# pnotp/ArcFlow

Hardware: AMD Instinct MI355X
Metric: 1024x1024 images/sec @ 2 NFE (FLUX-12B architecture, denoiser + ArcFlow integrator) (higher is better)
Workload: dtype bf16; 1 GPU; ArcFlow-FLUX-12B 2-NFE inference, 1024x1024, bs=1 per GPU; nfe=2, parallelism=1 independent replica(s), no collective, lora=merged into base weights

## Files before the change

arcflow_amd/_lib.py:

```python
from __future__ import annotations

import ctypes as C
import os
from typing import Optional

from .build import lib_path

AFX_DT_BF16 = 1
AFX_DT_F32 = 2
AFX_DT_FP8 = 3

EXPORTS = [
    'afx_last_error', 'afx_version', 'afx_create', 'afx_destroy', 'afx_bind_weight', 'afx_finalize',
    'afx_workspace_bytes', 'afx_head_width', 'afx_set_workspace', 'afx_mmdit_forward', 'afx_profile_enable', 'afx_profile_read', 'afx_set_checkpoint_buffer', 'afx_arcflow_step',
    'afx_arcflow_velocity', 'afx_linear_bf16', 'afx_attention_ws_bytes', 'afx_attention_bf16', 'afx_attention_to_mx8',
    'afx_norm_modulate_bf16', 'afx_qk_norm_rope_bf16', 'afx_gemv_bf16',
    'afx_attention_fwd_lse_bf16', 'afx_attention_bwd_ws_bytes', 'afx_attention_bwd_bf16',
    'afx_ln_modulate_backward', 'afx_qk_norm_rope_oop_bf16', 'afx_gelu_bf16', 'afx_add_scale_bf16',
    'afx_conv3x3_bf16', 'afx_conv3x3_bf16_stats', 'afx_groupnorm_nhwc_from_stats', 'afx_conv_stats_available', 'afx_upconv3x3_bf16', 'afx_groupnorm_nhwc', 'afx_groupnorm_ws_bytes', 'afx_upsample2x_nhwc', 'afx_interior_nhwc', 'afx_softmax_rows_f32',
    'afx_latent_to_nhwc', 'afx_nhwc_to_image', 'afx_latent_to_nhwc_affine', 'afx_rmsnorm_nhwc',
    'afx_conv3x3s2_bf16', 'afx_image_to_cols27', 'afx_posterior_latents',
    'afx_embed_rows_bf16', 'afx_norm_rows_bf16', 'afx_act_mul_bf16', 'afx_rope_half_bf16', 'afx_attention_ext_ws_bytes',
    'afx_attention_ext_bf16', 'afx_linear_bf16_splitk', 'afx_finish_f32_bf16', 'afx_linear_splitk_chunks', 'afx_quant_rows_fp8', 'afx_linear_fp8', 'afx_quant_rows_mx8', 'afx_linear_fp8_mx', 'afx_linear_fp8_to_mx8',
    'afx_linear_bf16_pre', 'afx_gemm_set_mode', 'afx_gemm_set_fp8_tile', 'afx_gemm_dropres_available', 'afx_attn_set_impl', 'afx_attn_bwd_set_impl', 'afx_mmdit_prepare_steps', 'afx_mmdit_use_prepared_step', 'afx_lora_dropout_bf16', 'afx_mmdit_forward_stage', 'afx_mmdit_import_tokens',
    'afx_coldot_bf16', 'afx_gate_residual_bf16', 'afx_gemv_t_bf16', 'afx_set_temb_override', 'afx_set_fp8_linear',
    'afx_arcflow_step_dropout', 'afx_arcflow_backward', 'afx_mse_loss', 'afx_euler_roll', 'afx_axpby_rows', 'afx_cfg_combine',
    'afx_head_grad', 'afx_linear_bf16_f32out', 'afx_linear_tn_f32out', 'afx_linear_tn_f32out_ws', 'afx_linear_tn_ws_bytes', 'afx_linear_bf16_dropres', 'afx_transpose_bf16', 'afx_colsum_bf16', 'afx_normout_backward', 'afx_normout_backward_split',
    'afx_outer_accum', 'afx_mmdit_export', 'afx_sumsq', 'afx_adamw_step', 'afx_adamw8bit_step', 'afx_ema_lerp', 'afx_cast_f32_bf16',
    'afx_qkv_operands', 'afx_norm_modulate_joint_bf16', 'afx_norm_modulate_mx8',
]

AFX_BLOCK_DOUBLE, AFX_BLOCK_SINGLE = 0, 1
AFX_QKV_PATHS = {'auto': 0, 'vt_proj': 1, 'qk_epi': 2, 'kv_prep': 3}


class ModelDesc(C.Structure):
    _fields_ = [(n, C.c_int32) for n in (
        'family', 'num_double', 'num_single', 'heads', 'head_dim', 'in_channels', 'joint_dim',
        'pooled_dim', 'guidance_embeds', 'num_gaussians', 'logweights_channels', 'head_mode')]


class ArcflowHipError(RuntimeError):
    pass


_lib: Optional[C.CDLL] = None


def load() -> C.CDLL:
    global _lib
    if _lib is not None:
        return _lib
    path = os.environ.get('ARCFLOW_HIP_LIB', lib_path())
    if not os.path.exists(path):
        raise ArcflowHipError(
            f'{path} not found: the HIP engine is not built. Run `python -m arcflow_amd.build` '
            '(needs hipcc, cross-compiles for gfx950 without a GPU). There is no CPU fallback.')
    lib = C.CDLL(path)
    vp, i32, i64, f32 = C.c_void_p, C.c_int32, C.c_int64, C.c_float
    lib.afx_last_error.restype = C.c_char_p
    lib.afx_version.restype = C.c_char_p
    lib.afx_create.argtypes = [C.POINTER(ModelDesc), C.POINTER(vp)]
    lib.afx_destroy.argtypes = [vp]
    lib.afx_bind_weight.argtypes = [vp, C.c_char_p, vp, i32, i32, C.POINTER(i64)]
    lib.afx_finalize.argtypes = [vp]
    lib.afx_workspace_bytes.argtypes = [vp, i32, i32, i32]
    lib.afx_workspace_bytes.restype = i64
    lib.afx_head_width.argtypes = [vp]
    lib.afx_head_width.restype = i32
    lib.afx_set_workspace.argtypes = [vp, vp, i64]
    lib.afx_mmdit_forward.argtypes = [vp, vp, vp, vp, vp, vp, vp, vp, i32, i32, i32, vp, vp, vp, vp]
    lib.afx_set_checkpoint_buffer.argtypes = [vp, vp]
    lib.afx_profile_enable.argtypes = [vp, i32]
    lib.afx_profile_read.argtypes = [vp, i32, C.POINTER(C.c_double), C.POINTER(i64), C.POINTER(C.c_double)]
    lib.afx_arcflow_step.argtypes = [vp, vp, vp, vp, i32, f32, f32, f32, vp, f32, vp, i32, i32, i32, i32, i32, vp]
    lib.afx_arcflow_velocity.argtypes = [vp, vp, vp, i32, f32, f32, vp, vp, i32, i32, i32, i32, i32, vp]
    lib.afx_linear_bf16.argtypes = [vp, i64, vp, i64, vp, vp, i64, i32, i32, i32, i32, i32, vp, i64, i32, vp, i64, vp]
    lib.afx_attention_ws_bytes.argtypes = [i32, i32, i32]
    lib.afx_attention_ws_bytes.restype = i64
    lib.afx_attention_bf16.argtypes = [vp, i64, vp, i64, vp, i64, vp, i64, vp, i32, i32, i32, vp]
    lib.afx_attention_to_mx8.argtypes = [vp, i64, vp, i64, vp, i64, vp, i64, vp, i64, vp, i32, i32, i32, vp]
    lib.afx_norm_modulate_bf16.argtypes = [vp, i64, vp, i64, i32, i32, vp, vp, i64, i32, i32, vp]
    lib.afx_qk_norm_rope_bf16.argtypes = [vp, i64, vp, vp, vp, vp, i32, i32, i32, i32, vp]
    lib.afx_gemv_bf16.argtypes = [vp, vp, vp, vp, i32, i32, i32, i32, i32, vp]
    lib.afx_attention_fwd_lse_bf16.argtypes = [vp, i64, vp, i64, vp, i64, vp, i64, vp, vp, i32, i32, i32, vp]
    lib.afx_attention_bwd_ws_bytes.argtypes = [i32, i32, i32]
    lib.afx_attention_bwd_ws_bytes.restype = i64
    lib.afx_attention_bwd_bf16.argtypes = [vp, i64, vp, i64, vp, i64, vp, i64, vp, i64, vp, vp, i64, vp, i64, vp, i64, vp, i32, i32, i32, vp]
    lib.afx_ln_modulate_backward.argtypes = [vp, i64, vp, i64, vp, i64, i32, vp, i64, vp, i64, i32, i32, vp]
    lib.afx_qk_norm_rope_oop_bf16.argtypes = [vp, i64, vp, i64, vp, i64, vp, vp, vp, vp, i32, i32, i32, i32, i32, vp]
    lib.afx_gelu_bf16.argtypes = [vp, i64, vp, i64, vp, i64, i64, i32, vp]
    lib.afx_add_scale_bf16.argtypes = [vp, i64, vp, i64, vp, i64, i32, vp, i64, i64, i32, vp]
    lib.afx_conv3x3_bf16.argtypes = [vp, vp, vp, vp, i32, i32, i32, i32, vp, vp]
    lib.afx_groupnorm_nhwc.argtypes = [vp, vp, vp, i32, i32, i32, i32, vp, vp, f32, i32, vp]
    lib.afx_groupnorm_ws_bytes.argtypes = [i32, i32]
    lib.afx_groupnorm_ws_bytes.restype = i64
    lib.afx_conv3x3_bf16_stats.argtypes = [vp, vp, vp, vp, i32, i32, i32, i32, vp, vp, i32, vp]
    lib.afx_groupnorm_nhwc_from_stats.argtypes = [vp, vp, vp, vp, i32, i32, i32, i32, vp, vp, f32, i32, vp]
    lib.afx_conv_stats_available.argtypes = []
    lib.afx_upconv3x3_bf16.argtypes = [vp, vp, vp, vp, i32, i32, i32, i32, vp]
    lib.afx_upsample2x_nhwc.argtypes = [vp, vp, i32, i32, i32, vp]
    lib.afx_interior_nhwc.argtypes = [vp, vp, vp, i32, i32, i32, i32, vp]
    lib.afx_softmax_rows_f32.argtypes = [vp, i64, vp, i64, i32, i32, f32, vp]
    lib.afx_latent_to_nhwc.argtypes = [vp, vp, i32, i32, i32, f32, f32, vp]
    lib.afx_nhwc_to_image.argtypes = [vp, vp, i32, i32, i32, vp]
    lib.afx_latent_to_nhwc_affine.argtypes = [vp, vp, i32, i32, i32, vp, vp, vp]
    lib.afx_rmsnorm_nhwc.argtypes = [vp, vp, i64, i32, i32, vp, i32, vp]
    lib.afx_conv3x3s2_bf16.argtypes = [vp, vp, vp, vp, vp, i32, i32, i32, i32, vp, i32, vp]
    lib.afx_image_to_cols27.argtypes = [vp, i32, vp, i32, i32, i32, vp]
    lib.afx_posterior_latents.argtypes = [vp, i32, i32, i32, vp, vp, vp, vp, vp, i32, vp, i32, vp, vp]
    lib.afx_embed_rows_bf16.argtypes = [vp, vp, vp, vp, i32, i32, vp]
    lib.afx_norm_rows_bf16.argtypes = [vp, i64, vp, i64, i32, i32, vp, vp, f32, i32, vp]
    lib.afx_act_mul_bf16.argtypes = [vp, i64, vp, i64, i64, i32, i32, i32, vp]
    lib.afx_rope_half_bf16.argtypes = [vp, i64, vp, vp, i32, i32, i32, vp]
    lib.afx_linear_bf16_splitk.argtypes = [vp, i64, vp, i64, vp, vp, i32, i32, i32, i32, vp]
    lib.afx_finish_f32_bf16.argtypes = [vp, i32, vp, i64, vp, i64, i64, i32, vp]
    lib.afx_quant_rows_fp8.argtypes = [vp, i64, vp, i64, vp, i32, i32, vp]
    lib.afx_linear_fp8.argtypes = [vp, i64, vp, vp, i64, vp, vp, vp, i64, i32, i32, i32, i32, i32, vp, i64, i32, vp, i64, vp]
    lib.afx_quant_rows_mx8.argtypes = [vp, i64, vp, i64, vp, i64, i32, i32, vp]
    lib.afx_linear_fp8_to_mx8.argtypes = [vp, i64, vp, i64, vp, vp, i64, vp, vp, vp, i64, vp, i64, vp, i64, i32, i32, i32, i32, i32, vp]
    lib.afx_linear_fp8_mx.argtypes = [vp, i64, vp, i64, vp, vp, i64, vp, vp, vp, i64, i32, i32, i32, i32, i32, vp, i64, i32, vp, i64, vp]
    lib.afx_linear_splitk_chunks.argtypes = [i32, i32, i32, i32]
    lib.afx_linear_bf16_pre.argtypes = [vp, i64, vp, i64, vp, vp, i64, i32, i32, i32, i32, i32, vp, i64, i32, vp, i64, vp, i64, vp]
    lib.afx_mmdit_prepare_steps.argtypes = [vp, vp, vp, vp, i32, i32, vp]
    lib.afx_mmdit_use_prepared_step.argtypes = [vp, i32]
    lib.afx_gemm_set_mode.argtypes = [i32, i32]
    lib.afx_gemm_set_mode.restype = i32
    lib.afx_gemm_set_fp8_tile.argtypes = [i32]
    lib.afx_gemm_set_fp8_tile.restype = i32
    lib.afx_gemm_dropres_available.argtypes = []
    lib.afx_gemm_dropres_available.restype = i32
    lib.afx_attn_set_impl.argtypes = [i32]
    lib.afx_attn_set_impl.restype = i32
    lib.afx_attn_bwd_set_impl.argtypes = [i32]
    lib.afx_attn_bwd_set_impl.restype = i32
    lib.afx_lora_dropout_bf16.argtypes = [vp, i64, vp, i64, i64, i32, i64, f32, C.c_uint32, i32, vp]
    lib.afx_mmdit_forward_stage.argtypes = [vp, vp, vp, vp, vp, vp, vp, vp, i32, i32, i32, vp, vp, vp, i32, vp]
    lib.afx_mmdit_import_tokens.argtypes = [vp, vp, i32, i32, i32, vp]
    lib.afx_coldot_bf16.argtypes = [vp, i64, vp, i64, vp, i32, i32, vp]
    lib.afx_gate_residual_bf16.argtypes = [vp, i64, vp, vp, i64, vp, i64, i64, i32, vp]
    lib.afx_gemv_t_bf16.argtypes = [vp, i64, vp, i64, vp, i32, i64, i32, vp]
    lib.afx_set_temb_override.argtypes = [vp, vp]
    lib.afx_set_fp8_linear.argtypes = [vp, i32]
    lib.afx_linear_splitk_chunks.restype = i32
    lib.afx_attention_ext_ws_bytes.argtypes = [i32, i32, i32, i32]
    lib.afx_attention_ext_ws_bytes.restype = i64
    lib.afx_attention_ext_bf16.argtypes = [vp, i64, vp, i64, vp, i64, vp, i64, vp, i32, i32, i32, i32, i32, f32, i32, vp, vp]
    lib.afx_arcflow_step_dropout.argtypes = [vp, vp, vp, vp, i32, vp, vp, f32, vp, i32, i32, i32, i32, i32, vp]
    lib.afx_arcflow_backward.argtypes = [vp, vp, vp, vp, i32, f32, f32, f32, vp, vp, f32, f32, vp, vp, vp, i32, i32, i32,
                                         i32, i32, i32, i32, vp]
    lib.afx_mse_loss.argtypes = [vp, vp, f32, vp, vp, i64, vp]
    lib.afx_euler_roll.argtypes = [vp, vp, vp, vp, vp, i32, i64, vp]
    lib.afx_axpby_rows.argtypes = [vp, vp, vp, vp, vp, i32, i64, vp]
    lib.afx_cfg_combine.argtypes = [vp, vp, f32, vp, i64, vp]
    lib.afx_head_grad.argtypes = [vp, vp, vp, vp, vp, i64, i64, i32, i32, i32, vp]
    lib.afx_linear_bf16_f32out.argtypes = [vp, i64, vp, i64, vp, i64, i32, i32, i32, i32, vp]
    lib.afx_linear_tn_f32out.argtypes = [vp, i64, vp, i64, vp, i64, i32, i32, i32, i32, vp]
    lib.afx_linear_tn_f32out_ws.argtypes = [vp, i64, vp, i64, vp, i64, i32, i32, i32, i32, vp, vp]
    lib.afx_linear_tn_ws_bytes.argtypes = [i32, i32, i32]
    lib.afx_linear_tn_ws_bytes.restype = i64
    lib.afx_linear_bf16_dropres.argtypes = [vp, i64, vp, i64, vp, i64, i32, i32, i32, vp, i64, f32, C.c_uint32, i64, vp]
    lib.afx_transpose_bf16.argtypes = [vp, i64, vp, i64, i32, i32, vp]
    lib.afx_colsum_bf16.argtypes = [vp, i64, vp, i32, i32, vp]
    lib.afx_normout_backward.argtypes = [vp, i64, vp, i64, vp, i32, i32, i32, vp]
    lib.afx_normout_backward_split.argtypes = [vp, i64, vp, i64, vp, vp, i32, i32, vp]
    lib.afx_outer_accum.argtypes = [vp, vp, vp, i32, i32, i32, vp]
    lib.afx_mmdit_export.argtypes = [vp, C.c_char_p, vp, i32, i32, i32, vp]
    lib.afx_sumsq.argtypes = [vp, vp, i64, vp]
    lib.afx_adamw_step.argtypes = [vp, vp, vp, vp, f32, f32, f32, f32, f32, i32, f32, i64, vp]
    lib.afx_adamw8bit_step.argtypes = [vp, vp, vp, vp, vp, vp, vp, vp, f32, f32, f32, f32, f32, i32, f32, i64, vp]
    lib.afx_ema_lerp.argtypes = [vp, vp, f32, i64, vp]
    lib.afx_cast_f32_bf16.argtypes = [vp, vp, i64, vp]
    lib.afx_qkv_operands.argtypes = [i32, vp, i64, vp, vp, vp, vp, vp, vp, vp, i32, i32, i32, i32, i32, vp, i64, vp, vp]
    lib.afx_norm_modulate_joint_bf16.argtypes = [vp, i64, vp, i64, i32, i32, vp, vp, vp, vp, i64, i32, i32, vp]
    lib.afx_norm_modulate_mx8.argtypes = [vp, i64, vp, i64, vp, i64, vp, i32, i32, vp, vp, vp, vp, i64, i32, i32, C.POINTER(i32), vp]
    for name in EXPORTS:
        fn = getattr(lib, name)
        if fn.restype is C.c_int:
            fn.restype = C.c_int32
    _lib = lib
    return lib


def check(rc: int) -> None:
    if rc != 0:
        raise ArcflowHipError(f'libarcflow_hip error {rc}: {load().afx_last_error().decode()}')
```

arcflow_amd/csrc/afx_elementwise.hip:

```cpp
#include <cstdlib>

#include "afx_common.h"
#include "afx_kernels.h"

namespace afx {

constexpr int NM_MAX_CHUNKS = 8;

__global__ __launch_bounds__(256) void norm_modulate_kernel(
    const bf16_t* __restrict__ x, int64_t ldx, bf16_t* __restrict__ out, int64_t ldo, int rows, int D,
    const float* __restrict__ scale, const float* __restrict__ shift, int64_t ldmod, int rows_per_batch,
    int rms, const float* __restrict__ scale_txt, const float* __restrict__ shift_txt, int n_txt) {
  const int lane = threadIdx.x & 63;
  const int row = blockIdx.x * 4 + (threadIdx.x >> 6);
  if (row >= rows) return;
  const int nchunk = D >> 3;
  const bf16_t* xr = x + (int64_t)row * ldx;
  float v[NM_MAX_CHUNKS][8];
  float s = 0.f;
#pragma unroll
  for (int i = 0; i < NM_MAX_CHUNKS; ++i) {
    const int c = lane + i * 64;
    if (c < nchunk) {
      const u32x4_t w = *reinterpret_cast<const u32x4_t*>(xr + c * 8);
      unpack8(w, v[i]);
#pragma unroll
      for (int e = 0; e < 8; ++e) s += rms ? v[i][e] * v[i][e] : v[i][e];
    }
  }
  s = wave_sum(s);
  float mean = 0.f, rstd;
  if (rms) {
    rstd = rsqrtf(s / (float)D + 1e-6f);
  } else {
    mean = s / (float)D;
    float q = 0.f;
#pragma unroll
    for (int i = 0; i < NM_MAX_CHUNKS; ++i) {
      const int c = lane + i * 64;
      if (c < nchunk) {
#pragma unroll
        for (int e = 0; e < 8; ++e) {
          const float d = v[i][e] - mean;
          q += d * d;
        }
      }
    }
    q = wave_sum(q);
    rstd = rsqrtf(q / (float)D + 1e-6f);
  }
  const int64_t moff = rms ? 0 : (int64_t)(row / rows_per_batch) * ldmod;
  if (scale_txt != nullptr && row % rows_per_batch < n_txt) {
    scale = scale_txt;
    shift = shift_txt;
  }
  bf16_t* orow = out + (int64_t)row * ldo;
#pragma unroll
  for (int i = 0; i < NM_MAX_CHUNKS; ++i) {
    const int c = lane + i * 64;
    if (c < nchunk) {
      const f32x4_t s0 = *reinterpret_cast<const f32x4_t*>(scale + moff + c * 8);
      const f32x4_t s1 = *reinterpret_cast<const f32x4_t*>(scale + moff + c * 8 + 4);
      const float sc[8] = {s0[0], s0[1], s0[2], s0[3], s1[0], s1[1], s1[2], s1[3]};
      float r[8];
      if (rms) {
#pragma unroll
        for (int e = 0; e < 8; ++e) r[e] = v[i][e] * rstd * sc[e];
      } else {
        const f32x4_t h0 = *reinterpret_cast<const f32x4_t*>(shift + moff + c * 8);
        const f32x4_t h1 = *reinterpret_cast<const f32x4_t*>(shift + moff + c * 8 + 4);
        const float sh[8] = {h0[0], h0[1], h0[2], h0[3], h1[0], h1[1], h1[2], h1[3]};
#pragma unroll
        for (int e = 0; e < 8; ++e) r[e] = (v[i][e] - mean) * rstd * (1.0f + sc[e]) + sh[e];
      }
      *reinterpret_cast<u32x4_t*>(orow + c * 8) = pack8(r);
    }
  }
}

template <int NCH, int R, int QOUT = 0>
__global__ __launch_bounds__(256) void norm_modulate_rows_kernel(
    const bf16_t* __restrict__ x, int64_t ldx, bf16_t* __restrict__ out, int64_t ldo, int rows,
    const float* __restrict__ scale, const float* __restrict__ shift, int64_t ldmod, int rows_per_batch,
    const float* __restrict__ scale_txt, const float* __restrict__ shift_txt, int n_txt, uint8_t* __restrict__ q8 = nullptr, int64_t ldq = 0,
    uint8_t* __restrict__ mx = nullptr, int64_t ld_mx = 0, float* __restrict__ rowscale = nullptr) {
  constexpr bool MX8 = QOUT == 1;
  constexpr int D = 512 * NCH;
  const int lane = threadIdx.x & 63;
  const int row0 = (blockIdx.x * 4 + (threadIdx.x >> 6)) * R;
  if (row0 >= rows) return;
  const int nrows = min(R, rows - row0);
  float sc[NCH][8], sh[NCH][8];
  int key = -1;
  u32x4_t cur[NCH], nxt[NCH];
  {
    const bf16_t* xr = x + (int64_t)row0 * ldx;
#pragma unroll
    for (int i = 0; i < NCH; ++i) cur[i] = *reinterpret_cast<const u32x4_t*>(xr + (lane + i * 64) * 8);
  }
#pragma unroll 1
  for (int rr = 0; rr < nrows; ++rr) {
    const int row = row0 + rr;
    if (rr + 1 < nrows) {
      const bf16_t* xn = x + (int64_t)(row + 1) * ldx;
#pragma unroll
      for (int i = 0; i < NCH; ++i) nxt[i] = *reinterpret_cast<const u32x4_t*>(xn + (lane + i * 64) * 8);
    }
    const int b = row / rows_per_batch;
    const bool txt = scale_txt != nullptr && row - b * rows_per_batch < n_txt;
    const int k = 2 * b + (txt ? 1 : 0);
    if (k != key) {
      key = k;
      const float* sp = (txt ? scale_txt : scale) + (int64_t)b * ldmod;
      const float* hp = (txt ? shift_txt : shift) + (int64_t)b * ldmod;
#pragma unroll
      for (int i = 0; i < NCH; ++i) {
        const int c = (lane + i * 64) * 8;
        const f32x4_t s0 = *reinterpret_cast<const f32x4_t*>(sp + c), s1 = *reinterpret_cast<const f32x4_t*>(sp + c + 4);
        const f32x4_t h0 = *reinterpret_cast<const f32x4_t*>(hp + c), h1 = *reinterpret_cast<const f32x4_t*>(hp + c + 4);
#pragma unroll
        for (int e = 0; e < 4; ++e) {
          sc[i][e] = 1.0f + s0[e]; sc[i][4 + e] = 1.0f + s1[e];
          sh[i][e] = h0[e];        sh[i][4 + e] = h1[e];
        }
      }
    }
    float v[NCH][8];
    float s = 0.f;
#pragma unroll
    for (int i = 0; i < NCH; ++i) {
      unpack8(cur[i], v[i]);
#pragma unroll
      for (int e = 0; e < 8; ++e) s += v[i][e];
    }
    s = wave_sum(s);
    const float mean = s / (float)D;
    float q = 0.f;
#pragma unroll
    for (int i = 0; i < NCH; ++i)
#pragma unroll
      for (int e = 0; e < 8; ++e) {
        const float d = v[i][e] - mean;
        q += d * d;
      }
    q = wave_sum(q);
    const float rstd = rsqrtf(q / (float)D + 1e-6f);
    bf16_t* orow = out + (int64_t)row * ldo;
    if constexpr (QOUT == 2) {
      float amax = 0.f;
#pragma unroll
      for (int i = 0; i < NCH; ++i)
#pragma unroll
        for (int e = 0; e < 8; ++e) {
          v[i][e] = (v[i][e] - mean) * rstd * sc[i][e] + sh[i][e];
          amax = fmaxf(amax, fabsf(v[i][e]));
        }
#pragma unroll
      for (int o = 32; o > 0; o >>= 1) amax = fmaxf(amax, __shfl_xor(amax, o, 64));
      const float s_ = fmaxf(amax, 1e-12f) / 448.0f;
      const float inv = 1.0f / s_;
      if (lane == 0) rowscale[row] = s_;
#pragma unroll
      for (int i = 0; i < NCH; ++i) {
        uint32_t w0, w1;
        mx_pack8(v[i], inv, w0, w1);
        *reinterpret_cast<u32x2_t*>(q8 + (int64_t)row * ldq + (lane + i * 64) * 8) = (u32x2_t){w0, w1};
      }
    } else
#pragma unroll
    for (int i = 0; i < NCH; ++i) {
      float r[8];
#pragma unroll
      for (int e = 0; e < 8; ++e) r[e] = (v[i][e] - mean) * rstd * sc[i][e] + sh[i][e];
      if constexpr (MX8) {
        float amax = 0.f;
#pragma unroll
        for (int e = 0; e < 8; ++e) amax = fmaxf(amax, fabsf(r[e]));
#pragma unroll
        for (int o = 8; o > 0; o >>= 1) amax = fmaxf(amax, __shfl_xor(amax, o, 64));
        const int eb = mx_exp(amax);
        uint32_t w0, w1;
        mx_pack8(r, mx_inv(eb), w0, w1);
        *reinterpret_cast<u32x2_t*>(q8 + (int64_t)row * ldq + (lane + i * 64) * 8) = (u32x2_t){w0, w1};
        if ((lane & 15) == 0) mx[(int64_t)row * ld_mx + 4 * i + (lane >> 4)] = (uint8_t)eb;
      } else
      *reinterpret_cast<u32x4_t*>(orow + (lane + i * 64) * 8) = pack8(r);
    }
#pragma unroll
    for (int i = 0; i < NCH; ++i) cur[i] = nxt[i];
  }
}

static int nm_rows_per_wave() {
  static int r = -1;
  if (r < 0) {
    const char* e = getenv("AFX_NM_ROWS");
    r = e ? atoi(e) : 2;
  }
  return r;
}

static bool launch_norm_modulate_rows(const uint16_t* x, int64_t ldx, uint16_t* out, int64_t ldo, int rows, int D, const float* scale,
                                      const float* shift, int64_t ldmod, int rows_per_batch, const float* scale_txt, const float* shift_txt,
                                      int n_txt, hipStream_t stream, uint8_t* q8 = nullptr, int64_t ldq = 0, uint8_t* mx = nullptr, int64_t ld_mx = 0,
                                      float* rowscale = nullptr) {
  const int R = nm_rows_per_wave();
  if (D != 3072 || rows < 1024 || (R != 2 && R != 4)) return false;
  const dim3 grid((rows + 4 * R - 1) / (4 * R));
  if (q8 != nullptr) {
    if (R != 2) return false;
    if (rowscale != nullptr)
      hipLaunchKernelGGL((norm_modulate_rows_kernel<6, 2, 2>), grid, dim3(256), 0, stream, x, ldx, out, ldo, rows, scale, shift, ldmod, rows_per_batch,
                         scale_txt, shift_txt, n_txt, q8, ldq, (uint8_t*)nullptr, (int64_t)0, rowscale);
    else
      hipLaunchKernelGGL((norm_modulate_rows_kernel<6, 2, 1>), grid, dim3(256), 0, stream, x, ldx, out, ldo, rows, scale, shift, ldmod, rows_per_batch,
                         scale_txt, shift_txt, n_txt, q8, ldq, mx, ld_mx, (float*)nullptr);
    return true;
  }
  if (R == 2)
    hipLaunchKernelGGL((norm_modulate_rows_kernel<6, 2, 0>), grid, dim3(256), 0, stream, x, ldx, out, ldo, rows, scale, shift, ldmod, rows_per_batch,
                       scale_txt, shift_txt, n_txt);
  else
    hipLaunchKernelGGL((norm_modulate_rows_kernel<6, 4, 0>), grid, dim3(256), 0, stream, x, ldx, out, ldo, rows, scale, shift, ldmod, rows_per_batch,
                       scale_txt, shift_txt, n_txt);
  return true;
}

hipError_t launch_norm_modulate(const uint16_t* x, int64_t ldx, uint16_t* out, int64_t ldo, int rows,
                                int D, const float* scale, const float* shift, int64_t ldmod,
                                int rows_per_batch, int rms, hipStream_t stream) {
  if (rows <= 0) return hipSuccess;
  if (D > NM_MAX_CHUNKS * 512 || (D & 7)) return hipErrorInvalidValue;
  if (!rms && launch_norm_modulate_rows(x, ldx, out, ldo, rows, D, scale, shift, ldmod, rows_per_batch > 0 ? rows_per_batch : rows, nullptr, nullptr, 0,
                                        stream))
    return hipGetLastError();
  hipLaunchKernelGGL(norm_modulate_kernel, dim3((rows + 3) / 4), dim3(256), 0, stream, x, ldx, out, ldo, rows,
                     D, scale, shift, ldmod, rows_per_batch > 0 ? rows_per_batch : rows, rms, (const float*)nullptr,
                     (const float*)nullptr, 0);
  return hipGetLastError();
}

hipError_t launch_norm_modulate_mx8(const uint16_t* x, int64_t ldx, uint8_t* q8, int64_t ldq, uint8_t* mx, int64_t ld_mx, int rows, int D,
                                    const float* scale, const float* shift, const float* scale_txt, const float* shift_txt, int64_t ldmod, int S,
                                    int n_txt, hipStream_t stream, bool* fused, float* rowscale) {
  *fused = rows > 0 && launch_norm_modulate_rows(x, ldx, nullptr, 0, rows, D, scale, shift, ldmod, S, scale_txt, shift_txt, n_txt, stream, q8, ldq, mx, ld_mx,
                                                 rowscale);
  return hipGetLastError();
}

hipError_t launch_norm_modulate_joint(const uint16_t* x, int64_t ldx, uint16_t* out, int64_t ldo, int rows, int D, const float* scale,
                                      const float* shift, const float* scale_txt, const float* shift_txt, int64_t ldmod, int S,
                                      int n_txt, hipStream_t stream) {
  if (rows <= 0) return hipSuccess;
  if (D > NM_MAX_CHUNKS * 512 || (D & 7) || S <= 0) return hipErrorInvalidValue;
  if (launch_norm_modulate_rows(x, ldx, out, ldo, rows, D, scale, shift, ldmod, S, scale_txt, shift_txt, n_txt, stream)) return hipGetLastError();
  hipLaunchKernelGGL(norm_modulate_kernel, dim3((rows + 3) / 4), dim3(256), 0, stream, x, ldx, out, ldo, rows, D, scale, shift, ldmod,
                     S, 0, scale_txt, shift_txt, n_txt);
  return hipGetLastError();
}

struct QkRopeArgs { bf16_t* x[2]; const float* w_txt[2]; const float* w_img[2]; };

__global__ __launch_bounds__(256) void qk_norm_rope_kernel(
    const QkRopeArgs a, int64_t ldx, const float* __restrict__ cos_t, const float* __restrict__ sin_t, int S, int n_txt, int H,
    int64_t total) {
  bf16_t* __restrict__ x = a.x[blockIdx.y];
  const float* __restrict__ w_txt = a.w_txt[blockIdx.y];
  const float* __restrict__ w_img = a.w_img[blockIdx.y];
  const int64_t g = (int64_t)blockIdx.x * 256 + threadIdx.x;
  if (g >= total) return;
  const int c = (int)(g & 15);
  const int64_t th = g >> 4;
  const int h = (int)(th % H);
  const int64_t row = th / H;
  const int s = (int)(row % S);
  bf16_t* p = x + row * ldx + h * 128 + c * 8;
  float v[8];
  unpack8(*reinterpret_cast<const u32x4_t*>(p), v);
  float ss = 0.f;
#pragma unroll
  for (int e = 0; e < 8; ++e) ss += v[e] * v[e];
#pragma unroll
  for (int o = 8; o > 0; o >>= 1) ss += __shfl_xor(ss, o, 64);
  const float rstd = rsqrtf(ss * (1.0f / 128.0f) + 1e-6f);
  const float* w = (s < n_txt ? w_txt : w_img) + c * 8;
  const f32x4_t w0 = *reinterpret_cast<const f32x4_t*>(w);
  const f32x4_t w1 = *reinterpret_cast<const f32x4_t*>(w + 4);
  const float wv[8] = {w0[0], w0[1], w0[2], w0[3], w1[0], w1[1], w1[2], w1[3]};
  const f32x4_t cs = *reinterpret_cast<const f32x4_t*>(cos_t + (int64_t)s * 64 + c * 4);
  const f32x4_t sn = *reinterpret_cast<const f32x4_t*>(sin_t + (int64_t)s * 64 + c * 4);
  float r[8];
#pragma unroll
  for (int i = 0; i < 4; ++i) {
    const float a = v[2 * i] * rstd * wv[2 * i];
    const float b = v[2 * i + 1] * rstd * wv[2 * i + 1];
    r[2 * i] = a * cs[i] - b * sn[i];
    r[2 * i + 1] = a * sn[i] + b * cs[i];
  }
  *reinterpret_cast<u32x4_t*>(p) = pack8(r);
}

hipError_t launch_qk_norm_rope(uint16_t* x, int64_t ldx, const float* w_txt, const float* w_img,
                               const float* cos_t, const float* sin_t, int B, int S, int n_txt, int H,
                               hipStream_t stream) {
  const int64_t total = (int64_t)B * S * H * 16;
  if (total == 0) return hipSuccess;
  QkRopeArgs a{};
  a.x[0] = x; a.w_txt[0] = w_txt; a.w_img[0] = w_img;
  hipLaunchKernelGGL(qk_norm_rope_kernel, dim3((unsigned)((total + 255) / 256), 1), dim3(256), 0, stream, a, ldx, cos_t, sin_t, S,
                     n_txt, H, total);
  return hipGetLastError();
}

hipError_t launch_qk_norm_rope2(uint16_t* xk, uint16_t* xq, int64_t ldx, const float* wk_txt, const float* wk_img, const float* wq_txt,
                                const float* wq_img, const float* cos_t, const float* sin_t, int B, int S, int n_txt, int H,
                                hipStream_t stream) {
  const int64_t total = (int64_t)B * S * H * 16;
  if (total == 0) return hipSuccess;
  QkRopeArgs a{};
  a.x[0] = xk; a.w_txt[0] = wk_txt; a.w_img[0] = wk_img;
  a.x[1] = xq; a.w_txt[1] = wq_txt; a.w_img[1] = wq_img;
  hipLaunchKernelGGL(qk_norm_rope_kernel, dim3((unsigned)((total + 255) / 256), 2), dim3(256), 0, stream, a, ldx, cos_t, sin_t, S,
                     n_txt, H, total);
  return hipGetLastError();
}

constexpr int GEMV_MAXB = 8;

__global__ __launch_bounds__(256) void gemv_kernel(const float* __restrict__ x, const bf16_t* __restrict__ W,
                                                   const bf16_t* __restrict__ bias, float* __restrict__ y,
                                                   int B, int N, int K, int act, int accumulate, int64_t ldy) {
  const int lane = threadIdx.x & 63;
  const int n = blockIdx.x * 4 + (threadIdx.x >> 6);
  if (n >= N) return;
  const bf16_t* wr = W + (int64_t)n * K;
  float acc[GEMV_MAXB];
#pragma unroll
  for (int b = 0; b < GEMV_MAXB; ++b) acc[b] = 0.f;
  for (int c = lane; c < (K >> 3); c += 64) {
    float w[8];
    unpack8(*reinterpret_cast<const u32x4_t*>(wr + c * 8), w);
#pragma unroll
    for (int b = 0; b < GEMV_MAXB; ++b) {
      if (b < B) {
        const f32x4_t x0 = *reinterpret_cast<const f32x4_t*>(x + (int64_t)b * K + c * 8);
        const f32x4_t x1 = *reinterpret_cast<const f32x4_t*>(x + (int64_t)b * K + c * 8 + 4);
        acc[b] += w[0] * x0[0] + w[1] * x0[1] + w[2] * x0[2] + w[3] * x0[3] + w[4] * x1[0] + w[5] * x1[1] +
                  w[6] * x1[2] + w[7] * x1[3];
      }
    }
  }
  const float bv = bias ? bf16_to_f32(bias[n]) : 0.f;
#pragma unroll
  for (int b = 0; b < GEMV_MAXB; ++b) {
    if (b < B) {
      float r = wave_sum(acc[b]) + bv;
      if (act == 1) r = silu(r);
      if (lane == 0) {
        float* yp = y + (int64_t)b * ldy + n;
        *yp = accumulate ? (*yp + r) : r;
      }
    }
  }
}

hipError_t launch_gemv(const float* x, const uint16_t* W, const uint16_t* bias, float* y, int B, int N,
                       int K, int act, int accumulate, hipStream_t stream, int64_t ldy) {
  if (ldy <= 0) ldy = N;
  if (B > GEMV_MAXB || (K & 7)) return hipErrorInvalidValue;
  if (N == 0 || B == 0) return hipSuccess;
  hipLaunchKernelGGL(gemv_kernel, dim3((N + 3) / 4), dim3(256), 0, stream, x, W, bias, y, B, N, K, act, accumulate, ldy);
  return hipGetLastError();
}

__global__ void sincos_kernel(const float* __restrict__ t, float scale, float* __restrict__ out, int B, int cast_mode) {
  const int i = threadIdx.x;
  const int b = blockIdx.x;
  if (b >= B) return;
  const float f = expf(-9.210340371976184f * (float)i / 128.0f);
  float tb = t[b];
  if (cast_mode != 0) tb = bf16_to_f32(f32_to_bf16(tb));
  float a;
  if (cast_mode == 1) a = bf16_to_f32(f32_to_bf16(tb * scale)) * f;
  else a = scale * (tb * f);
  out[b * 256 + i] = cosf(a);
  out[b * 256 + 128 + i] = sinf(a);
}
hipError_t launch_sincos(const float* t, float scale, float* out, int B, int cast_mode, hipStream_t stream) {
  hipLaunchKernelGGL(sincos_kernel, dim3(B), dim3(128), 0, stream, t, scale, out, B, cast_mode);
  return hipGetLastError();
}

__global__ void silu_kernel(const float* __restrict__ x, float* __restrict__ y, int64_t n) {
  const int64_t i = (int64_t)blockIdx.x * 256 + threadIdx.x;
  if (i < n) y[i] = silu(x[i]);
}
hipError_t launch_silu(const float* x, float* y, int64_t n, hipStream_t stream) {
  hipLaunchKernelGGL(silu_kernel, dim3((unsigned)((n + 255) / 256)), dim3(256), 0, stream, x, y, n);
  return hipGetLastError();
}

__global__ void bf16_to_f32_kernel(const bf16_t* __restrict__ x, float* __restrict__ y, int64_t n) {
  const int64_t i = (int64_t)blockIdx.x * 256 + threadIdx.x;
  if (i < n) y[i] = bf16_to_f32(x[i]);
}
hipError_t launch_bf16_to_f32(const uint16_t* x, float* y, int64_t n, hipStream_t stream) {
  hipLaunchKernelGGL(bf16_to_f32_kernel, dim3((unsigned)((n + 255) / 256)), dim3(256), 0, stream, x, y, n);
  return hipGetLastError();
}

__global__ void copy_rows_kernel(const bf16_t* __restrict__ src, int64_t lds_, bf16_t* __restrict__ dst,
                                 int64_t ldd, int64_t rows, int cols) {
  const int cpr = cols >> 3;
  const int64_t g = (int64_t)blockIdx.x * 256 + threadIdx.x;
  if (g >= rows * cpr) return;
  const int64_t r = g / cpr;
  const int c = (int)(g % cpr);
  *reinterpret_cast<u32x4_t*>(dst + r * ldd + c * 8) = *reinterpret_cast<const u32x4_t*>(src + r * lds_ + c * 8);
}
hipError_t launch_copy_rows(const uint16_t* src, int64_t lds_, uint16_t* dst, int64_t ldd, int64_t rows,
                            int cols, hipStream_t stream) {
  const int64_t total = rows * (cols >> 3);
  if (total == 0) return hipSuccess;
  hipLaunchKernelGGL(copy_rows_kernel, dim3((unsigned)((total + 255) / 256)), dim3(256), 0, stream, src, lds_,
                     dst, ldd, rows, cols);
  return hipGetLastError();
}

__global__ __launch_bounds__(256) void head_split_kernel(const bf16_t* __restrict__ head, int64_t ldh,
                                                         bf16_t* __restrict__ means, bf16_t* __restrict__ logw,
                                                         bf16_t* __restrict__ logg, int64_t rows, int K, int ch,
                                                         int lw) {
  const int64_t row = blockIdx.x;
  const bf16_t* hr = head + row * ldh;
  const int nm = K * ch, nw = K * lw, ng = (K - 1) * lw;
  for (int i = threadIdx.x; i < nm; i += 256) means[row * nm + i] = hr[i];
  for (int i = threadIdx.x; i < ng; i += 256) logg[row * ng + i] = hr[nm + nw + i];
  if (threadIdx.x < lw) {
    const int p = threadIdx.x;
    float mx = -INFINITY;
    for (int k = 0; k < K; ++k) mx = fmaxf(mx, bf16_to_f32(hr[nm + k * lw + p]));
    float se = 0.f;
    for (int k = 0; k < K; ++k) se += expf(bf16_to_f32(hr[nm + k * lw + p]) - mx);
    const float lse = mx + logf(se);
    for (int k = 0; k < K; ++k) logw[row * nw + k * lw + p] = f32_to_bf16(bf16_to_f32(hr[nm + k * lw + p]) - lse);
  }
}
hipError_t launch_head_split(const uint16_t* head, int64_t ldh, uint16_t* means, uint16_t* logw,
                             uint16_t* logg, int64_t rows, int K, int ch, int lw, hipStream_t stream) {
  if (rows == 0) return hipSuccess;
  hipLaunchKernelGGL(head_split_kernel, dim3((unsigned)rows), dim3(256), 0, stream, head, ldh, means, logw, logg,
                     rows, K, ch, lw);
  return hipGetLastError();
}

template <typename MixT> AFX_DEV float mix_load(const MixT* p, int64_t i);
template <> AFX_DEV float mix_load<float>(const float* p, int64_t i) { return p[i]; }
template <> AFX_DEV float mix_load<bf16_t>(const bf16_t* p, int64_t i) { return bf16_to_f32(p[i]); }

constexpr int ARC_MAXK = 32;

template <typename MixT>
__global__ __launch_bounds__(256) void arcflow_step_kernel(
    const float* __restrict__ x_in, const MixT* __restrict__ means, const MixT* __restrict__ logw,
    const MixT* __restrict__ logg, float s_src, float s_start, float s_end,
    const float* __restrict__ sigma_vec, float eps, float* __restrict__ x_out, int64_t tokens, int n_tok, int K,
    int ch, int pp, int velocity_only, const uint8_t* __restrict__ drop) {
  const int lane = threadIdx.x & 63;
  const int64_t tok = (int64_t)blockIdx.x * 4 + (threadIdx.x >> 6);
  if (tok >= tokens) return;
  const int64_t bidx = tok / n_tok;
  if (sigma_vec != nullptr) {
    s_src = sigma_vec[3 * bidx];
    s_start = sigma_vec[3 * bidx + 1];
    s_end = sigma_vec[3 * bidx + 2];
  }
  const float d_past = s_src - s_start;
  const float d_step = s_start - s_end;
  const uint8_t* dr = drop ? drop + bidx * K : nullptr;
  const MixT* mt = means + tok * (int64_t)K * ch;
  const MixT* wt = logw + tok * (int64_t)K * pp;
  const MixT* gt = logg + tok * (int64_t)(K - 1) * pp;
  for (int c = lane; c < ch; c += 64) {
    const int q = c % pp;
    float lw[ARC_MAXK];
    float mx = -INFINITY;
#pragma unroll
    for (int k = 0; k < ARC_MAXK; ++k)
      if (k < K) {
        lw[k] = (dr && dr[k]) ? -INFINITY : mix_load<MixT>(wt, k * pp + q);
        mx = fmaxf(mx, lw[k]);
      }
    float den = 0.f;
#pragma unroll
    for (int k = 0; k < ARC_MAXK; ++k)
      if (k < K) {
        lw[k] = expf(lw[k] - mx);
        den += lw[k];
      }
    const float inv = 1.0f / den;
    float acc = (lw[0] * inv) * mix_load<MixT>(mt, c) * (velocity_only ? 1.0f : d_step);
#pragma unroll
    for (int k = 1; k < ARC_MAXK; ++k)
      if (k < K) {
        const float g = mix_load<MixT>(gt, (k - 1) * pp + q);
        const float m = mix_load<MixT>(mt, (int64_t)k * ch + c);
        const float decay = expf(g * d_past);
        float term;
        if (velocity_only) {
          term = m * decay;
        } else {
          const float z = g * d_step;
          const float zs = (z < 0.f ? -1.0f : 1.0f) * fmaxf(fabsf(z), eps);
          const float phi = expm1f(zs) / zs;
          term = m * decay * d_step * phi;
        }
        acc += (lw[k] * inv) * term;
      }
    const int64_t xi = tok * ch + c;
    x_out[xi] = velocity_only ? acc : (x_in[xi] - acc);
  }
}


template <typename MixT> struct Mix8;
template <> struct Mix8<bf16_t> {
  AFX_DEV static void load(const bf16_t* p, float (&f)[8]) { unpack8(*reinterpret_cast<const u32x4_t*>(p), f); }
};
template <> struct Mix8<float> {
  AFX_DEV static void load(const float* p, float (&f)[8]) {
    const f32x4_t a = *reinterpret_cast<const f32x4_t*>(p), b = *reinterpret_cast<const f32x4_t*>(p + 4);
    f[0] = a[0]; f[1] = a[1]; f[2] = a[2]; f[3] = a[3]; f[4] = b[0]; f[5] = b[1]; f[6] = b[2]; f[7] = b[3];
  }
};

template <typename MixT, int TPW>
__global__ __launch_bounds__(256) void arcflow_step_k16_kernel(
    const float* __restrict__ x_in, const MixT* __restrict__ means, const MixT* __restrict__ logw,
    const MixT* __restrict__ logg, float s_src0, float s_start0, float s_end0, const float* __restrict__ sigma_vec, float eps,
    float* __restrict__ x_out, int64_t tokens, int n_tok, int velocity_only, const uint8_t* __restrict__ drop) {
  constexpr int K = 16, CH = 64, PP = 4;
  const int lane = threadIdx.x & 63;
  const int64_t tok0 = ((int64_t)blockIdx.x * 4 + (threadIdx.x >> 6)) * TPW;
  if (tok0 >= tokens) return;
  const int k = lane >> 2;
  float mA[TPW][8], mB[TPW][8], lw[TPW], lg[TPW], xv[TPW];
#pragma unroll
  for (int t = 0; t < TPW; ++t) {
    const int64_t tok = tok0 + t < tokens ? tok0 + t : tokens - 1;
    const MixT* mt = means + tok * (int64_t)(K * CH);
    Mix8<MixT>::load(mt + lane * 8, mA[t]);
    Mix8<MixT>::load(mt + (64 + lane) * 8, mB[t]);
    lw[t] = mix_load<MixT>(logw + tok * (K * PP), lane);
    lg[t] = k > 0 ? mix_load<MixT>(logg + tok * ((K - 1) * PP), lane - PP) : 0.f;
  }
  const int e3 = ((lane >> 5) & 1) * 4 + ((lane >> 4) & 1) * 2 + ((lane >> 3) & 1);
  const int cfin = (lane & 7) * 8 + e3;
  if (!velocity_only) {
#pragma unroll
    for (int t = 0; t < TPW; ++t) xv[t] = x_in[(tok0 + t < tokens ? tok0 + t : tokens - 1) * CH + cfin];
  }
#pragma unroll
  for (int t = 0; t < TPW; ++t) {
    const int64_t tok = tok0 + t;
    if (tok >= tokens) break;
    const int64_t bidx = tok / n_tok;
    float s_src = s_src0, s_start = s_start0, s_end = s_end0;
    if (sigma_vec != nullptr) {
      s_src = sigma_vec[3 * bidx];
      s_start = sigma_vec[3 * bidx + 1];
      s_end = sigma_vec[3 * bidx + 2];
    }
    const float d_past = s_src - s_start, d_step = s_start - s_end;
    float l = lw[t];
    if (drop != nullptr && drop[bidx * K + k]) l = -INFINITY;
    float mx = l;
#pragma unroll
    for (int o = 4; o < 64; o <<= 1) mx = fmaxf(mx, __shfl_xor(mx, o, 64));
    const float ex = expf(l - mx);
    float den = ex;
#pragma unroll
    for (int o = 4; o < 64; o <<= 1) den += __shfl_xor(den, o, 64);
    float coef = ex / den;
    if (k > 0) {
      const float g = lg[t];
      coef *= expf(g * d_past);
      if (!velocity_only) {
        const float z = g * d_step;
        const float zs = (z < 0.f ? -1.0f : 1.0f) * fmaxf(fabsf(z), eps);
        coef *= d_step * (expm1f(zs) / zs);
      }
    } else if (!velocity_only) {
      coef *= d_step;
    }
    float cA[4], cB[4];
#pragma unroll
    for (int q = 0; q < 4; ++q) {
      cA[q] = __shfl(coef, (lane >> 3) * 4 + q, 64);
      cB[q] = __shfl(coef, (8 + (lane >> 3)) * 4 + q, 64);
    }
    float v[8];
#pragma unroll
    for (int e = 0; e < 8; ++e) v[e] = cA[e & 3] * mA[t][e] + cB[e & 3] * mB[t][e];
    const bool h5 = (lane & 32) != 0, h4 = (lane & 16) != 0, h3 = (lane & 8) != 0;
    float w4[4], w2[2];
#pragma unroll
    for (int i = 0; i < 4; ++i) {
      const float keep = h5 ? v[4 + i] : v[i], send = h5 ? v[i] : v[4 + i];
      w4[i] = keep + __shfl_xor(send, 32, 64);
    }
#pragma unroll
    for (int i = 0; i < 2; ++i) {
      const float keep = h4 ? w4[2 + i] : w4[i], send = h4 ? w4[i] : w4[2 + i];
      w2[i] = keep + __shfl_xor(send, 16, 64);
    }
    const float keep = h3 ? w2[1] : w2[0], send = h3 ? w2[0] : w2[1];
    const float acc = keep + __shfl_xor(send, 8, 64);
    x_out[tok * CH + cfin] = velocity_only ? acc : (xv[t] - acc);
  }
}

hipError_t launch_arcflow_step(const float* x_in, const void* means, const void* logw, const void* logg,
                               int mix_bf16, float s_src, float s_start, float s_end,
                               const float* sigma_vec, float eps, float* x_out, int B, int n_tok, int K,
                               int ch, int pp, int velocity_only, const uint8_t* drop, hipStream_t stream) {
  if (K < 1 || K > ARC_MAXK || pp < 1 || ch < 1) return hipErrorInvalidValue;
  const int64_t tokens = (int64_t)B * n_tok;
  if (tokens == 0) return hipSuccess;
  if (K == 16 && ch == 64 && pp == 4) {
    static int tpw = -1;
    if (tpw < 0) {
      const char* e = getenv("AFX_STEP_TPW");
      tpw = e ? atoi(e) : 1;
      if (tpw != 1 && tpw != 2 && tpw != 4) tpw = 1;
    }
#define AFX_STEP_LAUNCH(T, TPW)                                                                                                     \
    hipLaunchKernelGGL((arcflow_step_k16_kernel<T, TPW>), dim3((unsigned)((tokens + 4 * TPW - 1) / (4 * TPW))), dim3(256), 0, stream, \
                       x_in, (const T*)means, (const T*)logw, (const T*)logg, s_src, s_start, s_end, sigma_vec, eps, x_out, tokens,  \
                       n_tok, velocity_only, drop)
    if (mix_bf16) {
      if (tpw == 1) AFX_STEP_LAUNCH(bf16_t, 1); else if (tpw == 4) AFX_STEP_LAUNCH(bf16_t, 4); else AFX_STEP_LAUNCH(bf16_t, 2);
    } else {
      if (tpw == 1) AFX_STEP_LAUNCH(float, 1); else if (tpw == 4) AFX_STEP_LAUNCH(float, 4); else AFX_STEP_LAUNCH(float, 2);
    }
#undef AFX_STEP_LAUNCH
    return hipGetLastError();
  }
  dim3 grid((unsigned)((tokens + 3) / 4)), block(256);
  if (mix_bf16)
    hipLaunchKernelGGL(arcflow_step_kernel<bf16_t>, grid, block, 0, stream, x_in, (const bf16_t*)means,
                       (const bf16_t*)logw, (const bf16_t*)logg, s_src, s_start, s_end, sigma_vec, eps, x_out,
                       tokens, n_tok, K, ch, pp, velocity_only, drop);
  else
    hipLaunchKernelGGL(arcflow_step_kernel<float>, grid, block, 0, stream, x_in, (const float*)means,
                       (const float*)logw, (const float*)logg, s_src, s_start, s_end, sigma_vec, eps, x_out,
                       tokens, n_tok, K, ch, pp, velocity_only, drop);
  return hipGetLastError();
}

}
```

arcflow_amd/csrc/afx_engine.hip:

```cpp
#include <hip/hip_runtime.h>

#include <cstdarg>
#include <cstdio>
#include <cstring>
#include <string>
#include <unordered_map>
#include <vector>

#include "../../include/arcflow_hip.h"
#include "afx_kernels.h"

using namespace afx;

#include "afx_api_util.h"

thread_local char afx_g_err[512] = "";

int afx_fail(int code, const char* fmt, ...) {
  va_list ap;
  va_start(ap, fmt);
  vsnprintf(afx_g_err, sizeof(afx_g_err), fmt, ap);
  va_end(ap);
  return code;
}

namespace {

struct Weight {
  const void* ptr = nullptr;
  int dtype = 0;
  std::vector<int64_t> shape;
};

inline int64_t align256(int64_t x) { return (x + 255) / 256 * 256; }

}

struct LinW {
  const uint16_t* w = nullptr;
  const uint16_t* b = nullptr;
  const void* wq = nullptr;
  const float* wscale = nullptr;
};
struct DoubleW { LinW qkv[2], out[2], mlp1[2], mlp2[2]; const float* qkn = nullptr; };
struct SingleW { LinW fused, out; const float* qkn = nullptr; };

struct afx_ctx {
  afx_model_desc d;
  std::unordered_map<std::string, Weight> w;
  bool finalized = false;
  std::vector<DoubleW> dbl;
  std::vector<SingleW> sgl;
  char* ws = nullptr;
  int64_t ws_bytes = 0;
  int D = 0;
  int64_t n_mod = 0;
  int head_n = 0;
  uint16_t* ckpt = nullptr;
  bool fp8 = false;
  int fp8_mx = -1;
  const float* temb_override = nullptr;
  int prep_steps = 0, prep_B = 0, prep_use = -1;
  bool prof_on = false;
  int prof_stride = 1;
  uint64_t prof_count = 0;
  struct ProfRec { hipEvent_t a, b; int klass; double flops; };
  std::vector<ProfRec> prof_pool;
  size_t prof_used = 0;
};

namespace {

const uint16_t* W16(const afx_ctx* c, const std::string& n) {
  auto it = c->w.find(n);
  return it == c->w.end() ? nullptr : (const uint16_t*)it->second.ptr;
}
const float* W32(const afx_ctx* c, const std::string& n) {
  auto it = c->w.find(n);
  return it == c->w.end() ? nullptr : (const float*)it->second.ptr;
}

const void* WQ(const afx_ctx* c, const std::string& n) {
  auto it = c->w.find(n);
  return it == c->w.end() ? nullptr : it->second.ptr;
}

int need(const afx_ctx* c, const std::string& n, int dtype, std::vector<int64_t> shape) {
  auto it = c->w.find(n);
  if (it == c->w.end()) return fail(AFX_E_MISSING, "weight '%s' is not bound", n.c_str());
  if (it->second.dtype != dtype) return fail(AFX_E_INVALID, "weight '%s': wrong dtype", n.c_str());
  if (it->second.shape != shape) {
    std::string got, want;
    for (auto v : it->second.shape) got += std::to_string(v) + ",";
    for (auto v : shape) want += std::to_string(v) + ",";
    return fail(AFX_E_INVALID, "weight '%s': shape [%s] expected [%s]", n.c_str(), got.c_str(), want.c_str());
  }
  return AFX_OK;
}

int need_linear(const afx_ctx* c, const std::string& n, int64_t out_f, int64_t in_f) {
  int r = need(c, n + ".weight", AFX_DT_BF16, {out_f, in_f});
  if (r) return r;
  return need(c, n + ".bias", AFX_DT_BF16, {out_f});
}

struct ModLayout {
  int64_t D;
  int nd, ns;
  int64_t dbl(int i, int stream , int chunk ) const {
    return ((int64_t)i * 12 + stream * 6 + chunk) * D;
  }
  int64_t sgl(int i, int chunk ) const { return (int64_t)nd * 12 * D + ((int64_t)i * 3 + chunk) * D; }
  int64_t fin(int chunk ) const { return (int64_t)nd * 12 * D + (int64_t)ns * 3 * D + chunk * D; }
  int64_t total() const { return (int64_t)nd * 12 * D + (int64_t)ns * 3 * D + 2 * D; }
};

constexpr int AFX_PREP_ROWS = 8;

struct Workspace {
  uint16_t *X, *Xn, *F, *Vt, *head;
  float *sincos, *tmp, *temb, *semb, *mod, *pooled;
  float *prep_temb, *prep_semb, *prep_mod;
  uint8_t* q8;
  uint8_t* q8n;
  uint8_t* mxn;
  uint8_t* mxw;
  float* ones;
  int64_t ld_mxn, ld_mxw;
  float* qs;
  int64_t total;
};

Workspace carve(const afx_ctx* c, char* base, int B, int N, int T) {
  const int64_t D = c->D, S = (int64_t)N + T, R = (int64_t)B * S;
  Workspace w;
  int64_t off = 0;
  auto take = [&](int64_t bytes) {
    char* p = base ? base + off : nullptr;
    off += align256(bytes);
    return p;
  };
  w.prep_temb = (float*)take((int64_t)AFX_PREP_ROWS * D * 4);
  w.prep_semb = (float*)take((int64_t)AFX_PREP_ROWS * D * 4);
  w.prep_mod = (float*)take((int64_t)AFX_PREP_ROWS * c->n_mod * 4);
  w.X = (uint16_t*)take(R * D * 2);
  w.Xn = (uint16_t*)take(R * D * 2);
  w.F = (uint16_t*)take(R * 7 * D * 2);
  w.Vt = (uint16_t*)take((int64_t)B * c->d.heads * 128 * attn_spad((int)S) * 2);
  w.head = (uint16_t*)take((int64_t)B * N * c->head_n * 2);
  w.sincos = (float*)take((int64_t)B * 256 * 4);
  w.tmp = (float*)take((int64_t)B * D * 4);
  w.temb = (float*)take((int64_t)B * D * 4);
  w.semb = (float*)take((int64_t)B * D * 4);
  w.pooled = (float*)take((int64_t)B * (c->d.pooled_dim > 0 ? c->d.pooled_dim : 8) * 4);
  w.mod = (float*)take((int64_t)B * c->n_mod * 4);
  w.q8 = nullptr;
  w.qs = nullptr;
  w.q8n = w.mxn = w.mxw = nullptr;
  w.ones = nullptr;
  w.ld_mxn = (D / 128 + 3) / 4 * 4;
  w.ld_mxw = (5 * D / 128 + 3) / 4 * 4;
  if (c->fp8) {
    w.q8 = (uint8_t*)take(R * 5 * D);
    w.qs = (float*)take(R * 4);
    w.q8n = (uint8_t*)take(R * D);
    w.mxn = (uint8_t*)take(R * w.ld_mxn);
    w.mxw = (uint8_t*)take(R * w.ld_mxw);
    w.ones = (float*)take(R * 4);
  }
  w.total = off;
  return w;
}

struct ProfScope {
  afx_ctx* c; hipStream_t st; afx_ctx::ProfRec* r = nullptr;
  ProfScope(afx_ctx* c_, hipStream_t st_, int klass, double flops) : c(c_), st(st_) {
    if (!c->prof_on) return;
    if ((c->prof_count++ % (uint64_t)c->prof_stride) != 0) return;
    if (c->prof_used == c->prof_pool.size()) {
      afx_ctx::ProfRec n{};
      if (hipEventCreate(&n.a) != hipSuccess || hipEventCreate(&n.b) != hipSuccess) return;
      c->prof_pool.push_back(n);
    }
    r = &c->prof_pool[c->prof_used++];
    r->klass = klass; r->flops = flops;
    launch_timer().start = r->a;
    launch_timer().stop = r->b;
  }
  ~ProfScope() { launch_timer() = LaunchTimer{}; }
};

double gemm_flops(const GemmBatch& gb) {
  double f = 0;
  for (int i = 0; i < gb.nprob; ++i) f += 2.0 * gb.p[i].M * (double)gb.p[i].N * gb.p[i].K;
  return f;
}

struct BlockShape {
  int64_t D;
  int H, B, N, T, S, S_pad;
  const float* rope_cos;
  const float* rope_sin;
  uint16_t* Vt;
};

BlockShape block_shape(int H, int B, int N, int T, const float* rope_cos, const float* rope_sin, uint16_t* Vt) {
  BlockShape q;
  q.D = (int64_t)H * 128; q.H = H; q.B = B; q.N = N; q.T = T; q.S = N + T; q.S_pad = (int)attn_spad(N + T);
  q.rope_cos = rope_cos; q.rope_sin = rope_sin; q.Vt = Vt;
  return q;
}

bool vt_proj_shape_ok(const BlockShape& q, bool single) {
  return q.T % 16 == 0 && q.S % 64 == 0 && (!single || q.B + 3 <= GEMM_MAX_PROBLEMS);
}

int qkv_path(const BlockShape& q, bool single, bool fp8, bool qk_fuse_fp8) {
  const bool qk_fuse = gemm_qk_fusion_available() && (!fp8 || qk_fuse_fp8);
  const bool vt_fuse = qk_fuse && !fp8 && getenv("AFX_VT_FUSE_OFF") == nullptr && vt_proj_shape_ok(q, single);
  return vt_fuse ? AFX_QKV_VT_PROJ : qk_fuse ? AFX_QKV_QK_EPI : AFX_QKV_KV_PREP;
}

void set_qk_epilogue(GemmProblem& p, const BlockShape& q, const float* wq, const float* wk, int row0, int period) {
  p.qk_D = (int)q.D; p.qk_wq = wq; p.qk_wk = wk;
  p.rope_cos = q.rope_cos; p.rope_sin = q.rope_sin; p.rope_row0 = row0; p.rope_period = period; p.rope_rows = q.S;
}

void stream_qk_epilogue(GemmProblem& p, const BlockShape& q, const float* qkn, int s) {
  set_qk_epilogue(p, q, qkn + (s == 0 ? 0 : 2) * 128, qkn + (s == 0 ? 1 : 3) * 128, s == 0 ? q.T : 0, 1 << 30);
}

void stream_problem(GemmProblem& p, const BlockShape& q, const uint16_t* A, int64_t lda, int K, const LinW& lw, uint16_t* C, int64_t ldc,
                    int Nout, int b, int s) {
  p = GemmProblem{};
  const int64_t row0 = (int64_t)b * q.S + (s == 0 ? q.T : 0);
  p.A = A + row0 * lda; p.lda = lda;
  p.W = lw.w; p.ldw = K; p.bias = lw.b;
  p.C = C + row0 * ldc; p.ldc = ldc;
  p.M = (s == 0 ? q.N : q.T); p.N = Nout; p.K = K;
}

void kqv_problems(GemmBatch& gb, const BlockShape& q, const uint16_t* A, int64_t lda, const LinW& lw, uint16_t* C, int64_t ldc, int64_t row0g,
                  int rows, int b, int pos0, int period, const float* wq, const float* wk, bool with_v) {
  const int64_t D = q.D;
  for (int part = 0; part < (with_v ? 3 : 2); ++part) {
    GemmProblem& p = gb.p[gb.nprob++];
    p = GemmProblem{};
    p.K = (int)D; p.epi = EPI_NONE;
    if (part < 2) {
      const int64_t wrow = part == 0 ? 0 : 2 * D;
      p.A = A + row0g * lda; p.lda = lda;
      p.W = lw.w + wrow * D; p.ldw = D; p.bias = lw.b ? lw.b + wrow : nullptr;
      p.C = C + row0g * ldc + wrow; p.ldc = ldc; p.M = rows; p.N = (int)D;
      set_qk_epilogue(p, q, part == 0 ? wk : wq, part == 0 ? wk : wq, pos0, period);
    } else {
      p.A = lw.w + D * D; p.lda = D; p.bias = lw.b ? lw.b + D : nullptr; p.bias_rows = 1;
      p.W = A + row0g * lda; p.ldw = lda; p.w_perm16 = 1;
      p.C = q.Vt + (int64_t)b * q.H * 128 * q.S_pad + pos0; p.ldc = q.S_pad; p.M = (int)D; p.N = rows;
    }
  }
}

void double_vt_batch(GemmBatch& gb, const BlockShape& q, const uint16_t* A, int64_t lda, const LinW (&lw)[2], uint16_t* QKV, int64_t ldq,
                     const float* qkn, int b) {
  for (int s = 0; s < 2; ++s)
    kqv_problems(gb, q, A, lda, lw[s], QKV, ldq, (int64_t)b * q.S + (s == 0 ? q.T : 0), s == 0 ? q.N : q.T, b, s == 0 ? q.T : 0, 1 << 30,
                 qkn + (s == 0 ? 0 : 2) * 128, qkn + (s == 0 ? 1 : 3) * 128, true);
}

void single_qkv_batch(GemmBatch& gb, int path, const BlockShape& q, const uint16_t* A, int64_t lda, const LinW& lw, uint16_t* F, int64_t ldf,
                      const float* qkn) {
  const int64_t D = q.D;
  const int R = q.B * q.S;
  gb.nprob = 1;
  GemmProblem& f = gb.p[0];
  f = GemmProblem{};
  f.A = A; f.lda = lda; f.W = lw.w; f.ldw = D; f.bias = lw.b;
  f.C = F; f.ldc = ldf; f.M = R; f.N = (int)(7 * D); f.K = (int)D; f.epi = EPI_GELU; f.gelu_col0 = (int)(3 * D);
  if (path == AFX_QKV_VT_PROJ) {
    gb.nprob = 0;
    kqv_problems(gb, q, A, lda, lw, F, ldf, 0, R, 0, 0, q.S, qkn, qkn + 128, false);
    GemmProblem& m = gb.p[gb.nprob++];
    m = GemmProblem{};
    m.A = A; m.lda = lda; m.W = lw.w + 3 * D * D; m.ldw = D; m.bias = lw.b ? lw.b + 3 * D : nullptr;
    m.C = F + 3 * D; m.ldc = ldf; m.M = R; m.N = (int)(4 * D); m.K = (int)D; m.epi = EPI_GELU; m.gelu_col0 = 0;
    for (int b = 0; b < q.B; ++b) {
      GemmProblem& v = gb.p[gb.nprob++];
      v = GemmProblem{};
      v.A = lw.w + D * D; v.lda = D; v.bias = lw.b ? lw.b + D : nullptr; v.bias_rows = 1;
      v.W = A + (int64_t)b * q.S * lda; v.ldw = lda; v.w_perm16 = 1;
      v.C = q.Vt + (int64_t)b * q.H * 128 * q.S_pad; v.ldc = q.S_pad; v.M = (int)D; v.N = q.S; v.K = (int)D; v.epi = EPI_NONE;
    }
  } else if (path == AFX_QKV_QK_EPI) {
    set_qk_epilogue(f, q, qkn, qkn + 128, 0, q.S);
  }
}

hipError_t qkv_finish(int path, const BlockShape& q, uint16_t* F, int64_t ldf, const float* wk_txt, const float* wk_img, const float* wq_txt,
                      const float* wq_img, hipStream_t st) {
  if (path == AFX_QKV_QK_EPI) return launch_v_transpose(F + q.D, ldf, q.Vt, q.B, q.H, q.S, st);
  if (path == AFX_QKV_KV_PREP)
    return launch_kv_prep(F, F + 2 * q.D, ldf, wk_txt, wk_img, wq_txt, wq_img, q.rope_cos, q.rope_sin, q.T, F + q.D, ldf, q.Vt, q.B, q.H, q.S, st);
  return hipSuccess;
}

}

extern "C" {

const char* afx_last_error(void) { return afx_g_err; }
const char* afx_version(void) { return "arcflow_hip 0.1 (gfx950)"; }

int afx_create(const afx_model_desc* desc, afx_ctx** out) {
  if (!desc || !out) return fail(AFX_E_INVALID, "null argument");
  if (desc->head_dim != 128) return fail(AFX_E_UNSUPPORTED, "head_dim must be 128");
  if (desc->heads <= 0 || desc->num_double < 0 || desc->num_single < 0 || desc->num_gaussians < 1 ||
      desc->num_gaussians > 32)
    return fail(AFX_E_INVALID, "bad model description");
  if (desc->in_channels % 64 != 0 || desc->joint_dim % 64 != 0)
    return fail(AFX_E_UNSUPPORTED, "in_channels and joint_dim must be multiples of 64");
  afx_ctx* c = new afx_ctx();
  c->d = *desc;
  c->D = desc->heads * desc->head_dim;
  ModLayout ml{c->D, desc->num_double, desc->num_single};
  c->n_mod = ml.total();
  const int K = desc->num_gaussians, ch = desc->in_channels, lw = desc->logweights_channels;
  const int raw = desc->head_mode == 0 ? K * ch + K * lw + (K - 1) * lw : ch;
  c->head_n = (raw + 7) / 8 * 8;
  *out = c;
  return AFX_OK;
}

int afx_destroy(afx_ctx* ctx) {
  if (ctx) {
    for (auto& r : ctx->prof_pool) { (void)hipEventDestroy(r.a); (void)hipEventDestroy(r.b); }
  }
  delete ctx;
  return AFX_OK;
}

int afx_bind_weight(afx_ctx* ctx, const char* name, const void* dptr, int32_t dtype, int32_t ndim,
                    const int64_t* shape) {
  if (!ctx || !name || !dptr || ndim < 1 || ndim > 4 || !shape) return fail(AFX_E_INVALID, "bad bind_weight argument");
  if (dtype != AFX_DT_BF16 && dtype != AFX_DT_F32 && dtype != AFX_DT_FP8) return fail(AFX_E_INVALID, "bad dtype for '%s'", name);
  Weight w;
  w.ptr = dptr;
  w.dtype = dtype;
  w.shape.assign(shape, shape + ndim);
  ctx->w[name] = w;
  ctx->finalized = false;
  return AFX_OK;
}

int afx_finalize(afx_ctx* c) {
  if (!c) return fail(AFX_E_INVALID, "null ctx");
  const int64_t D = c->D;
  const afx_model_desc& d = c->d;
  int r;
#define NEED(x) \
  if ((r = (x)) != AFX_OK) return r
  NEED(need_linear(c, "x_in", D, d.in_channels));
  NEED(need_linear(c, "ctx_in", D, d.joint_dim));
  if (d.family == 1) NEED(need(c, "txt_norm.weight", AFX_DT_F32, {d.joint_dim}));
  NEED(need_linear(c, "temb.t.l1", D, 256));
  NEED(need_linear(c, "temb.t.l2", D, D));
  if (d.guidance_embeds) {
    NEED(need_linear(c, "temb.g.l1", D, 256));
    NEED(need_linear(c, "temb.g.l2", D, D));
  }
  if (d.pooled_dim > 0) {
    NEED(need_linear(c, "temb.p.l1", D, d.pooled_dim));
    NEED(need_linear(c, "temb.p.l2", D, D));
  }
  NEED(need_linear(c, "mod", c->n_mod, D));
  for (int i = 0; i < d.num_double; ++i) {
    const std::string p = "d" + std::to_string(i) + ".";
    for (const char* s : {"img", "txt"}) {
      NEED(need_linear(c, p + s + "_qkv", 3 * D, D));
      NEED(need_linear(c, p + s + "_out", D, D));
      NEED(need_linear(c, p + s + "_mlp1", 4 * D, D));
      NEED(need_linear(c, p + s + "_mlp2", D, 4 * D));
    }
    NEED(need(c, p + "qknorm", AFX_DT_F32, {4, 128}));
  }
  for (int i = 0; i < d.num_single; ++i) {
    const std::string p = "s" + std::to_string(i) + ".";
    NEED(need_linear(c, p + "fused", 7 * D, D));
    NEED(need_linear(c, p + "out", D, 5 * D));
    NEED(need(c, p + "qknorm", AFX_DT_F32, {2, 128}));
  }
  NEED(need_linear(c, "head", c->head_n, D));
  if (c->w.count("mod_final.weight")) NEED(need_linear(c, "mod_final", 2 * D, D));
#undef NEED
  auto lin = [&](const std::string& n) {
    LinW l;
    l.w = W16(c, n + ".weight"); l.b = W16(c, n + ".bias");
    l.wq = WQ(c, n + ".weight_q"); l.wscale = W32(c, n + ".wscale");
    return l;
  };
  c->dbl.assign(d.num_double, DoubleW{});
  for (int i = 0; i < d.num_double; ++i) {
    const std::string p = "d" + std::to_string(i) + ".";
    for (int s = 0; s < 2; ++s) {
      const std::string q = p + (s == 0 ? "img_" : "txt_");
      c->dbl[i].qkv[s] = lin(q + "qkv"); c->dbl[i].out[s] = lin(q + "out");
      c->dbl[i].mlp1[s] = lin(q + "mlp1"); c->dbl[i].mlp2[s] = lin(q + "mlp2");
    }
    c->dbl[i].qkn = W32(c, p + "qknorm");
  }
  c->sgl.assign(d.num_single, SingleW{});
  for (int i = 0; i < d.num_single; ++i) {
    const std::string p = "s" + std::to_string(i) + ".";
    c->sgl[i].fused = lin(p + "fused"); c->sgl[i].out = lin(p + "out");
    c->sgl[i].qkn = W32(c, p + "qknorm");
  }
  c->finalized = true;
  return AFX_OK;
}

int64_t afx_workspace_bytes(const afx_ctx* ctx, int32_t batch, int32_t n_img, int32_t n_txt) {
  if (!ctx || batch < 1 || n_img < 1 || n_txt < 0) return fail(AFX_E_INVALID, "bad workspace query");
  return carve(ctx, nullptr, batch, n_img, n_txt).total;
}

int afx_head_width(const afx_ctx* ctx) {
  if (!ctx) return fail(AFX_E_INVALID, "afx_head_width: null ctx");
  return ctx->head_n;
}

int afx_set_workspace(afx_ctx* ctx, void* dptr, int64_t bytes) {
  if (!ctx || !dptr || bytes <= 0) return fail(AFX_E_INVALID, "bad workspace");
  if (((uintptr_t)dptr & 255) != 0) return fail(AFX_E_INVALID, "workspace must be 256-byte aligned");
  ctx->ws = (char*)dptr;
  ctx->ws_bytes = bytes;
  ctx->prep_steps = 0;
  ctx->prep_use = -1;
  return AFX_OK;
}

int afx_mmdit_forward(afx_ctx* c, const void* x, const void* ctx_emb, const void* pooled, const float* t,
                      const float* g, const float* rope_cos, const float* rope_sin, int32_t B, int32_t N,
                      int32_t T, void* means, void* logw, void* logg, void* stream_) {
  return afx_mmdit_forward_stage(c, x, ctx_emb, pooled, t, g, rope_cos, rope_sin, B, N, T, means, logw, logg, 0, stream_);
}

int afx_mmdit_forward_stage(afx_ctx* c, const void* x, const void* ctx_emb, const void* pooled, const float* t,
                            const float* g, const float* rope_cos, const float* rope_sin, int32_t B, int32_t N,
                            int32_t T, void* means, void* logw, void* logg, int32_t stage, void* stream_) {
  if (stage < 0 || stage > 2) return fail(AFX_E_INVALID, "stage must be 0 (all), 1 (conditioning + embedders) or 2 (norm_out + head)");
  if (!c || !x || !ctx_emb || !t || !rope_cos || !rope_sin || !means)
    return fail(AFX_E_INVALID, "null argument to afx_mmdit_forward");
  if (!c->finalized) return fail(AFX_E_MISSING, "afx_finalize() has not succeeded on this context");
  const afx_model_desc& d = c->d;
  if (B < 1 || N < 1 || T < 1) return fail(AFX_E_INVALID, "bad shape: batch, N, T >= 1");
  if (B > AFX_MAX_MICRO_BATCH) {
    if (stage != 0 || c->ckpt) return fail(AFX_E_INVALID, "staged / checkpointed forward: batch must be 1..4 per call");
    const int64_t K = d.num_gaussians, Cc = d.in_channels, lw = d.logweights_channels;
    for (int b0 = 0; b0 < B; b0 += AFX_MAX_MICRO_BATCH) {
      const int nb = B - b0 < AFX_MAX_MICRO_BATCH ? B - b0 : AFX_MAX_MICRO_BATCH;
      const uint16_t* xb = (const uint16_t*)x + (int64_t)b0 * N * Cc;
      const uint16_t* cb = (const uint16_t*)ctx_emb + (int64_t)b0 * T * d.joint_dim;
      const uint16_t* pb = pooled ? (const uint16_t*)pooled + (int64_t)b0 * d.pooled_dim : nullptr;
      uint16_t* mb = (uint16_t*)means + (int64_t)b0 * N * (d.head_mode == 0 ? K * Cc : Cc);
      uint16_t* wb = logw ? (uint16_t*)logw + (int64_t)b0 * N * K * lw : nullptr;
      uint16_t* gb_ = logg ? (uint16_t*)logg + (int64_t)b0 * N * (K - 1) * lw : nullptr;
      const float* temb_all = c->temb_override;
      if (temb_all) c->temb_override = temb_all + (int64_t)b0 * c->D;
      const int rc = afx_mmdit_forward_stage(c, xb, cb, pb, t + b0, g ? g + b0 : nullptr, rope_cos, rope_sin, nb, N, T, mb, wb, gb_, 0, stream_);
      c->temb_override = temb_all;
      if (rc != AFX_OK) return rc;
    }
    return AFX_OK;
  }
  if (d.guidance_embeds && !g) return fail(AFX_E_INVALID, "guidance vector required");
  if (d.pooled_dim > 0 && !pooled) return fail(AFX_E_INVALID, "pooled projections required");
  if (d.head_mode == 0 && (!logw || !logg)) return fail(AFX_E_INVALID, "logw/logg outputs required");
  Workspace ws = carve(c, c->ws, B, N, T);
  if (!c->ws || ws.total > c->ws_bytes)
    return fail(AFX_E_WORKSPACE, "workspace too small: need %lld bytes, have %lld", (long long)ws.total,
                (long long)c->ws_bytes);
  hipStream_t st = (hipStream_t)stream_;
  const int64_t D = c->D;
  const int H = d.heads, S = N + T;
  const int64_t R = (int64_t)B * S;
  ModLayout ml{D, d.num_double, d.num_single};
  const int64_t ldm = c->n_mod;

  const bool use_prep = c->prep_use >= 0 && c->prep_use < c->prep_steps && c->prep_B == B && stage != 2 && c->temb_override == nullptr;
  const int prep_k = c->prep_use;
  if (stage != 2) c->prep_use = -1;
  if (use_prep) {
    const int64_t r0 = (int64_t)prep_k * B;
    HIP_TRY(hipMemcpyAsync(ws.mod, ws.prep_mod + r0 * ldm, (size_t)B * ldm * 4, hipMemcpyDeviceToDevice, st));
    HIP_TRY(hipMemcpyAsync(ws.temb, ws.prep_temb + r0 * D, (size_t)B * D * 4, hipMemcpyDeviceToDevice, st));
    HIP_TRY(hipMemcpyAsync(ws.semb, ws.prep_semb + r0 * D, (size_t)B * D * 4, hipMemcpyDeviceToDevice, st));
  }
  if (stage != 2 && !use_prep) {
  if (c->temb_override != nullptr) {
    HIP_TRY(hipMemcpyAsync(ws.temb, c->temb_override, (size_t)B * D * 4, hipMemcpyDeviceToDevice, st));
  } else {
    HIP_TRY(launch_sincos(t, 1000.0f, ws.sincos, B, d.family == 0 ? 1 : 2, st));
    HIP_TRY(launch_gemv(ws.sincos, W16(c, "temb.t.l1.weight"), W16(c, "temb.t.l1.bias"), ws.tmp, B, (int)D, 256, 1, 0, st));
    HIP_TRY(launch_gemv(ws.tmp, W16(c, "temb.t.l2.weight"), W16(c, "temb.t.l2.bias"), ws.temb, B, (int)D, (int)D, 0, 0, st));
  }
  if (d.guidance_embeds) {
    HIP_TRY(launch_sincos(g, 1000.0f, ws.sincos, B, 1, st));
    HIP_TRY(launch_gemv(ws.sincos, W16(c, "temb.g.l1.weight"), W16(c, "temb.g.l1.bias"), ws.tmp, B, (int)D, 256, 1, 0, st));
    HIP_TRY(launch_gemv(ws.tmp, W16(c, "temb.g.l2.weight"), W16(c, "temb.g.l2.bias"), ws.temb, B, (int)D, (int)D, 0, 1, st));
  }
  if (d.pooled_dim > 0) {
    HIP_TRY(launch_bf16_to_f32((const uint16_t*)pooled, ws.pooled, (int64_t)B * d.pooled_dim, st));
    HIP_TRY(launch_gemv(ws.pooled, W16(c, "temb.p.l1.weight"), W16(c, "temb.p.l1.bias"), ws.tmp, B, (int)D, d.pooled_dim, 1, 0, st));
    HIP_TRY(launch_gemv(ws.tmp, W16(c, "temb.p.l2.weight"), W16(c, "temb.p.l2.bias"), ws.temb, B, (int)D, (int)D, 0, 1, st));
  }
  HIP_TRY(launch_silu(ws.temb, ws.semb, (int64_t)B * D, st));
  HIP_TRY(launch_gemv(ws.semb, W16(c, "mod.weight"), W16(c, "mod.bias"), ws.mod, B, (int)c->n_mod, (int)D, 0, 0, st, ldm));
  if (W16(c, "mod_final.weight") != nullptr)
    HIP_TRY(launch_gemv(ws.semb, W16(c, "mod_final.weight"), W16(c, "mod_final.bias"), ws.mod + ml.fin(0), B, (int)(2 * D),
                        (int)D, 0, 0, st, ldm));
  }
  if (stage != 2) {
  const uint16_t* ctx_src = (const uint16_t*)ctx_emb;
  if (d.family == 1) {
    HIP_TRY(launch_norm_modulate(ctx_src, d.joint_dim, ws.F, d.joint_dim, B * T, d.joint_dim,
                                 W32(c, "txt_norm.weight"), nullptr, 0, B * T, 1, st));
    ctx_src = ws.F;
  }
  {
    GemmBatch gb{};
    for (int b = 0; b < B; ++b) {
      GemmProblem& pi = gb.p[gb.nprob++];
      pi = GemmProblem{};
      pi.A = (const uint16_t*)x + (int64_t)b * N * d.in_channels; pi.lda = d.in_channels;
      pi.W = W16(c, "x_in.weight"); pi.ldw = d.in_channels; pi.bias = W16(c, "x_in.bias");
      pi.C = ws.X + ((int64_t)b * S + T) * D; pi.ldc = D; pi.M = N; pi.N = (int)D; pi.K = d.in_channels;
      GemmProblem& pt = gb.p[gb.nprob++];
      pt = GemmProblem{};
      pt.A = ctx_src + (int64_t)b * T * d.joint_dim; pt.lda = d.joint_dim;
      pt.W = W16(c, "ctx_in.weight"); pt.ldw = d.joint_dim; pt.bias = W16(c, "ctx_in.bias");
      pt.C = ws.X + (int64_t)b * S * D; pt.ldc = D; pt.M = T; pt.N = (int)D; pt.K = d.joint_dim;
    }
    { ProfScope ps_(c, st, 0, gemm_flops(gb)); HIP_TRY(launch_gemm(gb, st)); }
  }
  }
  if (stage == 1) return AFX_OK;

  if (c->fp8 && c->fp8_mx < 0) {
    const char* e = getenv("AFX_FP8_MX");
    c->fp8_mx = (e && e[0] == '0') ? 0 : 1;
  }
  const bool mx = c->fp8 && c->fp8_mx == 1 && D % 512 == 0 && gemm_fp8_mx_ok(R, (int)D, (int)D);
  if (mx) HIP_TRY(hipMemsetD32Async((hipDeviceptr_t)ws.ones, 0x3f800000, (size_t)R, st));
  const bool norm_rows = mx && getenv("AFX_FP8_NORM_MX") == nullptr;
  const bool attn_mx = mx && H * 128 == D && getenv("AFX_FP8_ATTN_MX_OFF") == nullptr;
  const char* qkf8 = getenv("AFX_FP8_QK_FUSE");
  const bool qk_fuse_fp8 = mx && qkf8 != nullptr && qkf8[0] == '1';
  const BlockShape bs = block_shape(H, B, N, T, rope_cos, rope_sin, ws.Vt);
  const int dpath = qkv_path(bs, false, c->fp8, qk_fuse_fp8), spath = qkv_path(bs, true, c->fp8, qk_fuse_fp8);
  const int split_txt_default = 0;
  auto stream_gemm = [&](const uint16_t* A, int64_t lda, int K, const LinW (&lw)[2], uint16_t* C, int64_t ldc, int Nout, int epi,
                         int blk, int gate_chunk, const float* qkn = nullptr, int mx_in = 0, bool mx_out = false, int kind = 0) -> int {
    GemmBatch gb{};
    if (mx && mx_in == 0) HIP_TRY(launch_quant_rows_mx8(A, lda, ws.q8n, K, ws.mxn, ws.ld_mxn, (int)R, K, st));
    else if (c->fp8 && !mx) HIP_TRY(launch_quant_rows_fp8(A, lda, ws.q8, K, ws.qs, (int)R, K, st));
    for (int b = 0; b < B; ++b)
      for (int s = 0; s < 2; ++s) {
        GemmProblem& p = gb.p[gb.nprob++];
        stream_problem(p, bs, A, lda, K, lw[s], C, ldc, Nout, b, s);
        const int64_t row0 = (int64_t)b * S + (s == 0 ? T : 0);
        if (mx) {
          p.W = (const uint16_t*)lw[s].wq; p.fp8 = 1; p.a_scale = ws.ones + row0; p.w_scale = lw[s].wscale; p.lda = K;
          if (mx_in == 2 && norm_rows) { p.A = (const uint16_t*)(ws.q8n + row0 * K); p.a_scale = ws.qs + row0; }
          else if (mx_in != 1) { p.A = (const uint16_t*)(ws.q8n + row0 * K); p.a_mx = ws.mxn + row0 * ws.ld_mxn; p.ld_mx = ws.ld_mxn; }
          else { p.A = (const uint16_t*)(ws.q8 + row0 * K); p.a_mx = ws.mxw + row0 * ws.ld_mxw; p.ld_mx = ws.ld_mxw; }
          if (mx_out) { p.c8 = ws.q8 + row0 * Nout; p.ldc8 = Nout; p.c_mx = ws.mxw + row0 * ws.ld_mxw; p.ld_cmx = ws.ld_mxw; p.c8_col0 = 0; }
        } else if (c->fp8) {
          p.A = (const uint16_t*)(ws.q8 + row0 * K); p.lda = K;
          p.W = (const uint16_t*)lw[s].wq; p.fp8 = 1; p.a_scale = ws.qs + row0; p.w_scale = lw[s].wscale;
        }
        p.epi = epi; p.gelu_col0 = 0;
        if (qkn != nullptr) stream_qk_epilogue(p, bs, qkn, s);
        if (epi == EPI_GATE_RES) {
          p.gate = ws.mod + (int64_t)b * ldm + ml.dbl(blk, s, gate_chunk); p.ldg = 0; p.rows_per_batch = 1 << 30;
          p.res = C + row0 * ldc; p.ldr = ldc;
        }
      }
    static int split_env = -2;
    if (split_env == -2) {
      const char* e = getenv("AFX_SPLIT_TXT");
      split_env = e ? atoi(e) : -1;
    }
    const int split_mask = split_env >= 0 ? split_env : split_txt_default;
    if ((split_mask & kind) != 0 && T > 0 && N > 0 && !mx && !c->fp8) {
      GemmBatch gi{}, gt{};
      for (int j = 0; j < gb.nprob; ++j) ((j & 1) ? gt : gi).p[((j & 1) ? gt : gi).nprob++] = gb.p[j];
      { ProfScope ps_(c, st, 0, gemm_flops(gi)); HIP_TRY(launch_gemm(gi, st)); }
      { ProfScope ps_(c, st, 0, gemm_flops(gt)); HIP_TRY(launch_gemm(gt, st)); }
      return AFX_OK;
    }
    { ProfScope ps_(c, st, 0, gemm_flops(gb)); HIP_TRY(launch_gemm(gb, st)); }
    return AFX_OK;
  };
  bool norm_fused = false;
  auto stream_norm = [&](int blk, int shift_chunk, int scale_chunk) -> int {
    norm_fused = false;
    if (mx) {
      HIP_TRY(launch_norm_modulate_mx8(ws.X, D, ws.q8n, D, ws.mxn, ws.ld_mxn, (int)R, (int)D, ws.mod + ml.dbl(blk, 0, scale_chunk),
                                       ws.mod + ml.dbl(blk, 0, shift_chunk), ws.mod + ml.dbl(blk, 1, scale_chunk),
                                       ws.mod + ml.dbl(blk, 1, shift_chunk), ldm, (int)S, T, st, &norm_fused, norm_rows ? ws.qs : nullptr));
      if (norm_fused) return AFX_OK;
    }
    HIP_TRY(launch_norm_modulate_joint(ws.X, D, ws.Xn, D, (int)R, (int)D, ws.mod + ml.dbl(blk, 0, scale_chunk),
                                       ws.mod + ml.dbl(blk, 0, shift_chunk), ws.mod + ml.dbl(blk, 1, scale_chunk),
                                       ws.mod + ml.dbl(blk, 1, shift_chunk), ldm, S, T, st));
    return AFX_OK;
  };

  int rc;
  uint16_t* QKV = ws.F;
  uint16_t* Hb = ws.F + R * 3 * D;
  for (int i = 0; stage == 0 && i < d.num_double; ++i) {
    const DoubleW& bw = c->dbl[i];
    const float* qkn = bw.qkn;
    if (c->ckpt) HIP_TRY(hipMemcpyAsync(c->ckpt + (int64_t)i * R * D, ws.X, (size_t)R * D * 2, hipMemcpyDeviceToDevice, st));
    if ((rc = stream_norm(i, 0, 1))) return rc;
    if (dpath == AFX_QKV_VT_PROJ) {
      for (int b = 0; b < B; ++b) {
        GemmBatch gb{};
        double_vt_batch(gb, bs, ws.Xn, D, bw.qkv, QKV, 3 * D, qkn, b);
        { ProfScope ps_(c, st, 0, gemm_flops(gb)); HIP_TRY(launch_gemm(gb, st)); }
      }
    } else
    if ((rc = stream_gemm(ws.Xn, D, (int)D, bw.qkv, QKV, 3 * D, (int)(3 * D), EPI_NONE, i, 0, dpath == AFX_QKV_QK_EPI ? qkn : nullptr,
                          norm_fused ? 2 : 0, false, 1))) return rc;
    HIP_TRY(qkv_finish(dpath, bs, QKV, 3 * D, qkn + 3 * 128, qkn + 1 * 128, qkn + 2 * 128, qkn, st));
    bool o_fused = false;
    const AttnMx8 omx_d{ws.q8n, D, ws.mxn, ws.ld_mxn};
    { ProfScope ps_(c, st, 1, 4.0 * B * H * (double)S * S * 128);
      HIP_TRY(launch_attention(QKV + 2 * D, 3 * D, QKV, 3 * D, ws.Vt, QKV + 2 * D, 3 * D, B, H, S, st, nullptr, attn_mx ? &omx_d : nullptr, &o_fused)); }
    if ((rc = stream_gemm(QKV + 2 * D, 3 * D, (int)D, bw.out, ws.X, D, (int)D, EPI_GATE_RES, i, 2, nullptr, o_fused ? 3 : 0, false, 2))) return rc;
    if ((rc = stream_norm(i, 3, 4))) return rc;
    if ((rc = stream_gemm(ws.Xn, D, (int)D, bw.mlp1, Hb, 4 * D, (int)(4 * D), EPI_GELU, i, 0, nullptr, norm_fused ? 2 : 0, mx, 4))) return rc;
    if ((rc = stream_gemm(Hb, 4 * D, (int)(4 * D), bw.mlp2, ws.X, D, (int)D, EPI_GATE_RES, i, 5, nullptr, mx ? 1 : 0, false, 8))) return rc;
  }

  for (int i = 0; stage == 0 && i < d.num_single; ++i) {
    const SingleW& bw = c->sgl[i];
    const float* qkn = bw.qkn;
    if (c->ckpt)
      HIP_TRY(hipMemcpyAsync(c->ckpt + (int64_t)(d.num_double + i) * R * D, ws.X, (size_t)R * D * 2, hipMemcpyDeviceToDevice, st));
    bool sgl_fused = false;
    if (mx) HIP_TRY(launch_norm_modulate_mx8(ws.X, D, ws.q8n, D, ws.mxn, ws.ld_mxn, (int)R, (int)D, ws.mod + ml.sgl(i, 1), ws.mod + ml.sgl(i, 0),
                                             nullptr, nullptr, ldm, (int)S, 0, st, &sgl_fused, norm_rows ? ws.qs : nullptr));
    if (!sgl_fused) HIP_TRY(launch_norm_modulate(ws.X, D, ws.Xn, D, (int)R, (int)D, ws.mod + ml.sgl(i, 1), ws.mod + ml.sgl(i, 0), ldm, S, 0, st));
    GemmBatch gb{};
    single_qkv_batch(gb, spath, bs, ws.Xn, D, bw.fused, ws.F, 7 * D, qkn);
    GemmProblem& f = gb.p[0];
    if (mx) {
      if (!sgl_fused) HIP_TRY(launch_quant_rows_mx8(ws.Xn, D, ws.q8n, D, ws.mxn, ws.ld_mxn, (int)R, (int)D, st));
      f.A = (const uint16_t*)ws.q8n; f.W = (const uint16_t*)bw.fused.wq; f.fp8 = 1; f.a_scale = ws.ones; f.w_scale = bw.fused.wscale;
      if (sgl_fused && norm_rows) f.a_scale = ws.qs;
      else { f.a_mx = ws.mxn; f.ld_mx = ws.ld_mxn; }
      f.c8 = ws.q8 + D; f.ldc8 = 5 * D; f.c_mx = ws.mxw + D / 128; f.ld_cmx = ws.ld_mxw; f.c8_col0 = (int)(3 * D);
    } else if (c->fp8) {
      HIP_TRY(launch_quant_rows_fp8(ws.Xn, D, ws.q8, D, ws.qs, (int)R, (int)D, st));
      f.A = (const uint16_t*)ws.q8; f.W = (const uint16_t*)bw.fused.wq; f.fp8 = 1; f.a_scale = ws.qs; f.w_scale = bw.fused.wscale;
    }
    { ProfScope ps_(c, st, 0, gemm_flops(gb)); HIP_TRY(launch_gemm(gb, st)); }
    HIP_TRY(qkv_finish(spath, bs, ws.F, 7 * D, qkn + 128, qkn + 128, qkn, qkn, st));
    bool o_fused = false;
    const AttnMx8 omx_s{ws.q8, 5 * D, ws.mxw, ws.ld_mxw};
    { ProfScope ps_(c, st, 1, 4.0 * B * H * (double)S * S * 128);
      HIP_TRY(launch_attention(ws.F + 2 * D, 7 * D, ws.F, 7 * D, ws.Vt, ws.F + 2 * D, 7 * D, B, H, S, st, nullptr, attn_mx ? &omx_s : nullptr, &o_fused)); }
    GemmBatch go{};
    go.nprob = 1;
    GemmProblem& o = go.p[0];
    o = GemmProblem{};
    o.A = ws.F + 2 * D; o.lda = 7 * D; o.W = bw.out.w; o.ldw = 5 * D; o.bias = bw.out.b;
    o.C = ws.X; o.ldc = D; o.M = (int)R; o.N = (int)D; o.K = (int)(5 * D); o.epi = EPI_GATE_RES;
    o.gate = ws.mod + ml.sgl(i, 2); o.ldg = ldm; o.rows_per_batch = S; o.res = ws.X; o.ldr = D;
    if (mx) {
      if (!o_fused) HIP_TRY(launch_quant_rows_mx8(ws.F + 2 * D, 7 * D, ws.q8, 5 * D, ws.mxw, ws.ld_mxw, (int)R, (int)D, st));
      o.A = (const uint16_t*)ws.q8; o.lda = 5 * D; o.W = (const uint16_t*)bw.out.wq; o.fp8 = 1; o.a_scale = ws.ones; o.w_scale = bw.out.wscale;
      o.a_mx = ws.mxw; o.ld_mx = ws.ld_mxw;
    } else if (c->fp8) {
      HIP_TRY(launch_quant_rows_fp8(ws.F + 2 * D, 7 * D, ws.q8, 5 * D, ws.qs, (int)R, (int)(5 * D), st));
      o.A = (const uint16_t*)ws.q8; o.lda = 5 * D; o.W = (const uint16_t*)bw.out.wq; o.fp8 = 1; o.a_scale = ws.qs;
      o.w_scale = bw.out.wscale;
    }
    { ProfScope ps_(c, st, 0, gemm_flops(go)); HIP_TRY(launch_gemm(go, st)); }
  }

  for (int b = 0; b < B; ++b)
    HIP_TRY(launch_norm_modulate(ws.X + ((int64_t)b * S + T) * D, D, ws.Xn + (int64_t)b * N * D, D, N, (int)D,
                                 ws.mod + (int64_t)b * ldm + ml.fin(0), ws.mod + (int64_t)b * ldm + ml.fin(1), 0,
                                 1 << 30, 0, st));
  {
    GemmBatch gb{};
    gb.nprob = 1;
    GemmProblem& hp = gb.p[0];
    hp = GemmProblem{};
    hp.A = ws.Xn; hp.lda = D; hp.W = W16(c, "head.weight"); hp.ldw = D; hp.bias = W16(c, "head.bias");
    hp.M = B * N; hp.N = c->head_n; hp.K = (int)D; hp.epi = EPI_NONE;
    if (d.head_mode == 0) {
      hp.C = ws.head; hp.ldc = c->head_n;
    } else {
      hp.C = (uint16_t*)means; hp.ldc = c->head_n;
    }
    { ProfScope ps_(c, st, 0, gemm_flops(gb)); HIP_TRY(launch_gemm(gb, st)); }
  }
  if (d.head_mode == 0)
    HIP_TRY(launch_head_split(ws.head, c->head_n, (uint16_t*)means, (uint16_t*)logw, (uint16_t*)logg, (int64_t)B * N,
                              d.num_gaussians, d.in_channels, d.logweights_channels, st));
  return AFX_OK;
}

int afx_mmdit_prepare_steps(afx_ctx* c, const void* pooled, const float* t_steps, const float* g, int32_t B, int32_t nsteps,
                            void* stream_) {
  if (!c || !t_steps) return fail(AFX_E_INVALID, "null argument to afx_mmdit_prepare_steps");
  if (!c->finalized) return fail(AFX_E_MISSING, "afx_finalize() has not succeeded on this context");
  const afx_model_desc& d = c->d;
  if (B < 1 || nsteps < 1 || B > AFX_MAX_MICRO_BATCH || (int64_t)B * nsteps > AFX_PREP_ROWS)
    return fail(AFX_E_INVALID, "afx_mmdit_prepare_steps: batch <= 4 and batch * steps <= %d", AFX_PREP_ROWS);
  if (d.guidance_embeds && !g) return fail(AFX_E_INVALID, "guidance vector required");
  if (d.pooled_dim > 0 && !pooled) return fail(AFX_E_INVALID, "pooled projections required");
  if (c->temb_override) return fail(AFX_E_INVALID, "afx_mmdit_prepare_steps: not with a timestep-embedding override");
  Workspace ws = carve(c, c->ws, 1, 1, 1);
  if (!c->ws || ws.total > c->ws_bytes) return fail(AFX_E_WORKSPACE, "workspace not set / too small");
  hipStream_t st = (hipStream_t)stream_;
  const int64_t D = c->D, ldm = c->n_mod;
  const int rows = B * nsteps;
  c->prep_steps = 0;
  c->prep_use = -1;
  float* sc = ws.prep_semb;
  for (int k = 0; k < nsteps; ++k) {
    float* temb = ws.prep_temb + (int64_t)k * B * D;
    float* hid = sc + (int64_t)k * B * D;
    float* sin_ = ws.prep_mod;
    HIP_TRY(launch_sincos(t_steps + (int64_t)k * B, 1000.0f, sin_, B, d.family == 0 ? 1 : 2, st));
    HIP_TRY(launch_gemv(sin_, W16(c, "temb.t.l1.weight"), W16(c, "temb.t.l1.bias"), hid, B, (int)D, 256, 1, 0, st));
    HIP_TRY(launch_gemv(hid, W16(c, "temb.t.l2.weight"), W16(c, "temb.t.l2.bias"), temb, B, (int)D, (int)D, 0, 0, st));
    if (d.guidance_embeds) {
      HIP_TRY(launch_sincos(g, 1000.0f, sin_, B, 1, st));
      HIP_TRY(launch_gemv(sin_, W16(c, "temb.g.l1.weight"), W16(c, "temb.g.l1.bias"), hid, B, (int)D, 256, 1, 0, st));
      HIP_TRY(launch_gemv(hid, W16(c, "temb.g.l2.weight"), W16(c, "temb.g.l2.bias"), temb, B, (int)D, (int)D, 0, 1, st));
    }
    if (d.pooled_dim > 0) {
      HIP_TRY(launch_bf16_to_f32((const uint16_t*)pooled, sin_, (int64_t)B * d.pooled_dim, st));
      HIP_TRY(launch_gemv(sin_, W16(c, "temb.p.l1.weight"), W16(c, "temb.p.l1.bias"), hid, B, (int)D, d.pooled_dim, 1, 0, st));
      HIP_TRY(launch_gemv(hid, W16(c, "temb.p.l2.weight"), W16(c, "temb.p.l2.bias"), temb, B, (int)D, (int)D, 0, 1, st));
    }
  }
  HIP_TRY(launch_silu(ws.prep_temb, ws.prep_semb, (int64_t)rows * D, st));
  HIP_TRY(launch_gemv(ws.prep_semb, W16(c, "mod.weight"), W16(c, "mod.bias"), ws.prep_mod, rows, (int)c->n_mod, (int)D, 0, 0, st, ldm));
  if (W16(c, "mod_final.weight") != nullptr) {
    ModLayout ml{D, d.num_double, d.num_single};
    HIP_TRY(launch_gemv(ws.prep_semb, W16(c, "mod_final.weight"), W16(c, "mod_final.bias"), ws.prep_mod + ml.fin(0), rows, (int)(2 * D),
                        (int)D, 0, 0, st, ldm));
  }
  c->prep_steps = nsteps;
  c->prep_B = B;
  return AFX_OK;
}

int afx_mmdit_use_prepared_step(afx_ctx* c, int32_t k) {
  if (!c) return fail(AFX_E_INVALID, "null ctx");
  if (k >= c->prep_steps) return fail(AFX_E_INVALID, "afx_mmdit_use_prepared_step: step %d of %d prepared", k, c->prep_steps);
  c->prep_use = k < 0 ? -1 : k;
  return AFX_OK;
}

int afx_set_fp8_linear(afx_ctx* c, int32_t on) {
  if (!c) return fail(AFX_E_INVALID, "null ctx");
  if (on) {
    const int64_t D = c->D;
    int r;
    auto chk = [&](const std::string& n, int64_t out_f, int64_t in_f) -> int {
      if ((r = need(c, n + ".weight_q", AFX_DT_FP8, {out_f, in_f})) != AFX_OK) return r;
      return need(c, n + ".wscale", AFX_DT_F32, {out_f});
    };
    for (int i = 0; i < c->d.num_double; ++i)
      for (const char* s : {"img_", "txt_"}) {
        const std::string p = "d" + std::to_string(i) + "." + s;
        if ((r = chk(p + "qkv", 3 * D, D)) || (r = chk(p + "out", D, D)) || (r = chk(p + "mlp1", 4 * D, D)) || (r = chk(p + "mlp2", D, 4 * D))) return r;
      }
    for (int i = 0; i < c->d.num_single; ++i) {
      const std::string p = "s" + std::to_string(i) + ".";
      if ((r = chk(p + "fused", 7 * D, D)) || (r = chk(p + "out", D, 5 * D))) return r;
    }
  }
  c->fp8 = on != 0;
  return AFX_OK;
}

int afx_set_temb_override(afx_ctx* ctx, const float* temb_t) {
  if (!ctx) return fail(AFX_E_INVALID, "null ctx");
  ctx->temb_override = temb_t;
  return AFX_OK;
}

int afx_set_checkpoint_buffer(afx_ctx* ctx, void* dptr) {
  if (!ctx) return fail(AFX_E_INVALID, "null ctx");
  ctx->ckpt = (uint16_t*)dptr;
  return AFX_OK;
}

int afx_profile_enable(afx_ctx* ctx, int32_t on) {
  if (!ctx) return fail(AFX_E_INVALID, "null ctx");
  ctx->prof_on = on != 0;
  ctx->prof_stride = on > 1 ? on : 1;
  ctx->prof_count = 0;
  ctx->prof_used = 0;
  return AFX_OK;
}

int afx_profile_read(afx_ctx* ctx, int32_t klass, double* total_ms, int64_t* launches, double* flops) {
  if (!ctx || !total_ms || !launches || !flops) return fail(AFX_E_INVALID, "null argument to afx_profile_read");
  double ms = 0, fl = 0;
  int64_t n = 0;
  for (size_t i = 0; i < ctx->prof_used; ++i) {
    auto& r = ctx->prof_pool[i];
    if (r.klass != klass) continue;
    HIP_TRY(hipEventSynchronize(r.b));
    float t = 0;
    HIP_TRY(hipEventElapsedTime(&t, r.a, r.b));
    ms += t; fl += r.flops; ++n;
  }
  *total_ms = ms; *launches = n; *flops = fl;
  return AFX_OK;
}

int afx_arcflow_step(const float* x_in, const void* means, const void* logw, const void* logg, int32_t mix_dtype,
                     float sigma_src, float sigma_start, float sigma_end, const float* sigma_vec, float eps,
                     float* x_out, int32_t batch, int32_t n_tok, int32_t K, int32_t ch, int32_t pp, void* stream) {
  if (!x_in || !means || !logw || !logg || !x_out) return fail(AFX_E_INVALID, "null argument to afx_arcflow_step");
  if (mix_dtype != AFX_DT_BF16 && mix_dtype != AFX_DT_F32) return fail(AFX_E_INVALID, "bad mix_dtype");
  if (batch < 0 || n_tok < 0 || K < 1 || K > 32 || ch < 1 || pp < 1 || ch % pp != 0)
    return fail(AFX_E_INVALID, "bad shape for afx_arcflow_step");
  HIP_TRY(launch_arcflow_step(x_in, means, logw, logg, mix_dtype == AFX_DT_BF16, sigma_src, sigma_start, sigma_end,
                              sigma_vec, eps, x_out, batch, n_tok, K, ch, pp, 0, nullptr, (hipStream_t)stream));
  return AFX_OK;
}

int afx_arcflow_step_dropout(const float* x_in, const void* means, const void* logw, const void* logg, int32_t mix_dtype,
                             const float* sigma_vec, const uint8_t* drop_mask, float eps, float* x_out, int32_t batch,
                             int32_t n_tok, int32_t K, int32_t ch, int32_t pp, void* stream) {
  if (!x_in || !means || !logw || !logg || !x_out || !sigma_vec)
    return fail(AFX_E_INVALID, "null argument to afx_arcflow_step_dropout");
  if (mix_dtype != AFX_DT_BF16 && mix_dtype != AFX_DT_F32) return fail(AFX_E_INVALID, "bad mix_dtype");
  if (batch < 0 || n_tok < 0 || K < 1 || K > 32 || ch < 1 || pp < 1 || ch % pp != 0)
    return fail(AFX_E_INVALID, "bad shape for afx_arcflow_step_dropout");
  HIP_TRY(launch_arcflow_step(x_in, means, logw, logg, mix_dtype == AFX_DT_BF16, 0.f, 0.f, 0.f, sigma_vec, eps, x_out,
                              batch, n_tok, K, ch, pp, 0, drop_mask, (hipStream_t)stream));
  return AFX_OK;
}

int afx_linear_tn_f32out(const void* X, int64_t ldx, const void* Y, int64_t ldy, float* C, int64_t ldc, int32_t M, int32_t N1, int32_t N2,
                         int32_t accumulate, void* stream) {
  if (!X || !Y || !C) return fail(AFX_E_INVALID, "null argument to afx_linear_tn_f32out");
  if (M < 0 || N1 < 0 || N2 < 0 || N1 % 8 || N2 % 8 || ldx % 8 || ldy % 8 || ldc % 4 || ldx < N1 || ldy < N2 || ldc < N2)
    return fail(AFX_E_INVALID, "afx_linear_tn_f32out: need N1%%8==0, N2%%8==0, ldx/ldy%%8==0, ldc%%4==0, leading dimensions >= the widths");
  if (((uintptr_t)X | (uintptr_t)Y | (uintptr_t)C) & 15) return fail(AFX_E_INVALID, "afx_linear_tn_f32out: operands must be 16-byte aligned");
  HIP_TRY(launch_gemm_tn_f32((const uint16_t*)X, ldx, (const uint16_t*)Y, ldy, C, ldc, M, N1, N2, accumulate, (hipStream_t)stream));
  return AFX_OK;
}

int64_t afx_linear_tn_ws_bytes(int32_t M, int32_t N1, int32_t N2) {
  if (M < 0 || N1 < 0 || N2 < 0) return fail(AFX_E_INVALID, "bad shape to afx_linear_tn_ws_bytes");
  return gemm_tn_ws_bytes(M, N1, N2);
}

int afx_linear_tn_f32out_ws(const void* X, int64_t ldx, const void* Y, int64_t ldy, float* C, int64_t ldc, int32_t M, int32_t N1, int32_t N2,
                            int32_t accumulate, void* ws, void* stream) {
  if (!X || !Y || !C) return fail(AFX_E_INVALID, "null argument to afx_linear_tn_f32out_ws");
  if (M < 0 || N1 < 0 || N2 < 0 || N1 % 8 || N2 % 8 || ldx % 8 || ldy % 8 || ldc % 4 || ldx < N1 || ldy < N2 || ldc < N2)
    return fail(AFX_E_INVALID, "afx_linear_tn_f32out_ws: need N1%%8==0, N2%%8==0, ldx/ldy%%8==0, ldc%%4==0, leading dimensions >= the widths");
  if (((uintptr_t)X | (uintptr_t)Y | (uintptr_t)C | (uintptr_t)ws) & 15) return fail(AFX_E_INVALID, "afx_linear_tn_f32out_ws: operands must be 16-byte aligned");
  if (!ws && gemm_tn_ws_bytes(M, N1, N2) > 0) return fail(AFX_E_INVALID, "afx_linear_tn_f32out_ws: this shape needs afx_linear_tn_ws_bytes() of workspace");
  HIP_TRY(launch_gemm_tn_f32((const uint16_t*)X, ldx, (const uint16_t*)Y, ldy, C, ldc, M, N1, N2, accumulate, (hipStream_t)stream, (float*)ws));
  return AFX_OK;
}

int afx_linear_bf16_f32out(const void* A, int64_t lda, const void* W, int64_t ldw, float* C, int64_t ldc, int32_t M,
                           int32_t N, int32_t K, int32_t accumulate, void* stream) {
  if (!A || !W || !C) return fail(AFX_E_INVALID, "null argument to afx_linear_bf16_f32out");
  if (M < 0 || N < 0 || K <= 0 || K % 64 || N % 8 || lda % 8 || ldw % 8 || ldc % 4)
    return fail(AFX_E_INVALID, "afx_linear_bf16_f32out: need K%%64==0, N%%8==0, lda/ldw%%8==0, ldc%%4==0");
  GemmBatch gb{};
  gb.nprob = 1;
  GemmProblem& p = gb.p[0];
  p = GemmProblem{};
  p.A = (const uint16_t*)A; p.lda = lda; p.W = (const uint16_t*)W; p.ldw = ldw; p.C = (uint16_t*)C; p.ldc = ldc;
  p.M = M; p.N = N; p.K = K; p.epi = EPI_NONE; p.rows_per_batch = 1; p.out_f32 = accumulate ? 2 : 1;
  HIP_TRY(launch_gemm(gb, (hipStream_t)stream));
  return AFX_OK;
}

int afx_mmdit_import_tokens(afx_ctx* c, const void* src, int32_t batch, int32_t n_img, int32_t n_txt, void* stream) {
  if (!c || !src || !c->ws || batch < 1 || n_img < 1 || n_txt < 0) return fail(AFX_E_INVALID, "bad argument to afx_mmdit_import_tokens");
  Workspace ws = carve(c, c->ws, batch, n_img, n_txt);
  if (ws.total > c->ws_bytes)
    return fail(AFX_E_WORKSPACE, "afx_mmdit_import_tokens: shape (%d, %d, %d) needs %lld workspace bytes, have %lld", batch, n_img, n_txt,
                (long long)ws.total, (long long)c->ws_bytes);
  HIP_TRY(hipMemcpyAsync(ws.X, src, (size_t)batch * (n_img + n_txt) * c->D * 2, hipMemcpyDeviceToDevice, (hipStream_t)stream));
  return AFX_OK;
}

int afx_linear_splitk_chunks(int32_t M, int32_t N, int32_t K, int32_t split_k) {
  const int tiles = ((M + 255) / 256) * ((N + 255) / 256), nk = K / 64;
  if (split_k <= 0) {
    split_k = (512 + tiles / 2) / tiles;
    if (split_k > nk / 4) split_k = nk / 4;
    if (split_k < 1) split_k = 1;
  }
  split_k = split_k < nk ? split_k : nk;
  const int per = (nk + split_k - 1) / split_k;
  return (nk + per - 1) / per;
}

int afx_linear_bf16_splitk(const void* A, int64_t lda, const void* W, int64_t ldw, const void* bias, float* partials, int32_t M,
                           int32_t N, int32_t K, int32_t split_k, void* stream) {
  if (!A || !W || !partials) return fail(AFX_E_INVALID, "null argument to afx_linear_bf16_splitk");
  if (M < 0 || N < 0 || K <= 0 || K % 64 || N % 8 || lda % 8 || ldw % 8 || split_k < 0)
    return fail(AFX_E_INVALID, "afx_linear_bf16_splitk: need K%%64==0, N%%8==0, lda/ldw%%8==0, split_k >= 0");
  GemmBatch gb{};
  gb.nprob = 1;
  GemmProblem& p = gb.p[0];
  p = GemmProblem{};
  p.A = (const uint16_t*)A; p.lda = lda; p.W = (const uint16_t*)W; p.ldw = ldw; p.bias = (const uint16_t*)bias; p.C = (uint16_t*)partials;
  p.ldc = N; p.M = M; p.N = N; p.K = K; p.epi = EPI_NONE; p.rows_per_batch = 1; p.out_f32 = 3;
  p.split_k = afx_linear_splitk_chunks(M, N, K, split_k);
  p.split_stride = (int64_t)M * N;
  HIP_TRY(launch_gemm(gb, (hipStream_t)stream));
  return AFX_OK;
}

int afx_mmdit_export(afx_ctx* c, const char* what, void* dst, int32_t batch, int32_t n_img, int32_t n_txt, void* stream) {
  if (!c || !what || !dst || !c->ws || batch < 1 || n_img < 1 || n_txt < 0) return fail(AFX_E_INVALID, "bad argument to afx_mmdit_export");
  Workspace ws = carve(c, c->ws, batch, n_img, n_txt);
  if (ws.total > c->ws_bytes)
    return fail(AFX_E_WORKSPACE, "afx_mmdit_export: shape (%d, %d, %d) needs %lld workspace bytes, have %lld", batch, n_img, n_txt,
                (long long)ws.total, (long long)c->ws_bytes);
  const int64_t D = c->D;
  ModLayout ml{D, c->d.num_double, c->d.num_single};
  hipStream_t st = (hipStream_t)stream;
  const std::string w(what);
  if (w == "head_in") {
    HIP_TRY(hipMemcpyAsync(dst, ws.Xn, (size_t)batch * n_img * D * 2, hipMemcpyDeviceToDevice, st));
  } else if (w == "x_final") {
    for (int b = 0; b < batch; ++b)
      HIP_TRY(hipMemcpyAsync((char*)dst + (size_t)b * n_img * D * 2, ws.X + ((int64_t)b * (n_img + n_txt) + n_txt) * D,
                             (size_t)n_img * D * 2, hipMemcpyDeviceToDevice, st));
  } else if (w == "x_tokens") {
    HIP_TRY(hipMemcpyAsync(dst, ws.X, (size_t)batch * (n_img + n_txt) * D * 2, hipMemcpyDeviceToDevice, st));
  } else if (w == "temb") {
    HIP_TRY(hipMemcpyAsync(dst, ws.temb, (size_t)batch * D * 4, hipMemcpyDeviceToDevice, st));
  } else if (w == "silu_temb") {
    HIP_TRY(hipMemcpyAsync(dst, ws.semb, (size_t)batch * D * 4, hipMemcpyDeviceToDevice, st));
  } else if (w == "mod_all") {
    HIP_TRY(hipMemcpyAsync(dst, ws.mod, (size_t)batch * c->n_mod * 4, hipMemcpyDeviceToDevice, st));
  } else if (w == "mod_final") {
    for (int b = 0; b < batch; ++b)
      HIP_TRY(hipMemcpyAsync((char*)dst + (size_t)b * 2 * D * 4, ws.mod + (int64_t)b * c->n_mod + ml.fin(0), (size_t)2 * D * 4,
                             hipMemcpyDeviceToDevice, st));
  } else {
    return fail(AFX_E_INVALID, "afx_mmdit_export: unknown buffer '%s'", what);
  }
  return AFX_OK;
}

int afx_arcflow_velocity(const void* means, const void* logw, const void* logg, int32_t mix_dtype, float sigma_src,
                         float sigma_t, const float* sigma_vec, float* u_out, int32_t batch, int32_t n_tok,
                         int32_t K, int32_t ch, int32_t pp, void* stream) {
  if (!means || !logw || !logg || !u_out) return fail(AFX_E_INVALID, "null argument to afx_arcflow_velocity");
  if (mix_dtype != AFX_DT_BF16 && mix_dtype != AFX_DT_F32) return fail(AFX_E_INVALID, "bad mix_dtype");
  if (batch < 0 || n_tok < 0 || K < 1 || K > 32 || ch < 1 || pp < 1 || ch % pp != 0)
    return fail(AFX_E_INVALID, "bad shape for afx_arcflow_velocity");
  HIP_TRY(launch_arcflow_step(u_out, means, logw, logg, mix_dtype == AFX_DT_BF16, sigma_src, sigma_t, sigma_t,
                              sigma_vec, 1e-4f, u_out, batch, n_tok, K, ch, pp, 1, nullptr, (hipStream_t)stream));
  return AFX_OK;
}

int afx_linear_bf16(const void* A, int64_t lda, const void* W, int64_t ldw, const void* bias, void* C, int64_t ldc,
                    int32_t M, int32_t N, int32_t K, int32_t epi, int32_t gelu_col0, const float* gate,
                    int64_t ldg, int32_t rows_per_batch, const void* res, int64_t ldr, void* stream) {
  return afx_linear_bf16_pre(A, lda, W, ldw, bias, C, ldc, M, N, K, epi, gelu_col0, gate, ldg, rows_per_batch, res, ldr, nullptr, 0,
                             stream);
}

int afx_gemm_dropres_available(void) { return gemm_dropres_available() ? 1 : 0; }
int afx_gemm_set_mode(int32_t impl, int32_t tile) {
  gemm_set_mode(impl, tile);
  return 0;
}
int afx_gemm_set_fp8_tile(int32_t tile) { return gemm_set_fp8_tile(tile); }
int afx_attn_set_impl(int32_t impl) {
  attn_set_impl(impl);
  return 0;
}
int afx_attn_bwd_set_impl(int32_t impl) {
  attn_bwd_set_impl(impl);
  return 0;
}

int afx_linear_bf16_pre(const void* A, int64_t lda, const void* W, int64_t ldw, const void* bias, void* C, int64_t ldc,
                        int32_t M, int32_t N, int32_t K, int32_t epi, int32_t gelu_col0, const float* gate,
                        int64_t ldg, int32_t rows_per_batch, const void* res, int64_t ldr, const void* pre, int64_t ldp,
                        void* stream) {
  if (!A || !W || !C) return fail(AFX_E_INVALID, "null argument to afx_linear_bf16");
  if (pre && ldp % 8) return fail(AFX_E_INVALID, "afx_linear_bf16_pre: ldp %% 8 == 0");
  if (M < 0 || N < 0 || K <= 0 || K % 64 || N % 8 || lda % 8 || ldw % 8 || ldc % 8)
    return fail(AFX_E_INVALID, "afx_linear_bf16: need K%%64==0, N%%8==0, strides%%8==0");
  if (epi < 0 || epi > 2) return fail(AFX_E_INVALID, "bad epilogue");
  if (epi == EPI_GATE_RES && (!res || ldr % 8 || (gate && rows_per_batch < 1)))
    return fail(AFX_E_INVALID, "gated residual epilogue needs res (and rows_per_batch with a gate)");
  GemmBatch gb{};
  gb.nprob = 1;
  GemmProblem& p = gb.p[0];
  p = GemmProblem{};
  p.A = (const uint16_t*)A; p.lda = lda; p.W = (const uint16_t*)W; p.ldw = ldw; p.bias = (const uint16_t*)bias;
  p.C = (uint16_t*)C; p.ldc = ldc; p.M = M; p.N = N; p.K = K; p.epi = epi; p.gelu_col0 = gelu_col0;
  p.gate = gate; p.ldg = ldg; p.rows_per_batch = rows_per_batch > 0 ? rows_per_batch : 1; p.res = (const uint16_t*)res; p.ldr = ldr;
  p.pre = (const uint16_t*)pre; p.ldp = ldp;
  HIP_TRY(launch_gemm(gb, (hipStream_t)stream));
  return AFX_OK;
}

int afx_linear_bf16_dropres(const void* A, int64_t lda, const void* W, int64_t ldw, void* C, int64_t ldc, int32_t M, int32_t N, int32_t K,
                            const void* res, int64_t ldr, float p, uint32_t seed, int64_t row0, void* stream) {
  if (!A || !W || !C || !res) return fail(AFX_E_INVALID, "null argument to afx_linear_bf16_dropres");
  if (M < 0 || N < 0 || K <= 0 || K % 64 || N % 8 || lda % 8 || ldw % 8 || ldc % 8 || ldr % 8 || !(p >= 0.f && p < 1.f))
    return fail(AFX_E_INVALID, "afx_linear_bf16_dropres: need K%%64==0, N%%8==0, strides%%8==0, 0 <= p < 1");
  GemmBatch gb{};
  gb.nprob = 1;
  GemmProblem& q = gb.p[0];
  q = GemmProblem{};
  q.A = (const uint16_t*)A; q.lda = lda; q.W = (const uint16_t*)W; q.ldw = ldw; q.C = (uint16_t*)C; q.ldc = ldc; q.M = M; q.N = N; q.K = K;
  q.epi = EPI_GATE_RES; q.rows_per_batch = M > 0 ? M : 1; q.res = (const uint16_t*)res; q.ldr = ldr;
  q.drop_on = 1; q.drop_thresh = (uint32_t)((double)p * 4294967296.0); q.drop_seed = seed; q.drop_inv_keep = 1.0f / (1.0f - p); q.drop_row0 = row0;
  HIP_TRY(launch_gemm(gb, (hipStream_t)stream));
  return AFX_OK;
}

int64_t afx_attention_ws_bytes(int32_t batch, int32_t heads, int32_t S) {
  if (batch < 1 || heads < 1 || S < 1) return fail(AFX_E_INVALID, "bad attention shape");
  return (int64_t)batch * heads * 128 * attn_spad(S) * 2;
}

int afx_attention_bf16(const void* q, int64_t ldq, const void* k, int64_t ldk, const void* v, int64_t ldv, void* o,
                       int64_t ldo, void* vt_ws, int32_t batch, int32_t heads, int32_t S, void* stream) {
  if (!q || !k || !v || !o || !vt_ws) return fail(AFX_E_INVALID, "null argument to afx_attention_bf16");
  if (batch < 1 || heads < 1 || S < 1 || ldq % 8 || ldk % 8 || ldv % 8 || ldo % 4)
    return fail(AFX_E_INVALID, "bad attention shape / stride");
  HIP_TRY(launch_v_transpose((const uint16_t*)v, ldv, (uint16_t*)vt_ws, batch, heads, S, (hipStream_t)stream));
  HIP_TRY(launch_attention((const uint16_t*)q, ldq, (const uint16_t*)k, ldk, (const uint16_t*)vt_ws, (uint16_t*)o, ldo,
                           batch, heads, S, (hipStream_t)stream));
  return AFX_OK;
}

int64_t afx_attention_bwd_ws_bytes(int32_t batch, int32_t heads, int32_t S) {
  if (batch < 1 || heads < 1 || S < 1) return fail(AFX_E_INVALID, "bad attention shape");
  return attn_bwd_ws_bytes(batch, heads, S);
}

int afx_attention_fwd_lse_bf16(const void* q, int64_t ldq, const void* k, int64_t ldk, const void* v, int64_t ldv, void* o,
                               int64_t ldo, float* lse, void* vt_ws, int32_t batch, int32_t heads, int32_t S, void* stream) {
  if (!q || !k || !v || !o || !vt_ws || !lse) return fail(AFX_E_INVALID, "null argument to afx_attention_fwd_lse_bf16");
  if (batch < 1 || heads < 1 || S < 1 || ldq % 8 || ldk % 8 || ldv % 8 || ldo % 4) return fail(AFX_E_INVALID, "bad attention shape / stride");
  HIP_TRY(launch_v_transpose((const uint16_t*)v, ldv, (uint16_t*)vt_ws, batch, heads, S, (hipStream_t)stream));
  HIP_TRY(launch_attention((const uint16_t*)q, ldq, (const uint16_t*)k, ldk, (const uint16_t*)vt_ws, (uint16_t*)o, ldo,
                           batch, heads, S, (hipStream_t)stream, lse));
  return AFX_OK;
}

int afx_attention_to_mx8(const void* q, int64_t ldq, const void* k, int64_t ldk, const void* v, int64_t ldv, void* o8, int64_t ldo8,
                         void* mx, int64_t ld_mx, void* vt_ws, int32_t batch, int32_t heads, int32_t S, void* stream) {
  if (!q || !k || !v || !o8 || !mx || !vt_ws) return fail(AFX_E_INVALID, "null argument to afx_attention_to_mx8");
  if (batch < 1 || heads < 1 || S < 1 || ldq % 8 || ldk % 8 || ldv % 8 || ldo8 % 8 || ld_mx < heads) return fail(AFX_E_INVALID, "bad attention shape / stride");
  if (!attention_v3_eligible(S)) return fail(AFX_E_INVALID, "afx_attention_to_mx8: S > 64 (the one-wave-per-SIMD kernel's epilogue)");
  HIP_TRY(launch_v_transpose((const uint16_t*)v, ldv, (uint16_t*)vt_ws, batch, heads, S, (hipStream_t)stream));
  const AttnMx8 m{(uint8_t*)o8, ldo8, (uint8_t*)mx, ld_mx};
  bool fused = false;
  HIP_TRY(launch_attention((const uint16_t*)q, ldq, (const uint16_t*)k, ldk, (const uint16_t*)vt_ws, nullptr, 0, batch, heads, S, (hipStream_t)stream,
                           nullptr, &m, &fused));
  if (!fused) return fail(AFX_E_INVALID, "afx_attention_to_mx8: the one-wave-per-SIMD attention kernel is switched off (AFX_ATTN_IMPL)");
  return AFX_OK;
}

int afx_attention_bwd_bf16(const void* q, int64_t ldq, const void* k, int64_t ldk, const void* v, int64_t ldv, const void* o,
                           int64_t ldo, const void* dout, int64_t lddo, const float* lse, void* dq, int64_t lddq, void* dk,
                           int64_t lddk, void* dv, int64_t lddv, void* ws, int32_t batch, int32_t heads, int32_t S,
                           void* stream) {
  if (!q || !k || !v || !o || !dout || !lse || !dq || !dk || !dv || !ws) return fail(AFX_E_INVALID, "null argument to afx_attention_bwd_bf16");
  if (batch < 1 || heads < 1 || S < 1 || ldq % 8 || ldk % 8 || ldv % 8 || ldo % 8 || lddo % 8 || lddq % 4 || lddk % 4 || lddv % 4)
    return fail(AFX_E_INVALID, "bad attention backward shape / stride");
  HIP_TRY(launch_attention_backward((const uint16_t*)q, ldq, (const uint16_t*)k, ldk, (const uint16_t*)v, ldv,
                                    (const uint16_t*)o, ldo, (const uint16_t*)dout, lddo, lse, (uint16_t*)dq, lddq,
                                    (uint16_t*)dk, lddk, (uint16_t*)dv, lddv, ws, batch, heads, S, (hipStream_t)stream));
  return AFX_OK;
}

int afx_norm_modulate_bf16(const void* x, int64_t ldx, void* out, int64_t ldo, int32_t rows, int32_t D,
                           const float* scale, const float* shift, int64_t ldmod, int32_t rows_per_batch, int32_t rms,
                           void* stream) {
  if (!x || !out || !scale || (!rms && !shift)) return fail(AFX_E_INVALID, "null argument to afx_norm_modulate_bf16");
  if (rows < 0 || D < 8 || D % 8 || D > 4096 || ldx % 8 || ldo % 8) return fail(AFX_E_INVALID, "bad norm shape");
  HIP_TRY(launch_norm_modulate((const uint16_t*)x, ldx, (uint16_t*)out, ldo, rows, D, scale, shift, ldmod,
                               rows_per_batch, rms, (hipStream_t)stream));
  return AFX_OK;
}

int afx_qk_norm_rope_bf16(void* x, int64_t ldx, const float* w_txt, const float* w_img, const float* rope_cos,
                          const float* rope_sin, int32_t batch, int32_t S, int32_t n_txt, int32_t heads, void* stream) {
  if (!x || !w_txt || !w_img || !rope_cos || !rope_sin) return fail(AFX_E_INVALID, "null argument to afx_qk_norm_rope_bf16");
  if (batch < 1 || S < 1 || heads < 1 || ldx % 8) return fail(AFX_E_INVALID, "bad qk_norm_rope shape");
  HIP_TRY(launch_qk_norm_rope((uint16_t*)x, ldx, w_txt, w_img, rope_cos, rope_sin, batch, S, n_txt, heads,
                              (hipStream_t)stream));
  return AFX_OK;
}

int afx_gemv_bf16(const float* x, const void* W, const void* bias, float* y, int32_t B, int32_t N, int32_t K,
                  int32_t act, int32_t accumulate, void* stream) {
  if (!x || !W || !y) return fail(AFX_E_INVALID, "null argument to afx_gemv_bf16");
  if (B < 1 || B > 8 || N < 1 || K < 8 || K % 8) return fail(AFX_E_INVALID, "bad gemv shape (B<=8, K%%8==0)");
  HIP_TRY(launch_gemv(x, (const uint16_t*)W, (const uint16_t*)bias, y, B, N, K, act, accumulate, (hipStream_t)stream));
  return AFX_OK;
}

int afx_qkv_operands(int32_t kind, const void* A, int64_t lda, const void* w_img, const void* b_img, const void* w_txt, const void* b_txt,
                     const float* qkn, const float* rope_cos, const float* rope_sin, int32_t B, int32_t N, int32_t T, int32_t heads,
                     int32_t path, void* F, int64_t ldf, void* Vt, void* stream) {
  if (kind != AFX_BLOCK_DOUBLE && kind != AFX_BLOCK_SINGLE) return fail(AFX_E_INVALID, "afx_qkv_operands: kind must be AFX_BLOCK_DOUBLE or AFX_BLOCK_SINGLE");
  const bool single = kind == AFX_BLOCK_SINGLE;
  if (!A || !w_img || !qkn || !rope_cos || !rope_sin || !F || !Vt || (!single && !w_txt) || (!single && (!b_img) != (!b_txt)))
    return fail(AFX_E_INVALID, "null argument to afx_qkv_operands");
  if (B < 1 || B > AFX_MAX_MICRO_BATCH || N < 1 || T < 1 || heads < 1 || path < AFX_QKV_AUTO || path > AFX_QKV_KV_PREP)
    return fail(AFX_E_INVALID, "afx_qkv_operands: need 1 <= batch <= %d, n_img, n_txt, heads >= 1 and a path AFX_QKV_*", AFX_MAX_MICRO_BATCH);
  const int64_t D = (int64_t)heads * 128, width = (single ? 7 : 3) * D;
  if (lda < D || ldf < width || lda % 8 || ldf % 8)
    return fail(AFX_E_INVALID, "afx_qkv_operands: need lda >= %lld, ldf >= %lld, both multiples of 8", (long long)D, (long long)width);
  if (((uintptr_t)A | (uintptr_t)w_img | (uintptr_t)b_img | (uintptr_t)w_txt | (uintptr_t)b_txt | (uintptr_t)qkn | (uintptr_t)rope_cos |
       (uintptr_t)rope_sin | (uintptr_t)F | (uintptr_t)Vt) & 15)
    return fail(AFX_E_INVALID, "afx_qkv_operands: operands must be 16-byte aligned");
  const BlockShape bs = block_shape(heads, B, N, T, rope_cos, rope_sin, (uint16_t*)Vt);
  const int p = path == AFX_QKV_AUTO ? qkv_path(bs, single, false, false) : path;
  if (p != AFX_QKV_KV_PREP && !gemm_qk_fusion_available())
    return fail(AFX_E_INVALID, "afx_qkv_operands: the GEMM kernel in use has no q / k epilogue (afx_gemm_set_mode / AFX_QK_FUSE)");
  if (p == AFX_QKV_VT_PROJ && !vt_proj_shape_ok(bs, single))
    return fail(AFX_E_INVALID, "afx_qkv_operands: V^T from the projection needs n_txt %% 16 == 0 and (n_img + n_txt) %% 64 == 0");
  hipStream_t st = (hipStream_t)stream;
  const uint16_t* a = (const uint16_t*)A;
  uint16_t* f = (uint16_t*)F;
  if (single) {
    LinW lw;
    lw.w = (const uint16_t*)w_img; lw.b = (const uint16_t*)b_img;
    GemmBatch gb{};
    single_qkv_batch(gb, p, bs, a, lda, lw, f, ldf, qkn);
    HIP_TRY(launch_gemm(gb, st));
    HIP_TRY(qkv_finish(p, bs, f, ldf, qkn + 128, qkn + 128, qkn, qkn, st));
    return AFX_OK;
  }
  LinW lw[2];
  lw[0].w = (const uint16_t*)w_img; lw[0].b = (const uint16_t*)b_img;
  lw[1].w = (const uint16_t*)w_txt; lw[1].b = (const uint16_t*)b_txt;
  if (p == AFX_QKV_VT_PROJ) {
    for (int b = 0; b < B; ++b) {
      GemmBatch gb{};
      double_vt_batch(gb, bs, a, lda, lw, f, ldf, qkn, b);
      HIP_TRY(launch_gemm(gb, st));
    }
    return AFX_OK;
  }
  GemmBatch gb{};
  for (int b = 0; b < B; ++b)
    for (int s = 0; s < 2; ++s) {
      GemmProblem& pr = gb.p[gb.nprob++];
      stream_problem(pr, bs, a, lda, (int)D, lw[s], f, ldf, (int)width, b, s);
      if (p == AFX_QKV_QK_EPI) stream_qk_epilogue(pr, bs, qkn, s);
    }
  HIP_TRY(launch_gemm(gb, st));
  HIP_TRY(qkv_finish(p, bs, f, ldf, qkn + 3 * 128, qkn + 1 * 128, qkn + 2 * 128, qkn, st));
  return AFX_OK;
}

static int norm_joint_args(const char* fn, const void* x, int64_t ldx, int64_t ldo, int32_t rows, int32_t D, const float* scale, const float* shift,
                           const float* scale_txt, const float* shift_txt, int64_t ldmod, int32_t S, int32_t n_txt) {
  if (!x || !scale || !shift || (!scale_txt) != (!shift_txt)) return fail(AFX_E_INVALID, "null argument to %s", fn);
  if (rows < 0 || D < 8 || D % 8 || D > 4096 || ldx < D || ldx % 8 || ldo < D || ldo % 8 || ldmod < 0 || ldmod % 4 || S < 1 || n_txt < 0 ||
      n_txt > S || (!scale_txt && n_txt != 0))
    return fail(AFX_E_INVALID, "%s: need D %% 8 == 0, D <= 4096, ldx / ldo >= D and multiples of 8, ldmod %% 4 == 0, 0 <= n_txt <= S "
                "(n_txt 0 without text vectors)", fn);
  if (((uintptr_t)x | (uintptr_t)scale | (uintptr_t)shift | (uintptr_t)scale_txt | (uintptr_t)shift_txt) & 15)
    return fail(AFX_E_INVALID, "%s: operands must be 16-byte aligned", fn);
  return AFX_OK;
}

int afx_norm_modulate_joint_bf16(const void* x, int64_t ldx, void* out, int64_t ldo, int32_t rows, int32_t D, const float* scale,
                                 const float* shift, const float* scale_txt, const float* shift_txt, int64_t ldmod, int32_t S,
                                 int32_t n_txt, void* stream) {
  int r = norm_joint_args("afx_norm_modulate_joint_bf16", x, ldx, ldo, rows, D, scale, shift, scale_txt, shift_txt, ldmod, S, n_txt);
  if (r != AFX_OK) return r;
  if (!out || ((uintptr_t)out & 15)) return fail(AFX_E_INVALID, "afx_norm_modulate_joint_bf16: out null or not 16-byte aligned");
  HIP_TRY(launch_norm_modulate_joint((const uint16_t*)x, ldx, (uint16_t*)out, ldo, rows, D, scale, shift, scale_txt, shift_txt, ldmod, S, n_txt,
                                     (hipStream_t)stream));
  return AFX_OK;
}

int afx_norm_modulate_mx8(const void* x, int64_t ldx, void* q8, int64_t ldq, void* mx, int64_t ld_mx, float* rowscale, int32_t rows, int32_t D,
                          const float* scale, const float* shift, const float* scale_txt, const float* shift_txt, int64_t ldmod, int32_t S,
                          int32_t n_txt, int32_t* fused, void* stream) {
  int r = norm_joint_args("afx_norm_modulate_mx8", x, ldx, ldq, rows, D, scale, shift, scale_txt, shift_txt, ldmod, S, n_txt);
  if (r != AFX_OK) return r;
  if (!q8 || !fused || ((uintptr_t)q8 & 7) || (!rowscale && (!mx || ld_mx < (D + 127) / 128 || ld_mx % 4)) || ((uintptr_t)rowscale & 3))
    return fail(AFX_E_INVALID, "afx_norm_modulate_mx8: need q8 (8-byte aligned), fused, and rowscale or mx with ld_mx >= D / 128, ld_mx %% 4 == 0");
  bool f = false;
  HIP_TRY(launch_norm_modulate_mx8((const uint16_t*)x, ldx, (uint8_t*)q8, ldq, (uint8_t*)mx, ld_mx, rows, D, scale, shift, scale_txt, shift_txt,
                                   ldmod, S, n_txt, (hipStream_t)stream, &f, rowscale));
  *fused = f ? 1 : 0;
  return AFX_OK;
}

}
```

arcflow_amd/ops.py:

```python
from __future__ import annotations

import ctypes as C
from typing import Optional, Tuple

import torch

from . import _lib


def _p(t: Optional[torch.Tensor]):
    return None if t is None else C.c_void_p(t.data_ptr())


def _s():
    return C.c_void_p(torch.cuda.current_stream().cuda_stream)


def _cuda(t: torch.Tensor, dtype) -> torch.Tensor:
    if t.device.type != 'cuda':
        raise _lib.ArcflowHipError('arcflow_amd.ops works on GPU tensors only (no CPU fallback)')
    return t.to(dtype).contiguous()


def _mat(t: torch.Tensor, dtype, name: str, shape=None) -> torch.Tensor:
    if t.device.type != 'cuda':
        raise _lib.ArcflowHipError(f'{name}: arcflow_amd.ops works on GPU tensors only (no CPU fallback)')
    if t.dim() != 2 or t.dtype != dtype or (t.shape[1] > 1 and t.stride(1) != 1):
        raise ValueError(f'{name}: need a 2-D {dtype} tensor with unit inner stride, got {tuple(t.shape)} {t.dtype} strides {t.stride()}')
    if shape is not None and tuple(t.shape) != tuple(shape):
        raise ValueError(f'{name}: shape {tuple(t.shape)} != {tuple(shape)}')
    return t


def _acc(t: torch.Tensor, shape, name: str) -> torch.Tensor:
    if t.device.type != 'cuda':
        raise _lib.ArcflowHipError(f'{name}: arcflow_amd.ops works on GPU tensors only (no CPU fallback)')
    if t.dtype != torch.float32 or not t.is_contiguous() or tuple(t.shape) != tuple(shape):
        raise ValueError(f'{name}: need a contiguous float32 accumulator of shape {tuple(shape)}, got {tuple(t.shape)} {t.dtype} '
                         f'strides {t.stride()}')
    return t


def _rows_f32(v: torch.Tensor, R: int, C: int, rows_per_batch: int, name: str) -> torch.Tensor:
    if v.device.type != 'cuda':
        raise _lib.ArcflowHipError(f'{name}: arcflow_amd.ops works on GPU tensors only (no CPU fallback)')
    if v.dim() == 1:
        v = v[None]
    if v.dim() != 2 or v.shape[1] != C:
        raise ValueError(f'{name}: need [{C}] or [batch, {C}], got {tuple(v.shape)}')
    if not (v.dtype == torch.float32 and v.stride(1) == 1 and v.stride(0) % 4 == 0 and v.data_ptr() % 16 == 0):
        v = v.to(torch.float32).contiguous()
    if rows_per_batch > 0:
        if R != rows_per_batch * v.shape[0]:
            raise ValueError(f'{name}: {R} rows != rows_per_batch {rows_per_batch} x {v.shape[0]} {name} rows')
    elif v.shape[0] != 1:
        raise ValueError(f'{name}: {v.shape[0]} {name} rows need rows_per_batch')
    return v


def linear(a: torch.Tensor, w: torch.Tensor, bias: Optional[torch.Tensor] = None, epilogue: str = 'none',
           gelu_col0: int = 0, gate: Optional[torch.Tensor] = None, residual: Optional[torch.Tensor] = None,
           rows_per_batch: int = 0, out: Optional[torch.Tensor] = None, pre: Optional[torch.Tensor] = None) -> torch.Tensor:
    lib = _lib.load()
    assert a.dtype == torch.bfloat16 and w.dtype == torch.bfloat16 and a.stride(-1) == 1 and w.stride(-1) == 1
    M, K = a.shape
    N = w.shape[0]
    if out is None:
        out = torch.empty(M, N, dtype=torch.bfloat16, device=a.device)
    epi = {'none': 0, 'gelu': 1, 'gate_res': 2}[epilogue]
    if gate is not None:
        gate = _cuda(gate, torch.float32)
        if gate.dim() == 1:
            gate = gate[None]
    rpb = rows_per_batch if rows_per_batch > 0 else max(M, 1)
    _lib.check(lib.afx_linear_bf16_pre(_p(a), a.stride(0), _p(w), w.stride(0), _p(bias), _p(out), out.stride(0), M, N, K,
                                       epi, gelu_col0, _p(gate), 0 if gate is None else gate.stride(0), rpb,
                                       _p(residual), 0 if residual is None else residual.stride(0),
                                       _p(pre), 0 if pre is None else pre.stride(0), _s()))
    return out


def set_gemm_mode(impl: int = 3, tile: int = 0) -> None:
    _lib.check(_lib.load().afx_gemm_set_mode(impl, tile))


def set_fp8_tile(tile: int = 0) -> int:
    return _lib.load().afx_gemm_set_fp8_tile(tile)


def set_attn_impl(impl: int = 0) -> None:
    _lib.check(_lib.load().afx_attn_set_impl(impl))


def set_attn_bwd_impl(impl: int = 3) -> None:
    _lib.check(_lib.load().afx_attn_bwd_set_impl(impl))


def lora_dropout(src: torch.Tensor, p: float, seed: int, row0: int = 0, mode: int = 0, out: Optional[torch.Tensor] = None) -> torch.Tensor:
    lib = _lib.load()
    M, N = src.shape
    if out is None:
        assert mode < 2
        out = torch.empty(M, N, dtype=torch.bfloat16, device=src.device)
    _lib.check(lib.afx_lora_dropout_bf16(_p(src), src.stride(0), _p(out), out.stride(0), M, N, row0, float(p), int(seed) & 0xffffffff, mode, _s()))
    return out


def attention(q: torch.Tensor, k: torch.Tensor, v: torch.Tensor) -> torch.Tensor:
    lib = _lib.load()
    B, S, H, Dh = q.shape
    assert Dh == 128 and q.dtype == torch.bfloat16
    q2, k2, v2 = (t.reshape(B * S, H * Dh) for t in (q.contiguous(), k.contiguous(), v.contiguous()))
    o = torch.empty(B * S, H * Dh, dtype=torch.bfloat16, device=q.device)
    ws = torch.empty(lib.afx_attention_ws_bytes(B, H, S), dtype=torch.uint8, device=q.device)
    _lib.check(lib.afx_attention_bf16(_p(q2), H * Dh, _p(k2), H * Dh, _p(v2), H * Dh, _p(o), H * Dh, _p(ws), B, H, S, _s()))
    return o.reshape(B, S, H * Dh)


def attention_to_mx8(q: torch.Tensor, k: torch.Tensor, v: torch.Tensor, out=None):
    lib = _lib.load()
    B, S, H, Dh = q.shape
    assert Dh == 128 and q.dtype == torch.bfloat16
    q2, k2, v2 = (t.reshape(B * S, H * Dh) for t in (q.contiguous(), k.contiguous(), v.contiguous()))
    if out is None:
        o8 = torch.empty(B * S, H * Dh, dtype=torch.uint8, device=q.device)
        mx = torch.empty(B * S, (H + 3) // 4 * 4, dtype=torch.uint8, device=q.device)
    else:
        o8, mx = out
        assert o8.shape == (B * S, H * Dh) and mx.shape[0] == B * S and mx.shape[1] >= H and o8.dtype == mx.dtype == torch.uint8
        assert o8.stride(1) == 1 and mx.stride(1) == 1 and o8.stride(0) % 16 == 0 and mx.stride(0) % 4 == 0
    ws = torch.empty(lib.afx_attention_ws_bytes(B, H, S), dtype=torch.uint8, device=q.device)
    _lib.check(lib.afx_attention_to_mx8(_p(q2), H * Dh, _p(k2), H * Dh, _p(v2), H * Dh, _p(o8), o8.stride(0), _p(mx), mx.stride(0), _p(ws), B, H, S, _s()))
    return o8, mx[:, :H]


def norm_modulate(x: torch.Tensor, scale: torch.Tensor, shift: Optional[torch.Tensor], rows_per_batch: int = 0,
                  rms: bool = False, out: Optional[torch.Tensor] = None) -> torch.Tensor:
    lib = _lib.load()
    R, D = x.shape
    if out is None:
        out = torch.empty(R, D, dtype=torch.bfloat16, device=x.device)
    scale = _cuda(scale, torch.float32)
    shift = None if shift is None else _cuda(shift, torch.float32)
    ldm = 0 if rms or scale.dim() == 1 else scale.stride(0)
    _lib.check(lib.afx_norm_modulate_bf16(_p(x), x.stride(0), _p(out), out.stride(0), R, D, _p(scale), _p(shift), ldm,
                                          rows_per_batch if rows_per_batch > 0 else max(R, 1), int(rms), _s()))
    return out


def qk_norm_rope_(x: torch.Tensor, w_txt: torch.Tensor, w_img: torch.Tensor, cos: torch.Tensor, sin: torch.Tensor,
                  n_txt: int) -> torch.Tensor:
    lib = _lib.load()
    B, S, H, Dh = x.shape
    assert x.is_contiguous() and Dh == 128
    _lib.check(lib.afx_qk_norm_rope_bf16(_p(x), H * Dh, _p(_cuda(w_txt, torch.float32)), _p(_cuda(w_img, torch.float32)),
                                         _p(_cuda(cos, torch.float32)), _p(_cuda(sin, torch.float32)), B, S, n_txt, H, _s()))
    return x


def _joint_vectors(vecs, B: int, D: int, name: str) -> int:
    ld = None
    for v, n in vecs:
        if v.device.type != 'cuda':
            raise _lib.ArcflowHipError(f'{name} {n}: arcflow_amd.ops works on GPU tensors only (no CPU fallback)')
        v2 = v[None] if v.dim() == 1 else v
        if v2.dim() != 2 or tuple(v2.shape) != (B, D) or v2.dtype != torch.float32 or v2.stride(1) != 1 or v2.data_ptr() % 16:
            raise ValueError(f'{name} {n}: need a [{B}, {D}] float32 tensor with unit inner stride and 16-byte aligned rows, got '
                             f'{tuple(v.shape)} {v.dtype} strides {v.stride()}')
        s = v2.stride(0) if B > 1 else 0
        if s % 4 or (ld is not None and s != ld):
            raise ValueError(f'{name} {n}: every modulation vector needs the same row stride (a multiple of 4), got {v2.stride(0)}')
        ld = s
    return ld


def _joint_norm_args(x, scale, shift, S, scale_txt, shift_txt, n_txt, name):
    _mat(x, torch.bfloat16, f'{name} x')
    R, D = x.shape
    if S < 1 or R % S:
        raise ValueError(f'{name}: {R} rows are not a whole number of samples of S = {S}')
    if (scale_txt is None) != (shift_txt is None) or not 0 <= n_txt <= S or (scale_txt is None and n_txt):
        raise ValueError(f'{name}: text vectors need both scale_txt and shift_txt and 0 <= n_txt <= S (n_txt 0 without them)')
    vecs = [(scale, 'scale'), (shift, 'shift')] + ([] if scale_txt is None else [(scale_txt, 'scale_txt'), (shift_txt, 'shift_txt')])
    return R, D, _joint_vectors(vecs, R // S, D, name)


def norm_modulate_joint(x, scale, shift, S: int, scale_txt=None, shift_txt=None, n_txt: int = 0, out=None):
    lib = _lib.load()
    R, D, ldm = _joint_norm_args(x, scale, shift, S, scale_txt, shift_txt, n_txt, 'norm_modulate_joint')
    if out is None:
        out = torch.empty(R, D, dtype=torch.bfloat16, device=x.device)
    _mat(out, torch.bfloat16, 'norm_modulate_joint out', (R, D))
    _lib.check(lib.afx_norm_modulate_joint_bf16(_p(x), x.stride(0), _p(out), out.stride(0), R, D, _p(scale), _p(shift), _p(scale_txt),
                                                _p(shift_txt), ldm, S, n_txt, _s()))
    return out


def norm_modulate_mx8(x, scale, shift, S: int, scale_txt=None, shift_txt=None, n_txt: int = 0, row_scale: bool = False):
    lib = _lib.load()
    R, D, ldm = _joint_norm_args(x, scale, shift, S, scale_txt, shift_txt, n_txt, 'norm_modulate_mx8')
    q = torch.empty(R, D, dtype=torch.uint8, device=x.device)
    nb = (D + 127) // 128
    mx = None if row_scale else torch.empty(R, (nb + 3) // 4 * 4, dtype=torch.uint8, device=x.device)
    rs = torch.empty(R, dtype=torch.float32, device=x.device) if row_scale else None
    fused = C.c_int32(0)
    _lib.check(lib.afx_norm_modulate_mx8(_p(x), x.stride(0), _p(q), D, _p(mx), 0 if mx is None else mx.stride(0), _p(rs), R, D, _p(scale),
                                         _p(shift), _p(scale_txt), _p(shift_txt), ldm, S, n_txt, C.byref(fused), _s()))
    return q, (rs if row_scale else mx[:, :nb]), bool(fused.value)


def qkv_operands(kind: str, a, w, bias, qkn, cos, sin, B: int, N: int, T: int, path: str = 'auto', out=None, vt=None):
    lib = _lib.load()
    if kind not in ('double', 'single') or path not in _lib.AFX_QKV_PATHS:
        raise ValueError(f'qkv_operands: kind {kind!r} / path {path!r}')
    single = kind == 'single'
    S = N + T
    _mat(a, torch.bfloat16, 'qkv_operands a')
    R, D = a.shape
    if D % 128 or R != B * S:
        raise ValueError(f'qkv_operands a: need [{B} x {S}, heads x 128], got {tuple(a.shape)}')
    H, width = D // 128, (7 if single else 3) * D
    ws = (w,) if single else tuple(w)
    bs = (bias,) if single else ((None, None) if bias is None else tuple(bias))
    if len(ws) != (1 if single else 2) or len(bs) != len(ws):
        raise ValueError('qkv_operands: a double block takes (w_img, w_txt) and (b_img, b_txt) or None')
    for i, t in enumerate(ws):
        _mat(t, torch.bfloat16, f'qkv_operands w[{i}]', ((width, D)))
        if not t.is_contiguous():
            raise ValueError(f'qkv_operands w[{i}]: the weight rows must be contiguous (row stride D)')
    for i, t in enumerate(bs):
        if t is not None and (t.device.type != 'cuda' or t.dtype != torch.bfloat16 or not t.is_contiguous() or tuple(t.shape) != (width,)):
            raise ValueError(f'qkv_operands bias[{i}]: need a contiguous bf16 [{width}] tensor')
    if sum(t is None for t in bs) not in (0, len(bs)):
        raise ValueError('qkv_operands: both streams with a bias or neither')
    for t, n, shp in ((qkn, 'qkn', (2 if single else 4, 128)), (cos, 'cos', (S, 64)), (sin, 'sin', (S, 64))):
        if t.device.type != 'cuda' or t.dtype != torch.float32 or not t.is_contiguous() or tuple(t.shape) != shp:
            raise ValueError(f'qkv_operands {n}: need a contiguous float32 {list(shp)} tensor, got {tuple(t.shape)} {t.dtype}')
    S_pad = (S + 63) // 64 * 64
    if out is None:
        out = torch.empty(R, width, dtype=torch.bfloat16, device=a.device)
    _mat(out, torch.bfloat16, 'qkv_operands out', (R, width))
    if vt is None:
        vt = torch.empty(B, H, 128, S_pad, dtype=torch.bfloat16, device=a.device)
    if vt.device.type != 'cuda' or vt.dtype != torch.bfloat16 or not vt.is_contiguous() or tuple(vt.shape) != (B, H, 128, S_pad):
        raise ValueError(f'qkv_operands vt: need a contiguous bf16 [{B}, {H}, 128, {S_pad}] workspace, got {tuple(vt.shape)} {vt.dtype}')
    w_img, w_txt = ws[0], (None if single else ws[1])
    b_img, b_txt = bs[0], (None if single else bs[1])
    _lib.check(lib.afx_qkv_operands(_lib.AFX_BLOCK_SINGLE if single else _lib.AFX_BLOCK_DOUBLE, _p(a), a.stride(0), _p(w_img), _p(b_img),
                                    _p(w_txt), _p(b_txt), _p(qkn), _p(cos), _p(sin), B, N, T, H, _lib.AFX_QKV_PATHS[path], _p(out),
                                    out.stride(0), _p(vt), _s()))
    return out, vt


def gemv(x: torch.Tensor, w: torch.Tensor, bias: Optional[torch.Tensor] = None, act: str = 'none',
         out: Optional[torch.Tensor] = None, accumulate: bool = False) -> torch.Tensor:
    lib = _lib.load()
    x = _cuda(x, torch.float32)
    B, K = x.shape
    N = w.shape[0]
    if out is None:
        out = torch.zeros(B, N, dtype=torch.float32, device=x.device)
    _lib.check(lib.afx_gemv_bf16(_p(x), _p(w), _p(bias), _p(out), B, N, K, 1 if act == 'silu' else 0, int(accumulate), _s()))
    return out


def _mix_dtype(means, logw, logg) -> Tuple[int, torch.Tensor, torch.Tensor, torch.Tensor]:
    if means.dtype == torch.bfloat16:
        return _lib.AFX_DT_BF16, means.contiguous(), logw.to(torch.bfloat16).contiguous(), logg.to(torch.bfloat16).contiguous()
    return _lib.AFX_DT_F32, means.float().contiguous(), logw.float().contiguous(), logg.float().contiguous()


def arcflow_step(x: torch.Tensor, means: torch.Tensor, logw: torch.Tensor, logg: torch.Tensor, sigma_src, sigma_start,
                 sigma_end, eps: float = 1e-4, out: Optional[torch.Tensor] = None) -> torch.Tensor:
    lib = _lib.load()
    B, N, K, ch = means.shape
    pp = logw.shape[-1]
    x = _cuda(x, torch.float32)
    dt, means, logw, logg = _mix_dtype(means, logw, logg)
    if out is None:
        out = torch.empty_like(x)
    sv = None
    if any(isinstance(s, torch.Tensor) and s.numel() > 1 for s in (sigma_src, sigma_start, sigma_end)):
        cols = [torch.as_tensor(s, dtype=torch.float32, device=x.device).flatten().expand(B) for s in (sigma_src, sigma_start, sigma_end)]
        sv = torch.stack(cols, dim=1).contiguous()
        s0 = s1 = s2 = 0.0
    else:
        s0, s1, s2 = (float(s) for s in (sigma_src, sigma_start, sigma_end))
    _lib.check(lib.afx_arcflow_step(_p(x), _p(means), _p(logw), _p(logg), dt, s0, s1, s2, _p(sv), eps, _p(out),
                                    B, N, K, ch, pp, _s()))
    return out


def arcflow_velocity(means: torch.Tensor, logw: torch.Tensor, logg: torch.Tensor, sigma_src, sigma_t) -> torch.Tensor:
    lib = _lib.load()
    B, N, K, ch = means.shape
    pp = logw.shape[-1]
    dt, means, logw, logg = _mix_dtype(means, logw, logg)
    out = torch.empty(B, N, ch, dtype=torch.float32, device=means.device)
    sv = None
    if any(isinstance(s, torch.Tensor) and s.numel() > 1 for s in (sigma_src, sigma_t)):
        cols = [torch.as_tensor(s, dtype=torch.float32, device=out.device).flatten().expand(B) for s in (sigma_src, sigma_t, sigma_t)]
        sv = torch.stack(cols, dim=1).contiguous()
        s0 = s1 = 0.0
    else:
        s0, s1 = float(sigma_src), float(sigma_t)
    _lib.check(lib.afx_arcflow_velocity(_p(means), _p(logw), _p(logg), dt, s0, s1, _p(sv), _p(out), B, N, K, ch, pp, _s()))
    return out


def _sigma_vec(B, device, *sig):
    cols = [torch.as_tensor(x, dtype=torch.float32, device=device).flatten().expand(B) for x in sig]
    return torch.stack(cols, dim=1).contiguous()


def arcflow_step_dropout(x, means, logw, logg, sigma_src, sigma_start, sigma_end, drop_mask=None, eps: float = 1e-4):
    lib = _lib.load()
    B, N, K, ch = means.shape
    pp = logw.shape[-1]
    x = _cuda(x, torch.float32)
    dt, means, logw, logg = _mix_dtype(means, logw, logg)
    sv = _sigma_vec(B, x.device, sigma_src, sigma_start, sigma_end)
    dm = None if drop_mask is None else drop_mask.to(device=x.device, dtype=torch.uint8).reshape(B, K).contiguous()
    out = torch.empty_like(x)
    _lib.check(lib.afx_arcflow_step_dropout(_p(x), _p(means), _p(logw), _p(logg), dt, _p(sv), _p(dm), eps, _p(out),
                                            B, N, K, ch, pp, _s()))
    return out


def arcflow_backward(g, means, logw, logg, sigma_src, sigma_start, sigma_end, gscale=None, velocity: bool = False,
                     grads=None, eps: float = 1e-4):
    lib = _lib.load()
    B, N, K, ch = means.shape
    pp = logw.shape[-1]
    g = _cuda(g, torch.float32)
    dt, means, logw, logg = _mix_dtype(means, logw, logg)
    sv = _sigma_vec(B, g.device, sigma_src, sigma_start, sigma_end)
    gs = None if gscale is None else _cuda(torch.as_tensor(gscale, device=g.device).flatten().expand(B), torch.float32)
    acc = grads is not None
    if not acc:
        grads = (torch.empty(B, N, K, ch, dtype=torch.float32, device=g.device),
                 torch.empty(B, N, K, pp, dtype=torch.float32, device=g.device),
                 torch.empty(B, N, K - 1, pp, dtype=torch.float32, device=g.device))
    _lib.check(lib.afx_arcflow_backward(_p(g), _p(means), _p(logw), _p(logg), dt, 0.0, 0.0, 0.0, _p(sv), _p(gs), 1.0, eps,
                                        _p(grads[0]), _p(grads[1]), _p(grads[2]), B, N, K, ch, pp, int(velocity), int(acc), _s()))
    return grads


def mse_loss(pred, target, coef: float, loss_accum: torch.Tensor, want_grad: bool = True):
    lib = _lib.load()
    pred, target = _cuda(pred, torch.float32), _cuda(target, torch.float32)
    grad = torch.empty_like(pred) if want_grad else None
    _lib.check(lib.afx_mse_loss(_p(pred), _p(target), coef, _p(grad), _p(loss_accum), pred.numel(), _s()))
    return grad


def euler_roll(x_a, u, sigma_a, sigma_b):
    lib = _lib.load()
    x_a, u = _cuda(x_a, torch.float32), _cuda(u, torch.float32)
    B = x_a.shape[0]
    sa = _cuda(sigma_a.flatten().expand(B), torch.float32)
    sb = _cuda(sigma_b.flatten().expand(B), torch.float32)
    out = torch.empty_like(x_a)
    _lib.check(lib.afx_euler_roll(_p(x_a), _p(u), _p(sa), _p(sb), _p(out), B, x_a[0].numel(), _s()))
    return out


def axpby_rows(a, alpha, b, beta):
    lib = _lib.load()
    a, b = _cuda(a, torch.float32), _cuda(b, torch.float32)
    B = a.shape[0]
    al, be = _cuda(alpha.flatten().expand(B), torch.float32), _cuda(beta.flatten().expand(B), torch.float32)
    out = torch.empty_like(a)
    _lib.check(lib.afx_axpby_rows(_p(a), _p(al), _p(b), _p(be), _p(out), B, a[0].numel(), _s()))
    return out


def cfg_combine(pos, neg, scale: float):
    lib = _lib.load()
    pos, neg = _cuda(pos, torch.float32), _cuda(neg, torch.float32)
    out = torch.empty_like(pos)
    _lib.check(lib.afx_cfg_combine(_p(pos), _p(neg), scale, _p(out), pos.numel(), _s()))
    return out


def head_grad(d_means, d_logw, d_logg, logw_out, ldy: int):
    lib = _lib.load()
    B, N, K, ch = d_means.shape
    lw = d_logw.shape[-1]
    dy = torch.empty(B * N, ldy, dtype=torch.bfloat16, device=d_means.device)
    _lib.check(lib.afx_head_grad(_p(d_means), _p(d_logw), _p(d_logg), _p(logw_out.contiguous()), _p(dy), ldy, B * N, K, ch, lw, _s()))
    return dy


def linear_f32out(a, w, out=None, accumulate: bool = False):
    lib = _lib.load()
    M, K = a.shape
    N = w.shape[0]
    if out is None:
        out = torch.zeros(M, N, dtype=torch.float32, device=a.device)
    _lib.check(lib.afx_linear_bf16_f32out(_p(a), a.stride(0), _p(w), w.stride(0), _p(out), out.stride(0), M, N, K,
                                          int(accumulate), _s()))
    return out


def linear_dropres(a, w, residual, p: float, seed: int, row0: int = 0, out=None):
    lib = _lib.load()
    M, K = a.shape
    N = w.shape[0]
    if out is None:
        out = torch.empty(M, N, dtype=torch.bfloat16, device=a.device)
    if not lib.afx_gemm_dropres_available():
        if out.data_ptr() != residual.data_ptr():
            out.copy_(residual)
        return lora_dropout(linear(a, w), p, seed, row0, mode=3, out=out)
    _lib.check(lib.afx_linear_bf16_dropres(_p(a), a.stride(0), _p(w), w.stride(0), _p(out), out.stride(0), M, N, K, _p(residual), residual.stride(0),
                                           float(p), seed & 0xffffffff, row0, _s()))
    return out


def linear_tn_f32out(x, y, out=None, accumulate: bool = False):
    lib = _lib.load()
    M, N1 = x.shape
    N2 = y.shape[1]
    assert y.shape[0] == M and x.stride(1) == 1 and y.stride(1) == 1
    if out is None:
        out = torch.zeros(N1, N2, dtype=torch.float32, device=x.device)
    nws = lib.afx_linear_tn_ws_bytes(M, N1, N2)
    ws = torch.empty(nws, dtype=torch.uint8, device=x.device) if nws > 0 else None
    _lib.check(lib.afx_linear_tn_f32out_ws(_p(x), x.stride(0), _p(y), y.stride(0), _p(out), out.stride(0), M, N1, N2, int(accumulate), _p(ws), _s()))
    return out


def quant_rows_fp8(x: torch.Tensor):
    lib = _lib.load()
    M, K = x.shape
    q = torch.empty(M, K, dtype=torch.uint8, device=x.device)
    scale = torch.empty(M, dtype=torch.float32, device=x.device)
    _lib.check(lib.afx_quant_rows_fp8(_p(x), x.stride(0), _p(q), K, _p(scale), M, K, _s()))
    return q, scale


def linear_fp8(aq, a_scale, wq, w_scale, bias=None, epilogue: str = 'none', gelu_col0: int = 0, gate=None, residual=None,
               rows_per_batch: int = 0, out=None):
    lib = _lib.load()
    M, K = aq.shape
    N = wq.shape[0]
    if out is None:
        out = torch.empty(M, N, dtype=torch.bfloat16, device=aq.device)
    epi = {'none': 0, 'gelu': 1, 'gate_res': 2}[epilogue]
    if gate is not None:
        gate = _cuda(gate, torch.float32)
        if gate.dim() == 1:
            gate = gate[None]
    rpb = rows_per_batch if rows_per_batch > 0 else max(M, 1)
    _lib.check(lib.afx_linear_fp8(_p(aq), aq.stride(0), _p(a_scale), _p(wq), wq.stride(0), _p(w_scale), _p(bias), _p(out), out.stride(0),
                                  M, N, K, epi, gelu_col0, _p(gate), 0 if gate is None else gate.stride(0), rpb, _p(residual),
                                  0 if residual is None else residual.stride(0), _s()))
    return out


def quant_rows_mx8(x: torch.Tensor):
    lib = _lib.load()
    M, K = x.shape
    q = torch.empty(M, K, dtype=torch.uint8, device=x.device)
    nb = K // 128
    mx = torch.empty(M, (nb + 3) // 4 * 4, dtype=torch.uint8, device=x.device)
    _lib.check(lib.afx_quant_rows_mx8(_p(x), x.stride(0), _p(q), K, _p(mx), mx.stride(0), M, K, _s()))
    return q, mx[:, :nb]


def linear_fp8_mx(aq, a_mx, wq, w_scale, bias=None, epilogue: str = 'none', gelu_col0: int = 0, gate=None, residual=None,
                  rows_per_batch: int = 0, out=None, a_scale=None):
    lib = _lib.load()
    M, K = aq.shape
    N = wq.shape[0]
    if out is None:
        out = torch.empty(M, N, dtype=torch.bfloat16, device=aq.device)
    if a_scale is None:
        a_scale = torch.ones(M, dtype=torch.float32, device=aq.device)
    epi = {'none': 0, 'gelu': 1, 'gate_res': 2}[epilogue]
    if gate is not None:
        gate = _cuda(gate, torch.float32)
        if gate.dim() == 1:
            gate = gate[None]
    rpb = rows_per_batch if rows_per_batch > 0 else max(M, 1)
    _lib.check(lib.afx_linear_fp8_mx(_p(aq), aq.stride(0), _p(a_mx), a_mx.stride(0), _p(a_scale), _p(wq), wq.stride(0), _p(w_scale), _p(bias),
                                     _p(out), out.stride(0), M, N, K, epi, gelu_col0, _p(gate), 0 if gate is None else gate.stride(0), rpb,
                                     _p(residual), 0 if residual is None else residual.stride(0), _s()))
    return out


def linear_fp8_to_mx8(aq, a_mx, wq, w_scale, bias=None, gelu: bool = False, c8_col0: int = 0, a_scale=None, out=None):
    lib = _lib.load()
    M, K = aq.shape
    N = wq.shape[0]
    n8 = N - c8_col0
    nb = (n8 + 127) // 128
    if out is None:
        head = torch.empty(M, c8_col0, dtype=torch.bfloat16, device=aq.device) if c8_col0 > 0 else None
        q = torch.empty(M, n8, dtype=torch.uint8, device=aq.device)
        mx = torch.empty(M, (nb + 3) // 4 * 4, dtype=torch.uint8, device=aq.device)
    else:
        head, q, mx = out
        assert (head is None) == (c8_col0 == 0) and (head is None or (head.shape == (M, c8_col0) and head.dtype == torch.bfloat16))
        assert q.shape == (M, n8) and q.dtype == torch.uint8 and mx.shape[0] == M and mx.shape[1] >= nb and mx.dtype == torch.uint8
        assert q.stride(1) == 1 and mx.stride(1) == 1 and q.stride(0) % 8 == 0 and mx.stride(0) % 4 == 0
        assert head is None or (head.stride(1) == 1 and head.stride(0) % 8 == 0)
    if a_scale is None:
        a_scale = torch.ones(M, dtype=torch.float32, device=aq.device)
    _lib.check(lib.afx_linear_fp8_to_mx8(_p(aq), aq.stride(0), _p(a_mx), 0 if a_mx is None else a_mx.stride(0), _p(a_scale), _p(wq), wq.stride(0),
                                         _p(w_scale), _p(bias), _p(head), head.stride(0) if head is not None else 8, _p(q), q.stride(0), _p(mx), mx.stride(0),
                                         c8_col0, M, N, K, int(gelu), _s()))
    return head, q, mx[:, :nb]


def linear_splitk(a, w, bias=None, residual=None, out=None, split_k: int = 0):
    lib = _lib.load()
    M, K = a.shape
    N = w.shape[0]
    n = lib.afx_linear_splitk_chunks(M, N, K, split_k)
    part = torch.empty(n, M, N, dtype=torch.float32, device=a.device)
    _lib.check(lib.afx_linear_bf16_splitk(_p(a), a.stride(0), _p(w), w.stride(0), _p(bias), _p(part), M, N, K, split_k, _s()))
    if out is None:
        out = torch.empty(M, N, dtype=torch.bfloat16, device=a.device)
    _lib.check(lib.afx_finish_f32_bf16(_p(part), n, _p(residual), 0 if residual is None else residual.stride(0), _p(out), out.stride(0),
                                       M, N, _s()))
    return out


def transpose(x, pad_to: int = 1):
    lib = _lib.load()
    R, Cc = x.shape
    Rp = (R + pad_to - 1) // pad_to * pad_to
    y = (torch.zeros if Rp != R else torch.empty)(Cc, Rp, dtype=torch.bfloat16, device=x.device)
    _lib.check(lib.afx_transpose_bf16(_p(x), x.stride(0), _p(y), Rp, R, Cc, _s()))
    return y


def coldot(a, b, out_accum):
    lib = _lib.load()
    _mat(a, torch.bfloat16, 'coldot a')
    _mat(b, torch.bfloat16, 'coldot b', a.shape)
    _acc(out_accum, (a.shape[1],), 'coldot out_accum')
    _lib.check(lib.afx_coldot_bf16(_p(a), a.stride(0), _p(b), b.stride(0), _p(out_accum), a.shape[0], a.shape[1], _s()))
    return out_accum


def gate_residual(y, gate, res, out=None):
    lib = _lib.load()
    _mat(y, torch.bfloat16, 'gate_residual y')
    _mat(res, torch.bfloat16, 'gate_residual res', y.shape)
    gate = _cuda(gate, torch.float32)
    if tuple(gate.shape) != (y.shape[1],):
        raise ValueError(f'gate_residual gate: need [{y.shape[1]}], got {tuple(gate.shape)}')
    if out is None:
        out = torch.empty(y.shape[0], y.shape[1], dtype=torch.bfloat16, device=y.device)
    _mat(out, torch.bfloat16, 'gate_residual out', y.shape)
    _lib.check(lib.afx_gate_residual_bf16(_p(y), y.stride(0), _p(gate), _p(res), res.stride(0), _p(out), out.stride(0),
                                          y.shape[0], y.shape[1], _s()))
    return out


def gemv_t(x, w, out_accum):
    lib = _lib.load()
    _mat(x, torch.float32, 'gemv_t x')
# ... 249 lines not shown
```

include/arcflow_hip.h:

```cpp
#ifndef ARCFLOW_HIP_H_
#define ARCFLOW_HIP_H_

#include <stddef.h>
#include <stdint.h>

#ifdef __cplusplus
extern "C" {
#endif

#define AFX_OK 0
#define AFX_MAX_MICRO_BATCH 4
#define AFX_E_INVALID (-1)
#define AFX_E_MISSING (-2)
#define AFX_E_WORKSPACE (-3)
#define AFX_E_HIP (-4)
#define AFX_E_UNSUPPORTED (-5)

#define AFX_DT_BF16 1
#define AFX_DT_F32 2
#define AFX_DT_FP8 3

typedef struct afx_ctx afx_ctx;

typedef struct afx_model_desc {
  int32_t family;
  int32_t num_double;
  int32_t num_single;
  int32_t heads;
  int32_t head_dim;
  int32_t in_channels;
  int32_t joint_dim;
  int32_t pooled_dim;
  int32_t guidance_embeds;
  int32_t num_gaussians;
  int32_t logweights_channels;
  int32_t head_mode;
} afx_model_desc;

const char* afx_last_error(void);
const char* afx_version(void);

int afx_create(const afx_model_desc* desc, afx_ctx** out);
int afx_destroy(afx_ctx* ctx);

int afx_bind_weight(afx_ctx* ctx, const char* name, const void* dptr, int32_t dtype,
                    int32_t ndim, const int64_t* shape);
int afx_finalize(afx_ctx* ctx);

int afx_head_width(const afx_ctx* ctx);

int64_t afx_workspace_bytes(const afx_ctx* ctx, int32_t batch, int32_t n_img, int32_t n_txt);
int afx_set_workspace(afx_ctx* ctx, void* dptr, int64_t bytes);

int afx_mmdit_forward(afx_ctx* ctx, const void* x, const void* ctx_emb, const void* pooled,
                      const float* t, const float* g, const float* rope_cos, const float* rope_sin,
                      int32_t batch, int32_t n_img, int32_t n_txt,
                      void* means, void* logw, void* logg, void* stream);

int afx_mmdit_prepare_steps(afx_ctx* ctx, const void* pooled, const float* t_steps, const float* g, int32_t batch, int32_t nsteps,
                            void* stream);
int afx_mmdit_use_prepared_step(afx_ctx* ctx, int32_t k);

int afx_set_checkpoint_buffer(afx_ctx* ctx, void* dptr);

int afx_profile_enable(afx_ctx* ctx, int32_t on);
int afx_profile_read(afx_ctx* ctx, int32_t klass, double* total_ms, int64_t* launches, double* flops);

int afx_arcflow_step(const float* x_in, const void* means, const void* logw, const void* logg,
                     int32_t mix_dtype, float sigma_src, float sigma_start, float sigma_end,
                     const float* sigma_vec, float eps, float* x_out,
                     int32_t batch, int32_t n_tok, int32_t K, int32_t ch, int32_t pp, void* stream);

int afx_arcflow_velocity(const void* means, const void* logw, const void* logg, int32_t mix_dtype,
                         float sigma_src, float sigma_t, const float* sigma_vec, float* u_out,
                         int32_t batch, int32_t n_tok, int32_t K, int32_t ch, int32_t pp, void* stream);


int afx_arcflow_step_dropout(const float* x_in, const void* means, const void* logw, const void* logg,
                             int32_t mix_dtype, const float* sigma_vec, const uint8_t* drop_mask, float eps,
                             float* x_out, int32_t batch, int32_t n_tok, int32_t K, int32_t ch, int32_t pp,
                             void* stream);

int afx_arcflow_backward(const float* g, const void* means, const void* logw, const void* logg, int32_t mix_dtype,
                         float sigma_src, float sigma_start, float sigma_end, const float* sigma_vec,
                         const float* gscale_vec, float gscale, float eps, float* d_means, float* d_logw,
                         float* d_logg, int32_t batch, int32_t n_tok, int32_t K, int32_t ch, int32_t pp,
                         int32_t velocity_only, int32_t accumulate, void* stream);

int afx_mse_loss(const float* pred, const float* target, float coef, float* grad, float* loss_accum, int64_t n,
                 void* stream);
int afx_euler_roll(const float* x_a, const float* u, const float* sigma_a, const float* sigma_b, float* out,
                   int32_t batch, int64_t per_sample, void* stream);
int afx_axpby_rows(const float* a, const float* alpha, const float* b, const float* beta, float* out, int32_t batch,
                   int64_t per_sample, void* stream);
int afx_cfg_combine(const float* pos, const float* neg, float scale, float* out, int64_t n, void* stream);

int afx_head_grad(const float* d_means, const float* d_logw, const float* d_logg, const void* logw_out, void* dy,
                  int64_t ldy, int64_t rows, int32_t K, int32_t ch, int32_t lw, void* stream);
int afx_linear_bf16_f32out(const void* A, int64_t lda, const void* W, int64_t ldw, float* C, int64_t ldc, int32_t M,
                           int32_t N, int32_t K, int32_t accumulate, void* stream);
int afx_linear_tn_f32out(const void* X, int64_t ldx, const void* Y, int64_t ldy, float* C, int64_t ldc, int32_t M, int32_t N1, int32_t N2,
                         int32_t accumulate, void* stream);
int64_t afx_linear_tn_ws_bytes(int32_t M, int32_t N1, int32_t N2);
int afx_linear_tn_f32out_ws(const void* X, int64_t ldx, const void* Y, int64_t ldy, float* C, int64_t ldc, int32_t M, int32_t N1, int32_t N2,
                            int32_t accumulate, void* ws, void* stream);
int afx_linear_bf16_dropres(const void* A, int64_t lda, const void* W, int64_t ldw, void* C, int64_t ldc, int32_t M, int32_t N, int32_t K,
                            const void* res, int64_t ldr, float p, uint32_t seed, int64_t row0, void* stream);
int afx_transpose_bf16(const void* x, int64_t ldx, void* y, int64_t ldy, int32_t rows, int32_t cols, void* stream);
int afx_colsum_bf16(const void* x, int64_t ldx, float* out_accum, int32_t rows, int32_t cols, void* stream);
int afx_normout_backward(const void* x, int64_t ldx, const void* dxn, int64_t ldd, float* dmod_accum, int32_t rows,
                         int32_t D, int32_t rows_per_batch, void* stream);
int afx_normout_backward_split(const void* x, int64_t ldx, const void* dxn, int64_t ldd, float* d_scale_accum, float* d_shift_accum, int32_t rows,
                               int32_t D, void* stream);
int afx_coldot_bf16(const void* a, int64_t lda, const void* b, int64_t ldb, float* out_accum, int32_t rows, int32_t cols, void* stream);
int afx_gate_residual_bf16(const void* y, int64_t ldy, const float* gate, const void* res, int64_t ldr, void* out, int64_t ldo,
                           int64_t rows, int32_t cols, void* stream);
int afx_gemv_t_bf16(const float* x, int64_t ldx, const void* W, int64_t ldw, float* out_accum, int32_t B, int64_t N, int32_t K,
                    void* stream);
int afx_outer_accum(const float* dmod, const float* x, float* dW_accum, int32_t B, int32_t J, int32_t Kd, void* stream);
int afx_mmdit_forward_stage(afx_ctx* ctx, const void* x, const void* ctx_emb, const void* pooled, const float* t, const float* g,
                            const float* rope_cos, const float* rope_sin, int32_t B, int32_t N, int32_t T, void* means, void* logw,
                            void* logg, int32_t stage, void* stream);
int afx_mmdit_import_tokens(afx_ctx* ctx, const void* src, int32_t batch, int32_t n_img, int32_t n_txt, void* stream);
int afx_set_fp8_linear(afx_ctx* ctx, int32_t on);
int afx_set_temb_override(afx_ctx* ctx, const float* temb_t);

int afx_mmdit_export(afx_ctx* ctx, const char* what, void* dst, int32_t batch, int32_t n_img, int32_t n_txt,
                     void* stream);

int afx_ln_modulate_backward(const void* x, int64_t ldx, const void* dxn, int64_t ldd, const float* scale, int64_t ldmod,
                             int32_t rows_per_batch, const void* dres, int64_t ldr, void* dx, int64_t ldo, int32_t rows,
                             int32_t D, void* stream);
int afx_qk_norm_rope_oop_bf16(const void* x, int64_t ldx, void* y, int64_t ldy, const void* dy, int64_t lddy,
                              const float* w_txt, const float* w_img, const float* rope_cos, const float* rope_sin,
                              int32_t batch, int32_t S, int32_t n_txt, int32_t heads, int32_t backward, void* stream);
int afx_gelu_bf16(const void* pre, int64_t ldp, const void* dh, int64_t ldh, void* out, int64_t ldo, int64_t rows,
                  int32_t cols, void* stream);
int afx_add_scale_bf16(const void* a, int64_t lda, const void* b, int64_t ldb, const float* gate, int64_t ldg,
                       int32_t rows_per_batch, void* out, int64_t ldo, int64_t rows, int32_t cols, void* stream);

int afx_sumsq(const float* x, float* out_accum, int64_t n, void* stream);
int afx_adamw_step(float* param, const float* grad, float* exp_avg, float* exp_avg_sq, float lr, float beta1,
                   float beta2, float eps, float weight_decay, int32_t step, float grad_scale, int64_t n, void* stream);
int afx_adamw8bit_step(float* param, const float* grad, void* state1, void* state2, float* absmax1, float* absmax2,
                       const float* qmap1, const float* qmap2, float lr, float beta1, float beta2, float eps, float weight_decay,
                       int32_t step, float grad_scale, int64_t n, void* stream);
int afx_ema_lerp(float* ema, const float* net, float beta, int64_t n, void* stream);
int afx_cast_f32_bf16(const float* x, void* y, int64_t n, void* stream);

int afx_conv3x3_bf16(const void* x, const void* w, const void* bias, void* y, int32_t H, int32_t W, int32_t Cin,
                     int32_t Cout, const void* res, void* stream);
#define AFX_GN_SLOTS 64
int64_t afx_groupnorm_ws_bytes(int32_t C, int32_t groups);
int afx_groupnorm_nhwc(const void* x, void* y, double* stats_ws, int32_t H, int32_t W, int32_t C, int32_t groups,
                       const float* gamma, const float* beta, float eps, int32_t act, void* stream);
int afx_conv3x3_bf16_stats(const void* x, const void* w, const void* bias, void* y, int32_t H, int32_t W, int32_t Cin, int32_t Cout,
                           const void* res, double* gn_stats, int32_t groups, void* stream);
int afx_groupnorm_nhwc_from_stats(const void* x, void* y, const double* gn_stats, double* stats_ws, int32_t H, int32_t W, int32_t C,
                                  int32_t groups, const float* gamma, const float* beta, float eps, int32_t act, void* stream);
int afx_conv_stats_available(void);
int afx_upconv3x3_bf16(const void* x, const void* w4, const void* bias, void* y, int32_t H, int32_t W, int32_t Cin, int32_t Cout, void* stream);
int afx_upsample2x_nhwc(const void* x, void* y, int32_t H, int32_t W, int32_t C, void* stream);
int afx_interior_nhwc(void* padded, void* compact, const void* res_padded, int32_t H, int32_t W, int32_t C, int32_t scatter,
                      void* stream);
int afx_softmax_rows_f32(const float* s, int64_t lds_, void* p, int64_t ldp, int32_t rows, int32_t cols, float scale,
                         void* stream);
int afx_latent_to_nhwc(const float* tokens, void* y, int32_t hp, int32_t wp, int32_t Cpad, float scaling_factor,
                       float shift_factor, void* stream);
int afx_nhwc_to_image(const void* x, float* img, int32_t H, int32_t W, int32_t C, void* stream);
int afx_latent_to_nhwc_affine(const float* tokens, void* y, int32_t hp, int32_t wp, int32_t Cpad, const float* A, const float* b,
                              void* stream);
int afx_rmsnorm_nhwc(const void* x, void* y, int64_t rows, int32_t Cpad, int32_t Creal, const float* gamma, int32_t act,
                     void* stream);

int afx_conv3x3s2_bf16(const void* x, const void* w, const void* bias, void* y, void* ws, int32_t H, int32_t W, int32_t Cin, int32_t Cout,
                       double* gn_stats, int32_t groups, void* stream);
int afx_image_to_cols27(const void* img, int32_t img_bf16, void* y, int32_t H, int32_t W, int32_t from01, void* stream);
int afx_posterior_latents(const void* grid, int32_t Cpad, int32_t h, int32_t w, const float* A, const float* b, const float* eps, const float* sub,
                          const float* fac, int32_t divide, float* out, int32_t packed, float* moments, void* stream);

int afx_embed_rows_bf16(const void* table, const int32_t* ids, const void* pos, void* out, int32_t S, int32_t D, void* stream);
int afx_norm_rows_bf16(const void* x, int64_t ldx, void* y, int64_t ldy, int32_t rows, int32_t D, const float* w, const float* b,
                       float eps, int32_t rms, void* stream);
int afx_act_mul_bf16(const void* x, int64_t ldx, void* out, int64_t ldo, int64_t M, int32_t F, int32_t gate_off, int32_t act,
                     void* stream);
int afx_rope_half_bf16(void* x, int64_t ldx, const float* cos_t, const float* sin_t, int32_t S, int32_t H, int32_t head_dim,
                       void* stream);
int afx_quant_rows_fp8(const void* x, int64_t ldx, void* q, int64_t ldq, float* scale, int32_t rows, int32_t K, void* stream);
int afx_linear_fp8(const void* Aq, int64_t lda, const float* a_scale, const void* Wq, int64_t ldw, const float* w_scale, const void* bias,
                   void* C, int64_t ldc, int32_t M, int32_t N, int32_t K, int32_t epi, int32_t gelu_col0, const float* gate, int64_t ldg,
                   int32_t rows_per_batch, const void* res, int64_t ldr, void* stream);
int afx_quant_rows_mx8(const void* x, int64_t ldx, void* q, int64_t ldq, void* mx, int64_t ld_mx, int32_t rows, int32_t K, void* stream);
int afx_linear_fp8_mx(const void* Aq, int64_t lda, const void* a_mx, int64_t ld_mx, const float* a_scale, const void* Wq, int64_t ldw,
                      const float* w_scale, const void* bias, void* C, int64_t ldc, int32_t M, int32_t N, int32_t K, int32_t epi,
                      int32_t gelu_col0, const float* gate, int64_t ldg, int32_t rows_per_batch, const void* res, int64_t ldr, void* stream);
int afx_linear_fp8_to_mx8(const void* Aq, int64_t lda, const void* a_mx, int64_t ld_mx, const float* a_scale, const void* Wq, int64_t ldw,
                          const float* w_scale, const void* bias, void* C, int64_t ldc, void* c8, int64_t ldc8, void* c_mx, int64_t ld_cmx,
                          int32_t c8_col0, int32_t M, int32_t N, int32_t K, int32_t gelu, void* stream);
int afx_linear_splitk_chunks(int32_t M, int32_t N, int32_t K, int32_t split_k);
int afx_linear_bf16_splitk(const void* A, int64_t lda, const void* W, int64_t ldw, const void* bias, float* partials, int32_t M,
                           int32_t N, int32_t K, int32_t split_k, void* stream);
int afx_finish_f32_bf16(const float* partials, int32_t nslab, const void* res, int64_t ldr, void* out, int64_t ldo, int64_t M, int32_t N,
                        void* stream);
int64_t afx_attention_ext_ws_bytes(int32_t B, int32_t Hkv, int32_t S, int32_t head_dim);
int afx_attention_ext_bf16(const void* q, int64_t ldq, const void* k, int64_t ldk, const void* v, int64_t ldv, void* o, int64_t ldo,
                           void* ws, int32_t B, int32_t H, int32_t Hkv, int32_t S, int32_t head_dim, float scale, int32_t causal,
                           const float* bias, void* stream);


int afx_linear_bf16(const void* A, int64_t lda, const void* W, int64_t ldw, const void* bias,
                    void* C, int64_t ldc, int32_t M, int32_t N, int32_t K,
                    int32_t epi, int32_t gelu_col0, const float* gate, int64_t ldg,
                    int32_t rows_per_batch, const void* res, int64_t ldr, void* stream);
int afx_linear_bf16_pre(const void* A, int64_t lda, const void* W, int64_t ldw, const void* bias,
                        void* C, int64_t ldc, int32_t M, int32_t N, int32_t K,
                        int32_t epi, int32_t gelu_col0, const float* gate, int64_t ldg,
                        int32_t rows_per_batch, const void* res, int64_t ldr, const void* pre, int64_t ldp, void* stream);
int afx_gemm_set_mode(int32_t impl, int32_t tile);
int afx_gemm_set_fp8_tile(int32_t tile);
int afx_gemm_dropres_available(void);
int afx_attn_set_impl(int32_t impl);
int afx_lora_dropout_bf16(const void* src, int64_t lds_, void* dst, int64_t ldd, int64_t M, int32_t N, int64_t row0, float p,
                          uint32_t seed, int32_t mode, void* stream);

int64_t afx_attention_ws_bytes(int32_t batch, int32_t heads, int32_t S);
int afx_attention_bf16(const void* q, int64_t ldq, const void* k, int64_t ldk, const void* v,
                       int64_t ldv, void* o, int64_t ldo, void* vt_ws,
                       int32_t batch, int32_t heads, int32_t S, void* stream);
int afx_attention_to_mx8(const void* q, int64_t ldq, const void* k, int64_t ldk, const void* v, int64_t ldv, void* o8, int64_t ldo8,
                         void* mx, int64_t ld_mx, void* vt_ws, int32_t batch, int32_t heads, int32_t S, void* stream);

int afx_attention_fwd_lse_bf16(const void* q, int64_t ldq, const void* k, int64_t ldk, const void* v, int64_t ldv, void* o,
                               int64_t ldo, float* lse, void* vt_ws, int32_t batch, int32_t heads, int32_t S, void* stream);
int64_t afx_attention_bwd_ws_bytes(int32_t batch, int32_t heads, int32_t S);
int afx_attn_bwd_set_impl(int32_t impl);
int afx_attention_bwd_bf16(const void* q, int64_t ldq, const void* k, int64_t ldk, const void* v, int64_t ldv, const void* o,
                           int64_t ldo, const void* dout, int64_t lddo, const float* lse, void* dq, int64_t lddq, void* dk,
                           int64_t lddk, void* dv, int64_t lddv, void* ws, int32_t batch, int32_t heads, int32_t S,
                           void* stream);

int afx_norm_modulate_bf16(const void* x, int64_t ldx, void* out, int64_t ldo, int32_t rows,
                           int32_t D, const float* scale, const float* shift, int64_t ldmod,
                           int32_t rows_per_batch, int32_t rms, void* stream);

int afx_qk_norm_rope_bf16(void* x, int64_t ldx, const float* w_txt, const float* w_img,
                          const float* rope_cos, const float* rope_sin,
                          int32_t batch, int32_t S, int32_t n_txt, int32_t heads, void* stream);

int afx_gemv_bf16(const float* x, const void* W, const void* bias, float* y, int32_t B, int32_t N,
                  int32_t K, int32_t act, int32_t accumulate, void* stream);

#define AFX_BLOCK_DOUBLE 0
#define AFX_BLOCK_SINGLE 1
#define AFX_QKV_AUTO 0
#define AFX_QKV_VT_PROJ 1
#define AFX_QKV_QK_EPI 2
#define AFX_QKV_KV_PREP 3
int afx_qkv_operands(int32_t kind, const void* A, int64_t lda, const void* w_img, const void* b_img, const void* w_txt, const void* b_txt,
                     const float* qkn, const float* rope_cos, const float* rope_sin, int32_t batch, int32_t n_img, int32_t n_txt,
                     int32_t heads, int32_t path, void* F, int64_t ldf, void* Vt, void* stream);
int afx_norm_modulate_joint_bf16(const void* x, int64_t ldx, void* out, int64_t ldo, int32_t rows, int32_t D, const float* scale,
                                 const float* shift, const float* scale_txt, const float* shift_txt, int64_t ldmod, int32_t S,
                                 int32_t n_txt, void* stream);
int afx_norm_modulate_mx8(const void* x, int64_t ldx, void* q8, int64_t ldq, void* mx, int64_t ld_mx, float* rowscale, int32_t rows,
                          int32_t D, const float* scale, const float* shift, const float* scale_txt, const float* shift_txt,
                          int64_t ldmod, int32_t S, int32_t n_txt, int32_t* fused, void* stream);

#ifdef __cplusplus
}
#endif
#endif
```

Measured before the change: 8.171 images/s.

## Multi-row GEMV, even row split for norm-modulate, skip prepared mod copies

The GEMV kernel now handles four output rows per wave for large N, using nontemporal weight loads so the activation vector is reused across rows. The R==2 norm-modulate path switches to a persistent-style grid that divides rows evenly among about twice the CU count. On stage 0 the forward reads prepared modulation vectors in place instead of copying them into the workspace, and export is redirected to the prepared buffers. A strided-output GEMV entry point is also added, and fp contraction is turned off in the GEMV, which may change rounding.

```diff
diff --git a/arcflow_amd/_lib.py b/arcflow_amd/_lib.py
--- a/arcflow_amd/_lib.py
+++ b/arcflow_amd/_lib.py
@@ -27,7 +27,7 @@
     'afx_arcflow_step_dropout', 'afx_arcflow_backward', 'afx_mse_loss', 'afx_euler_roll', 'afx_axpby_rows', 'afx_cfg_combine',
     'afx_head_grad', 'afx_linear_bf16_f32out', 'afx_linear_tn_f32out', 'afx_linear_tn_f32out_ws', 'afx_linear_tn_ws_bytes', 'afx_linear_bf16_dropres', 'afx_transpose_bf16', 'afx_colsum_bf16', 'afx_normout_backward', 'afx_normout_backward_split',
     'afx_outer_accum', 'afx_mmdit_export', 'afx_sumsq', 'afx_adamw_step', 'afx_adamw8bit_step', 'afx_ema_lerp', 'afx_cast_f32_bf16',
-    'afx_qkv_operands', 'afx_norm_modulate_joint_bf16', 'afx_norm_modulate_mx8',
+    'afx_qkv_operands', 'afx_norm_modulate_joint_bf16', 'afx_norm_modulate_mx8', 'afx_gemv_bf16_ld',
 ]
 
 AFX_BLOCK_DOUBLE, AFX_BLOCK_SINGLE = 0, 1
@@ -83,6 +83,7 @@
     lib.afx_norm_modulate_bf16.argtypes = [vp, i64, vp, i64, i32, i32, vp, vp, i64, i32, i32, vp]
     lib.afx_qk_norm_rope_bf16.argtypes = [vp, i64, vp, vp, vp, vp, i32, i32, i32, i32, vp]
     lib.afx_gemv_bf16.argtypes = [vp, vp, vp, vp, i32, i32, i32, i32, i32, vp]
+    lib.afx_gemv_bf16_ld.argtypes = [vp, vp, vp, vp, i64, i32, i32, i32, i32, i32, vp]
     lib.afx_attention_fwd_lse_bf16.argtypes = [vp, i64, vp, i64, vp, i64, vp, i64, vp, vp, i32, i32, i32, vp]
     lib.afx_attention_bwd_ws_bytes.argtypes = [i32, i32, i32]
     lib.afx_attention_bwd_ws_bytes.restype = i64
diff --git a/arcflow_amd/csrc/afx_elementwise.hip b/arcflow_amd/csrc/afx_elementwise.hip
--- a/arcflow_amd/csrc/afx_elementwise.hip
+++ b/arcflow_amd/csrc/afx_elementwise.hip
@@ -87,9 +87,17 @@
   constexpr bool MX8 = QOUT == 1;
   constexpr int D = 512 * NCH;
   const int lane = threadIdx.x & 63;
-  const int row0 = (blockIdx.x * 4 + (threadIdx.x >> 6)) * R;
-  if (row0 >= rows) return;
-  const int nrows = min(R, rows - row0);
+  int row0, nrows;
+  if constexpr (R == 0) {
+    const int64_t w = blockIdx.x * 4 + (threadIdx.x >> 6), nw = (int64_t)gridDim.x * 4;
+    row0 = (int)(w * rows / nw);
+    nrows = (int)((w + 1) * rows / nw) - row0;
+    if (nrows <= 0) return;
+  } else {
+    row0 = (blockIdx.x * 4 + (threadIdx.x >> 6)) * R;
+    if (row0 >= rows) return;
+    nrows = min(R, rows - row0);
+  }
   float sc[NCH][8], sh[NCH][8];
   int key = -1;
   u32x4_t cur[NCH], nxt[NCH];
@@ -217,10 +225,16 @@
                          scale_txt, shift_txt, n_txt, q8, ldq, mx, ld_mx, (float*)nullptr);
     return true;
   }
-  if (R == 2)
-    hipLaunchKernelGGL((norm_modulate_rows_kernel<6, 2, 0>), grid, dim3(256), 0, stream, x, ldx, out, ldo, rows, scale, shift, ldmod, rows_per_batch,
+  if (R == 2) {
+    static int cus = 0;
+    if (cus == 0) {
+      int dev = 0;
+      if (hipGetDevice(&dev) != hipSuccess || hipDeviceGetAttribute(&cus, hipDeviceAttributeMultiprocessorCount, dev) != hipSuccess || cus <= 0) cus = 256;
+    }
+    const dim3 span_grid(min(2 * cus, (rows + 7) / 8));
+    hipLaunchKernelGGL((norm_modulate_rows_kernel<6, 0, 0>), span_grid, dim3(256), 0, stream, x, ldx, out, ldo, rows, scale, shift, ldmod, rows_per_batch,
                        scale_txt, shift_txt, n_txt);
-  else
+  } else
     hipLaunchKernelGGL((norm_modulate_rows_kernel<6, 4, 0>), grid, dim3(256), 0, stream, x, ldx, out, ldo, rows, scale, shift, ldmod, rows_per_batch,
                        scale_txt, shift_txt, n_txt);
   return true;
@@ -326,39 +340,61 @@
 }
 
 constexpr int GEMV_MAXB = 8;
-
+constexpr int GEMV_ROWS = 4;
+constexpr int GEMV_ROWS_MIN_N = 8192;
+
+template <int R>
 __global__ __launch_bounds__(256) void gemv_kernel(const float* __restrict__ x, const bf16_t* __restrict__ W,
                                                    const bf16_t* __restrict__ bias, float* __restrict__ y,
                                                    int B, int N, int K, int act, int accumulate, int64_t ldy) {
+#pragma clang fp contract(off)
   const int lane = threadIdx.x & 63;
-  const int n = blockIdx.x * 4 + (threadIdx.x >> 6);
-  if (n >= N) return;
-  const bf16_t* wr = W + (int64_t)n * K;
-  float acc[GEMV_MAXB];
-#pragma unroll
-  for (int b = 0; b < GEMV_MAXB; ++b) acc[b] = 0.f;
+  const int n0 = (blockIdx.x * 4 + (threadIdx.x >> 6)) * R;
+  if (n0 >= N) return;
+  const bf16_t* wr[R];
+#pragma unroll
+  for (int r = 0; r < R; ++r) wr[r] = W + (int64_t)min(n0 + r, N - 1) * K;
+  float acc[R][GEMV_MAXB];
+#pragma unroll
+  for (int r = 0; r < R; ++r)
+#pragma unroll
+    for (int b = 0; b < GEMV_MAXB; ++b) acc[r][b] = 0.f;
   for (int c = lane; c < (K >> 3); c += 64) {
-    float w[8];
-    unpack8(*reinterpret_cast<const u32x4_t*>(wr + c * 8), w);
+    u32x4_t wv[R];
+#pragma unroll
+    for (int r = 0; r < R; ++r) {
+      const u32x4_t* wp = reinterpret_cast<const u32x4_t*>(wr[r] + c * 8);
+      wv[r] = R > 1 ? __builtin_nontemporal_load(wp) : *wp;
+    }
 #pragma unroll
     for (int b = 0; b < GEMV_MAXB; ++b) {
       if (b < B) {
         const f32x4_t x0 = *reinterpret_cast<const f32x4_t*>(x + (int64_t)b * K + c * 8);
         const f32x4_t x1 = *reinterpret_cast<const f32x4_t*>(x + (int64_t)b * K + c * 8 + 4);
-        acc[b] += w[0] * x0[0] + w[1] * x0[1] + w[2] * x0[2] + w[3] * x0[3] + w[4] * x1[0] + w[5] * x1[1] +
-                  w[6] * x1[2] + w[7] * x1[3];
-      }
-    }
-  }
-  const float bv = bias ? bf16_to_f32(bias[n]) : 0.f;
-#pragma unroll
-  for (int b = 0; b < GEMV_MAXB; ++b) {
-    if (b < B) {
-      float r = wave_sum(acc[b]) + bv;
-      if (act == 1) r = silu(r);
-      if (lane == 0) {
-        float* yp = y + (int64_t)b * ldy + n;
-        *yp = accumulate ? (*yp + r) : r;
+#pragma unroll
+        for (int r = 0; r < R; ++r) {
+          float w[8];
+          unpack8(wv[r], w);
+          acc[r][b] += w[0] * x0[0] + w[1] * x0[1] + w[2] * x0[2] + w[3] * x0[3] + w[4] * x1[0] + w[5] * x1[1] +
+                       w[6] * x1[2] + w[7] * x1[3];
+        }
+      }
+    }
+  }
+#pragma unroll
+  for (int r = 0; r < R; ++r) {
+    const int n = n0 + r;
+    if (n >= N) break;
+    const float bv = bias ? bf16_to_f32(bias[n]) : 0.f;
+#pragma unroll
+    for (int b = 0; b < GEMV_MAXB; ++b) {
+      if (b < B) {
+        float v = wave_sum(acc[r][b]) + bv;
+        if (act == 1) v = silu(v);
+        if (lane == 0) {
+          float* yp = y + (int64_t)b * ldy + n;
+          *yp = accumulate ? (*yp + v) : v;
+        }
       }
     }
   }
@@ -369,7 +405,11 @@
   if (ldy <= 0) ldy = N;
   if (B > GEMV_MAXB || (K & 7)) return hipErrorInvalidValue;
   if (N == 0 || B == 0) return hipSuccess;
-  hipLaunchKernelGGL(gemv_kernel, dim3((N + 3) / 4), dim3(256), 0, stream, x, W, bias, y, B, N, K, act, accumulate, ldy);
+  if (N >= GEMV_ROWS_MIN_N)
+    hipLaunchKernelGGL(gemv_kernel<GEMV_ROWS>, dim3((N + 4 * GEMV_ROWS - 1) / (4 * GEMV_ROWS)), dim3(256), 0, stream, x, W, bias, y, B, N, K, act,
+                       accumulate, ldy);
+  else
+    hipLaunchKernelGGL(gemv_kernel<1>, dim3((N + 3) / 4), dim3(256), 0, stream, x, W, bias, y, B, N, K, act, accumulate, ldy);
   return hipGetLastError();
 }
 
diff --git a/arcflow_amd/csrc/afx_engine.hip b/arcflow_amd/csrc/afx_engine.hip
--- a/arcflow_amd/csrc/afx_engine.hip
+++ b/arcflow_amd/csrc/afx_engine.hip
@@ -61,6 +61,7 @@
   int fp8_mx = -1;
   const float* temb_override = nullptr;
   int prep_steps = 0, prep_B = 0, prep_use = -1;
+  int cond_prep = -1;
   bool prof_on = false;
   int prof_stride = 1;
   uint64_t prof_count = 0;
@@ -435,6 +436,7 @@
   ctx->ws_bytes = bytes;
   ctx->prep_steps = 0;
   ctx->prep_use = -1;
+  ctx->cond_prep = -1;
   return AFX_OK;
 }
 
@@ -489,12 +491,18 @@
   const bool use_prep = c->prep_use >= 0 && c->prep_use < c->prep_steps && c->prep_B == B && stage != 2 && c->temb_override == nullptr;
   const int prep_k = c->prep_use;
   if (stage != 2) c->prep_use = -1;
+  const float* mod = ws.mod;
   if (use_prep) {
     const int64_t r0 = (int64_t)prep_k * B;
-    HIP_TRY(hipMemcpyAsync(ws.mod, ws.prep_mod + r0 * ldm, (size_t)B * ldm * 4, hipMemcpyDeviceToDevice, st));
-    HIP_TRY(hipMemcpyAsync(ws.temb, ws.prep_temb + r0 * D, (size_t)B * D * 4, hipMemcpyDeviceToDevice, st));
-    HIP_TRY(hipMemcpyAsync(ws.semb, ws.prep_semb + r0 * D, (size_t)B * D * 4, hipMemcpyDeviceToDevice, st));
-  }
+    if (stage == 0) {
+      mod = ws.prep_mod + r0 * ldm;
+    } else {
+      HIP_TRY(hipMemcpyAsync(ws.mod, ws.prep_mod + r0 * ldm, (size_t)B * ldm * 4, hipMemcpyDeviceToDevice, st));
+      HIP_TRY(hipMemcpyAsync(ws.temb, ws.prep_temb + r0 * D, (size_t)B * D * 4, hipMemcpyDeviceToDevice, st));
+      HIP_TRY(hipMemcpyAsync(ws.semb, ws.prep_semb + r0 * D, (size_t)B * D * 4, hipMemcpyDeviceToDevice, st));
+    }
+  }
+  if (stage != 2) c->cond_prep = use_prep && stage == 0 ? prep_k : -1;
   if (stage != 2 && !use_prep) {
   if (c->temb_override != nullptr) {
     HIP_TRY(hipMemcpyAsync(ws.temb, c->temb_override, (size_t)B * D * 4, hipMemcpyDeviceToDevice, st));
@@ -581,7 +589,7 @@
         p.epi = epi; p.gelu_col0 = 0;
         if (qkn != nullptr) stream_qk_epilogue(p, bs, qkn, s);
         if (epi == EPI_GATE_RES) {
-          p.gate = ws.mod + (int64_t)b * ldm + ml.dbl(blk, s, gate_chunk); p.ldg = 0; p.rows_per_batch = 1 << 30;
+          p.gate = mod + (int64_t)b * ldm + ml.dbl(blk, s, gate_chunk); p.ldg = 0; p.rows_per_batch = 1 << 30;
           p.res = C + row0 * ldc; p.ldr = ldc;
         }
       }
@@ -605,14 +613,14 @@
   auto stream_norm = [&](int blk, int shift_chunk, int scale_chunk) -> int {
     norm_fused = false;
     if (mx) {
-      HIP_TRY(launch_norm_modulate_mx8(ws.X, D, ws.q8n, D, ws.mxn, ws.ld_mxn, (int)R, (int)D, ws.mod + ml.dbl(blk, 0, scale_chunk),
-                                       ws.mod + ml.dbl(blk, 0, shift_chunk), ws.mod + ml.dbl(blk, 1, scale_chunk),
-                                       ws.mod + ml.dbl(blk, 1, shift_chunk), ldm, (int)S, T, st, &norm_fused, norm_rows ? ws.qs : nullptr));
+      HIP_TRY(launch_norm_modulate_mx8(ws.X, D, ws.q8n, D, ws.mxn, ws.ld_mxn, (int)R, (int)D, mod + ml.dbl(blk, 0, scale_chunk),
+                                       mod + ml.dbl(blk, 0, shift_chunk), mod + ml.dbl(blk, 1, scale_chunk),
+                                       mod + ml.dbl(blk, 1, shift_chunk), ldm, (int)S, T, st, &norm_fused, norm_rows ? ws.qs : nullptr));
       if (norm_fused) return AFX_OK;
     }
-    HIP_TRY(launch_norm_modulate_joint(ws.X, D, ws.Xn, D, (int)R, (int)D, ws.mod + ml.dbl(blk, 0, scale_chunk),
-                                       ws.mod + ml.dbl(blk, 0, shift_chunk), ws.mod + ml.dbl(blk, 1, scale_chunk),
-                                       ws.mod + ml.dbl(blk, 1, shift_chunk), ldm, S, T, st));
+    HIP_TRY(launch_norm_modulate_joint(ws.X, D, ws.Xn, D, (int)R, (int)D, mod + ml.dbl(blk, 0, scale_chunk),
+                                       mod + ml.dbl(blk, 0, shift_chunk), mod + ml.dbl(blk, 1, scale_chunk),
+                                       mod + ml.dbl(blk, 1, shift_chunk), ldm, S, T, st));
     return AFX_OK;
   };
 
@@ -650,9 +658,9 @@
     if (c->ckpt)
       HIP_TRY(hipMemcpyAsync(c->ckpt + (int64_t)(d.num_double + i) * R * D, ws.X, (size_t)R * D * 2, hipMemcpyDeviceToDevice, st));
     bool sgl_fused = false;
-    if (mx) HIP_TRY(launch_norm_modulate_mx8(ws.X, D, ws.q8n, D, ws.mxn, ws.ld_mxn, (int)R, (int)D, ws.mod + ml.sgl(i, 1), ws.mod + ml.sgl(i, 0),
+    if (mx) HIP_TRY(launch_norm_modulate_mx8(ws.X, D, ws.q8n, D, ws.mxn, ws.ld_mxn, (int)R, (int)D, mod + ml.sgl(i, 1), mod + ml.sgl(i, 0),
                                              nullptr, nullptr, ldm, (int)S, 0, st, &sgl_fused, norm_rows ? ws.qs : nullptr));
-    if (!sgl_fused) HIP_TRY(launch_norm_modulate(ws.X, D, ws.Xn, D, (int)R, (int)D, ws.mod + ml.sgl(i, 1), ws.mod + ml.sgl(i, 0), ldm, S, 0, st));
+    if (!sgl_fused) HIP_TRY(launch_norm_modulate(ws.X, D, ws.Xn, D, (int)R, (int)D, mod + ml.sgl(i, 1), mod + ml.sgl(i, 0), ldm, S, 0, st));
     GemmBatch gb{};
     single_qkv_batch(gb, spath, bs, ws.Xn, D, bw.fused, ws.F, 7 * D, qkn);
     GemmProblem& f = gb.p[0];
@@ -678,7 +686,7 @@
     o = GemmProblem{};
     o.A = ws.F + 2 * D; o.lda = 7 * D; o.W = bw.out.w; o.ldw = 5 * D; o.bias = bw.out.b;
     o.C = ws.X; o.ldc = D; o.M = (int)R; o.N = (int)D; o.K = (int)(5 * D); o.epi = EPI_GATE_RES;
-    o.gate = ws.mod + ml.sgl(i, 2); o.ldg = ldm; o.rows_per_batch = S; o.res = ws.X; o.ldr = D;
+    o.gate = mod + ml.sgl(i, 2); o.ldg = ldm; o.rows_per_batch = S; o.res = ws.X; o.ldr = D;
     if (mx) {
       if (!o_fused) HIP_TRY(launch_quant_rows_mx8(ws.F + 2 * D, 7 * D, ws.q8, 5 * D, ws.mxw, ws.ld_mxw, (int)R, (int)D, st));
       o.A = (const uint16_t*)ws.q8; o.lda = 5 * D; o.W = (const uint16_t*)bw.out.wq; o.fp8 = 1; o.a_scale = ws.ones; o.w_scale = bw.out.wscale;
@@ -693,7 +701,7 @@
 
   for (int b = 0; b < B; ++b)
     HIP_TRY(launch_norm_modulate(ws.X + ((int64_t)b * S + T) * D, D, ws.Xn + (int64_t)b * N * D, D, N, (int)D,
-                                 ws.mod + (int64_t)b * ldm + ml.fin(0), ws.mod + (int64_t)b * ldm + ml.fin(1), 0,
+                                 mod + (int64_t)b * ldm + ml.fin(0), mod + (int64_t)b * ldm + ml.fin(1), 0,
                                  1 << 30, 0, st));
   {
     GemmBatch gb{};
@@ -732,6 +740,7 @@
   const int rows = B * nsteps;
   c->prep_steps = 0;
   c->prep_use = -1;
+  if (c->cond_prep >= 0) c->cond_prep = -2;
   float* sc = ws.prep_semb;
   for (int k = 0; k < nsteps; ++k) {
     float* temb = ws.prep_temb + (int64_t)k * B * D;
@@ -945,6 +954,13 @@
   ModLayout ml{D, c->d.num_double, c->d.num_single};
   hipStream_t st = (hipStream_t)stream;
   const std::string w(what);
+  const float *temb = ws.temb, *semb = ws.semb, *mod = ws.mod;
+  if (c->cond_prep != -1 && (w == "temb" || w == "silu_temb" || w == "mod_all" || w == "mod_final")) {
+    if (c->cond_prep < 0 || c->cond_prep >= c->prep_steps || batch != c->prep_B)
+      return fail(AFX_E_INVALID, "afx_mmdit_export: '%s' of a forward on a prepared step must be read with that forward's batch and before the next afx_mmdit_prepare_steps", what);
+    const int64_t r0 = (int64_t)c->cond_prep * batch;
+    temb = ws.prep_temb + r0 * D; semb = ws.prep_semb + r0 * D; mod = ws.prep_mod + r0 * c->n_mod;
+  }
   if (w == "head_in") {
     HIP_TRY(hipMemcpyAsync(dst, ws.Xn, (size_t)batch * n_img * D * 2, hipMemcpyDeviceToDevice, st));
   } else if (w == "x_final") {
@@ -954,14 +970,14 @@
   } else if (w == "x_tokens") {
     HIP_TRY(hipMemcpyAsync(dst, ws.X, (size_t)batch * (n_img + n_txt) * D * 2, hipMemcpyDeviceToDevice, st));
   } else if (w == "temb") {
-    HIP_TRY(hipMemcpyAsync(dst, ws.temb, (size_t)batch * D * 4, hipMemcpyDeviceToDevice, st));
+    HIP_TRY(hipMemcpyAsync(dst, temb, (size_t)batch * D * 4, hipMemcpyDeviceToDevice, st));
   } else if (w == "silu_temb") {
-    HIP_TRY(hipMemcpyAsync(dst, ws.semb, (size_t)batch * D * 4, hipMemcpyDeviceToDevice, st));
+    HIP_TRY(hipMemcpyAsync(dst, semb, (size_t)batch * D * 4, hipMemcpyDeviceToDevice, st));
   } else if (w == "mod_all") {
-    HIP_TRY(hipMemcpyAsync(dst, ws.mod, (size_t)batch * c->n_mod * 4, hipMemcpyDeviceToDevice, st));
+    HIP_TRY(hipMemcpyAsync(dst, mod, (size_t)batch * c->n_mod * 4, hipMemcpyDeviceToDevice, st));
   } else if (w == "mod_final") {
     for (int b = 0; b < batch; ++b)
-      HIP_TRY(hipMemcpyAsync((char*)dst + (size_t)b * 2 * D * 4, ws.mod + (int64_t)b * c->n_mod + ml.fin(0), (size_t)2 * D * 4,
+      HIP_TRY(hipMemcpyAsync((char*)dst + (size_t)b * 2 * D * 4, mod + (int64_t)b * c->n_mod + ml.fin(0), (size_t)2 * D * 4,
                              hipMemcpyDeviceToDevice, st));
   } else {
     return fail(AFX_E_INVALID, "afx_mmdit_export: unknown buffer '%s'", what);
@@ -1124,6 +1140,14 @@
   if (!x || !W || !y) return fail(AFX_E_INVALID, "null argument to afx_gemv_bf16");
   if (B < 1 || B > 8 || N < 1 || K < 8 || K % 8) return fail(AFX_E_INVALID, "bad gemv shape (B<=8, K%%8==0)");
   HIP_TRY(launch_gemv(x, (const uint16_t*)W, (const uint16_t*)bias, y, B, N, K, act, accumulate, (hipStream_t)stream));
+  return AFX_OK;
+}
+
+int afx_gemv_bf16_ld(const float* x, const void* W, const void* bias, float* y, int64_t ldy, int32_t B, int32_t N, int32_t K,
+                     int32_t act, int32_t accumulate, void* stream) {
+  if (!x || !W || !y) return fail(AFX_E_INVALID, "null argument to afx_gemv_bf16_ld");
+  if (B < 1 || B > 8 || N < 1 || K < 8 || K % 8 || ldy < N) return fail(AFX_E_INVALID, "bad gemv shape (B<=8, K%%8==0, ldy>=N)");
+  HIP_TRY(launch_gemv(x, (const uint16_t*)W, (const uint16_t*)bias, y, B, N, K, act, accumulate, (hipStream_t)stream, ldy));
   return AFX_OK;
 }
 
diff --git a/arcflow_amd/ops.py b/arcflow_amd/ops.py
--- a/arcflow_amd/ops.py
+++ b/arcflow_amd/ops.py
@@ -260,7 +260,10 @@
     N = w.shape[0]
     if out is None:
         out = torch.zeros(B, N, dtype=torch.float32, device=x.device)
-    _lib.check(lib.afx_gemv_bf16(_p(x), _p(w), _p(bias), _p(out), B, N, K, 1 if act == 'silu' else 0, int(accumulate), _s()))
+    if out.shape != (B, N) or out.dtype != torch.float32 or out.stride(1) != 1 or (B > 1 and out.stride(0) < N):
+        raise ValueError(f'gemv out: expected fp32 [{B}, {N}] with unit inner stride and row stride >= {N}')
+    _lib.check(lib.afx_gemv_bf16_ld(_p(x), _p(w), _p(bias), _p(out), out.stride(0) if B > 1 else N, B, N, K, 1 if act == 'silu' else 0,
+                                    int(accumulate), _s()))
     return out
 
 
diff --git a/include/arcflow_hip.h b/include/arcflow_hip.h
--- a/include/arcflow_hip.h
+++ b/include/arcflow_hip.h
@@ -249,6 +249,8 @@
 
 int afx_gemv_bf16(const float* x, const void* W, const void* bias, float* y, int32_t B, int32_t N,
                   int32_t K, int32_t act, int32_t accumulate, void* stream);
+int afx_gemv_bf16_ld(const float* x, const void* W, const void* bias, float* y, int64_t ldy, int32_t B, int32_t N,
+                     int32_t K, int32_t act, int32_t accumulate, void* stream);
 
 #define AFX_BLOCK_DOUBLE 0
 #define AFX_BLOCK_SINGLE 1
```

New measurement: 8.229 images/s, median of 6. No clear change (+0.7%).
